# alenzhao/Mitty

Hardware: AMD Instinct MI355X
Metric: paired 2x150bp reads/sec at 30x WGS, 1/2/4/8 MI355X; qname POS/CIGAR bit-exact (higher is better)
Workload: dtype int64+u8

## Files before the change

include/mitty_hip.h:

```cpp
#ifndef MITTY_HIP_H
#define MITTY_HIP_H

#include <stdint.h>

#ifdef __cplusplus
extern "C" {
#endif

typedef struct mh_ctx mh_ctx;

enum {
  MH_OK = 0,
  MH_E_ARG = -1,
  MH_E_HIP = -2,
  MH_E_OOM = -3,
  MH_E_CAPACITY = -4,
  MH_E_COMPLEX_VARIANT = -5,
  MH_E_SEED = -6,
  MH_E_STATE = -7,
  MH_E_NO_DEVICE = -8
};

enum { MH_RNG_MITTY = 0, MH_RNG_PHILOX = 1 };

int32_t mh_version(void);
int32_t mh_device_count(int32_t *out);
int32_t mh_create(int32_t device, mh_ctx **out);
int32_t mh_destroy(mh_ctx *ctx);
const char *mh_last_error(const mh_ctx *ctx);
int32_t mh_sync(mh_ctx *ctx);

int32_t mh_selftest_scan_fault(mh_ctx *ctx);
int32_t mh_selftest_scan(mh_ctx *ctx, int32_t kind, int32_t fields, const int64_t *in, int64_t n, int32_t repeat,
                         int64_t *incl, int64_t *excl, int64_t *total, int64_t *info);
int32_t mh_selftest_sort(mh_ctx *ctx, const uint32_t *keys, int64_t n, int32_t end_bit, uint32_t *keys_out,
                         uint32_t *vals_out);

int32_t mh_read_model_params(int64_t mean_rlen, double coverage, double *p, int64_t *passes);
int32_t mh_work_units(uint64_t seed, const int32_t *ploidy, int64_t n_regions, int64_t passes,
                      int32_t *out_region, int32_t *out_cpy, uint32_t *out_seed, int64_t *out_n);

int32_t mh_upload_contig(mh_ctx *ctx, int32_t contig_id, const char *seq, int64_t len);
int32_t mh_release_contig(mh_ctx *ctx, int32_t contig_id);
int32_t mh_build_haplotype(mh_ctx *ctx, int32_t slot, int32_t contig_id, int64_t ref_start_pos,
                           const int64_t *v_pos, const uint8_t *v_op, const int64_t *v_oplen,
                           const int64_t *v_alt_off, const int64_t *v_alt_len, const char *alt_pool,
                           int64_t alt_pool_len, int64_t n_var,
                           int64_t *out_n_nodes, int64_t *out_p_min, int64_t *out_p_max);
int32_t mh_upload_variants(mh_ctx *ctx, int32_t vset, const int64_t *v_pos, const uint8_t *v_op,
                           const int64_t *v_oplen, const int64_t *v_alt_off, const int64_t *v_alt_len,
                           const char *alt_pool, int64_t alt_pool_len, int64_t n_var);
int32_t mh_build_haplotype_vset(mh_ctx *ctx, int32_t slot, int32_t contig_id, int64_t ref_start_pos, int32_t vset,
                                int64_t *out_n_nodes, int64_t *out_p_min, int64_t *out_p_max);
int32_t mh_build_haplotypes_vset(mh_ctx *ctx, int32_t n, const int32_t *slots, const int32_t *contig_ids,
                                 const int64_t *ref_starts, const int32_t *vsets, int64_t *out_n_nodes,
                                 int64_t *out_p_min, int64_t *out_p_max);
int32_t mh_prefetch_haplotypes_vset(mh_ctx *ctx, int32_t n, const int32_t *slots, const int32_t *contig_ids,
                                    const int64_t *ref_starts, const int32_t *vsets, int32_t n_units,
                                    const int32_t *unit_slots, const uint64_t *unit_seeds, double p);
int32_t mh_release_variants(mh_ctx *ctx, int32_t vset);
int32_t mh_get_nodes(mh_ctx *ctx, int32_t slot, int64_t *ps, int64_t *pr, uint8_t *op, int64_t *oplen,
                     char *hap, int64_t hap_cap, int64_t *hap_len);
int32_t mh_get_haplotype_aux(mh_ctx *ctx, int32_t slot, char *rc, int64_t rc_cap, int64_t *hap_len,
                             int64_t *run_start, int64_t *run_end, int64_t run_cap, int64_t *n_runs,
                             int32_t *bkt, int64_t bkt_cap, int64_t *n_bkt);
int32_t mh_release_haplotype(mh_ctx *ctx, int32_t slot);
int32_t mh_expand_variant(int64_t samp_pos, int64_t ref_pos, int64_t ref_start_pos, int64_t v_pos, int32_t op,
                          int64_t oplen, int64_t *out, int32_t *n_nodes, int64_t *samp_next, int64_t *ref_next);

int32_t mh_sample_templates(mh_ctx *ctx, int32_t slot, double p, int32_t rlen, const double *cum_tlen,
                            int32_t n_tlen, uint64_t seed, int32_t rng_mode, int64_t *out_n_templates);
int32_t mh_sample_templates_span(mh_ctx *ctx, int64_t p_min, int64_t p_max, double p, int32_t rlen,
                                 const double *cum_tlen, int32_t n_tlen, uint64_t seed, int32_t rng_mode,
                                 int64_t *out_n_templates);
int32_t mh_sample_units(mh_ctx *ctx, int32_t n_units, const int32_t *tpl_ids, const int32_t *slots,
                        const uint64_t *seeds, double p, int32_t rlen, const double *cum_tlen, int32_t n_tlen,
                        int32_t rng_mode, int64_t *out_n);
int32_t mh_sample_units_async(mh_ctx *ctx, int32_t n_units, const int32_t *tpl_ids, const int32_t *slots,
                              const uint64_t *seeds, double p, int32_t rlen, const double *cum_tlen, int32_t n_tlen,
                              int32_t rng_mode);
int32_t mh_templates_count(mh_ctx *ctx, int32_t tpl_id, int64_t *n);
int32_t mh_use_templates(mh_ctx *ctx, int32_t tpl_id);
int32_t mh_release_templates(mh_ctx *ctx, int32_t tpl_id);
int32_t mh_set_templates(mh_ctx *ctx, const int8_t *fo0, const int64_t *pos0, const int64_t *pos1, int64_t n,
                         int32_t rlen);
int32_t mh_get_templates(mh_ctx *ctx, int8_t *fo0, int64_t *pos0, int64_t *pos1, int64_t cap, int64_t *n);
int32_t mh_templates_export(mh_ctx *ctx, int32_t tpl_id, int32_t on_device, int8_t *fo0, int64_t *pos0,
                            int64_t *pos1, int64_t cap, int64_t *n);
int32_t mh_templates_import(mh_ctx *ctx, int32_t tpl_id, int32_t on_device, const int8_t *fo0, const int64_t *pos0,
                            const int64_t *pos1, int64_t n, int32_t rlen);

int32_t mh_emit_reads(mh_ctx *ctx, int32_t slot, const char *serial_stub, const char *chrom, int64_t cpy,
                      int32_t write_fastq2, uint64_t unit_key, int64_t *out_kept, int64_t *out_bytes1,
                      int64_t *out_bytes2);
int32_t mh_emit_prepare(mh_ctx *ctx, int32_t slot, const char *serial_stub, const char *chrom, int64_t cpy,
                        int32_t write_fastq2, uint64_t unit_key, int64_t *out_kept, int64_t *out_b1, int64_t *out_b2);
int32_t mh_emit_reads_range(mh_ctx *ctx, int32_t slot, const char *serial_stub, const char *chrom, int64_t cpy,
                            int32_t write_fastq2, uint64_t unit_key, int64_t t_begin, int64_t t_end,
                            int64_t cnt_base, int64_t *out_kept, int64_t *out_bytes1, int64_t *out_bytes2);
int32_t mh_emit_reads_async(mh_ctx *ctx, int32_t slot, const char *serial_stub, const char *chrom, int64_t cpy,
                            int32_t write_fastq2, uint64_t unit_key);
int32_t mh_emit_collect(mh_ctx *ctx, int64_t *out, int64_t cap, int64_t *n_units);
int32_t mh_emit_measure(mh_ctx *ctx, int32_t slot, const char *serial_stub, const char *chrom, int64_t cpy,
                        int32_t write_fastq2, uint64_t unit_key, int64_t t_begin, int64_t t_end, int64_t cnt_base,
                        int64_t *out_kept, int64_t *out_b1, int64_t *out_b2);
int32_t mh_count_kept(mh_ctx *ctx, int32_t slot, int64_t t_begin, int64_t t_end, int64_t *out_kept);
int32_t mh_output_size(mh_ctx *ctx, int64_t *bytes1, int64_t *bytes2);
int32_t mh_output_fetch(mh_ctx *ctx, int64_t offset1, char *fq1, int64_t len1, int64_t offset2, char *fq2,
                        int64_t len2);
int32_t mh_output_fetch_async(mh_ctx *ctx, int64_t offset1, char *fq1, int64_t len1, int64_t offset2, char *fq2,
                              int64_t len2, int32_t *ticket);
int32_t mh_output_fetch_wait(mh_ctx *ctx, int32_t ticket);
int32_t mh_output_reset(mh_ctx *ctx);
int32_t mh_host_alloc(int64_t bytes, void **out);
int32_t mh_host_free(void *p);
int32_t mh_device_cache_trim(int64_t *freed_bytes);
int32_t mh_device_live_bytes(int64_t *live, int64_t *peak, int32_t reset_peak);

int32_t mh_read_batch(mh_ctx *ctx, int32_t slot, const int64_t *p, const int64_t *l, int64_t n,
                      int64_t *out_pos, int64_t *out_n0, int64_t *out_n1,
                      char *cigar, int64_t cigar_cap, int64_t *cigar_off, int64_t *cigar_used,
                      char *vlist, int64_t vlist_cap, int64_t *vlist_off, int64_t *vlist_used,
                      char *seq, int64_t seq_cap, int64_t *seq_off, int64_t *seq_used);

int32_t mh_bam_set_refs(mh_ctx *ctx, int32_t n_refs, const char *names, const int64_t *lengths);
int32_t mh_bam_add_fastq(mh_ctx *ctx, const char *fq1, int64_t len1, const char *fq2, int64_t len2,
                         int64_t max_templates, int64_t *used1, int64_t *used2, int64_t *templates);
int32_t mh_bam_add_output(mh_ctx *ctx, int64_t max_templates, int64_t *templates);
int32_t mh_bam_records(mh_ctx *ctx, int64_t *n_records, int64_t *bytes);
int32_t mh_bam_sort(mh_ctx *ctx);
int32_t mh_bam_write(mh_ctx *ctx, const char *bam_path, const char *header_text, int64_t header_len, int32_t level,
                     int32_t threads, const char *bai_path, int64_t *out_records, int64_t *out_bytes);
int32_t mh_bam_reset(mh_ctx *ctx);
int32_t mh_bam_set_capacity(mh_ctx *ctx, int64_t bytes);
int32_t mh_bam_set_spill_dir(mh_ctx *ctx, const char *dir);
int32_t mh_bam_spilled(mh_ctx *ctx, int64_t *bytes, int64_t *blocks);
int32_t mh_bam_export(mh_ctx *ctx, int64_t r0, int64_t r1, uint8_t *recs, int64_t *roff, uint64_t *keys,
                      int32_t *info);
int32_t mh_bam_import(mh_ctx *ctx, const uint8_t *recs, const int64_t *roff, const uint64_t *keys, const int32_t *info,
                      int64_t n);
int32_t mh_bam_write_gpu(mh_ctx *ctx, const char *bam_path, const char *header_text, int64_t header_len,
                         const char *bai_path, int64_t *out_records, int64_t *out_bytes, int64_t *out_file_bytes);
int32_t mh_bam_partition(mh_ctx *ctx, const uint64_t *splitters, int32_t n_dest, uint64_t tie_base, int64_t *seg_off,
                         int64_t *seg_n, int64_t *seg_bytes);
int32_t mh_bam_partition_fetch(mh_ctx *ctx, void *out, int64_t cap);
int32_t mh_bam_import_tie(mh_ctx *ctx, const uint8_t *recs, const int64_t *roff, const uint64_t *keys,
                          const int32_t *info, const uint64_t *ties, int64_t n);
int32_t mh_bam_sorted_head(mh_ctx *ctx, int64_t len, uint8_t *out);
int32_t mh_bam_write_part(mh_ctx *ctx, const char *path, const char *header_text, int64_t header_len, int64_t skip,
                          const uint8_t *tail, int64_t tail_len, int32_t eof, int64_t *out_blocks, int64_t *out_data_pos,
                          int64_t *out_bytes, int64_t *boff, int64_t boff_cap);
int32_t mh_bam_bai_runs(mh_ctx *ctx, int64_t *n_runs, int64_t *runs, int64_t runs_cap, int64_t *n_win, int64_t *win,
                        int64_t win_cap, int64_t *ref_nwin);

typedef struct mh_bamfile mh_bamfile;
int32_t mh_bamfile_open(const char *path, int32_t threads, mh_bamfile **out);
int32_t mh_bamfile_open_gpu(const char *path, int32_t device, int32_t threads, mh_bamfile **out);
const char *mh_bamfile_error(const mh_bamfile *f);
int32_t mh_bamfile_header(const mh_bamfile *f, const char **text, int64_t *text_len, int32_t *n_ref,
                          const char **names, const int64_t **lengths);
int32_t mh_bamfile_next(mh_bamfile *f, int64_t max_bytes, const uint8_t **recs, int64_t *len, const int64_t **roff,
                        int64_t *n);
int32_t mh_bamfile_close(mh_bamfile *f);

int32_t mh_score_begin(mh_ctx *ctx, int32_t n_refs, const char *names, int32_t max_d, int32_t max_v_len,
                       int32_t strict, const char *sample_prefix);
int32_t mh_score_add_records(mh_ctx *ctx, const uint8_t *recs, int64_t len, const int64_t *roff, int64_t n);
int32_t mh_score_add_store(mh_ctx *ctx);
int32_t mh_score_result(mh_ctx *ctx, uint64_t *mq_mat, uint64_t *derr_mat, int64_t *counts);
int32_t mh_score_reset(mh_ctx *ctx);

#define MH_MODEL_NO_RLEN INT64_MAX
int32_t mh_model_begin(mh_ctx *ctx, int32_t n_refs, int32_t every, int32_t min_mq, int32_t max_bq, int32_t max_bp,
                       int32_t max_tlen);
int32_t mh_model_add_records(mh_ctx *ctx, const uint8_t *recs, int64_t len, const int64_t *roff, int64_t n);
int32_t mh_model_add_store(mh_ctx *ctx);
int32_t mh_model_result(mh_ctx *ctx, uint64_t *bq_mat, uint64_t *tlen_mat, int64_t *counts);
int32_t mh_model_reset(mh_ctx *ctx);

#define MH_COV_NO_POS INT64_MAX
int32_t mh_cov_begin(mh_ctx *ctx, int32_t n_refs, const int64_t *lengths, int64_t block_len);
int32_t mh_cov_add_records(mh_ctx *ctx, const uint8_t *recs, int64_t len, const int64_t *roff, int64_t n);
int32_t mh_cov_add_store(mh_ctx *ctx);
int32_t mh_cov_gc(mh_ctx *ctx, int32_t ref_index, int32_t contig_id);
int32_t mh_cov_result(mh_ctx *ctx, int32_t ref_index, uint32_t *n_n, uint32_t *n_gc, int64_t *covered,
                      uint64_t *span_sum, int64_t *min_pos, int64_t *max_end, int64_t n_blocks, int64_t *counts);
int32_t mh_cov_reset(mh_ctx *ctx);

#define MH_BQ_MAX_BP 500
// ... 68 lines not shown
```

mitty_amd/_native.py:

```python
import ctypes
import os
import sys

import numpy as np

LIB_PATH = (os.environ.get('MH_LIB') or
            os.path.join(os.path.dirname(os.path.abspath(__file__)), '_lib', 'libmitty_hip.so'))

MH_OK, MH_E_ARG, MH_E_HIP, MH_E_OOM, MH_E_CAPACITY, MH_E_COMPLEX_VARIANT, MH_E_SEED, MH_E_STATE, MH_E_NO_DEVICE = \
  0, -1, -2, -3, -4, -5, -6, -7, -8
MH_RNG_MITTY, MH_RNG_PHILOX = 0, 1

EXPORTS = ['mh_version', 'mh_device_count', 'mh_create', 'mh_destroy', 'mh_last_error', 'mh_sync',
           'mh_selftest_scan_fault', 'mh_selftest_scan', 'mh_selftest_sort', 'mh_selftest_bgzf',
           'mh_read_model_params', 'mh_work_units', 'mh_upload_contig', 'mh_release_contig', 'mh_build_haplotype', 'mh_upload_variants', 'mh_build_haplotype_vset', 'mh_build_haplotypes_vset', 'mh_prefetch_haplotypes_vset', 'mh_release_variants', 'mh_get_nodes', 'mh_get_haplotype_aux',
           'mh_release_haplotype', 'mh_expand_variant', 'mh_sample_templates', 'mh_sample_templates_span', 'mh_set_templates',
           'mh_get_templates', 'mh_templates_export', 'mh_templates_import', 'mh_emit_reads', 'mh_emit_prepare', 'mh_emit_reads_async', 'mh_emit_collect', 'mh_output_size', 'mh_output_fetch', 'mh_output_reset', 'mh_host_alloc', 'mh_host_free', 'mh_device_cache_trim', 'mh_device_live_bytes',
           'mh_read_batch', 'mh_set_corruption', 'mh_set_corruption_stream', 'mh_get_corruption_stream', 'mh_stage_times', 'mh_enable_timing', 'mh_sample_units', 'mh_sample_units_async', 'mh_templates_count',
           'mh_use_templates', 'mh_release_templates', 'mh_mt_window_at', 'mh_fixup_count', 'mh_set_emit_mode', 'mh_set_decode_mode',
           'mh_emit_reads_range', 'mh_emit_measure', 'mh_count_kept', 'mh_bam_set_refs', 'mh_bam_add_fastq', 'mh_bam_add_output',
           'mh_bam_records', 'mh_bam_set_capacity', 'mh_bam_set_spill_dir', 'mh_bam_spilled', 'mh_bam_export', 'mh_bam_import', 'mh_bam_sort', 'mh_bam_write', 'mh_bam_write_gpu', 'mh_bam_reset', 'mh_bam_partition', 'mh_bam_partition_fetch', 'mh_bam_import_tie', 'mh_bam_sorted_head', 'mh_bam_write_part', 'mh_bam_bai_runs', 'mh_corrupt_fastq', 'mh_bgzf_compress', 'mh_bgzf_eof', 'mh_bgzf_compress_device', 'mh_bgzf_compress_gpu', 'mh_output_bgzf',
           'mh_output_bgzf_range', 'mh_output_bgzf_pair', 'mh_output_bgzf_wait', 'mh_output_fetch_async',
           'mh_output_fetch_wait',
           'mh_vcf_open', 'mh_vcf_error', 'mh_vcf_close', 'mh_vcf_region', 'mh_vcf_copy', 'mh_vcf_filter',
           'mh_bamfile_open', 'mh_bamfile_open_gpu', 'mh_bgzf_inflate_gpu', 'mh_bamfile_error', 'mh_bamfile_header', 'mh_bamfile_next', 'mh_bamfile_close',
           'mh_score_begin', 'mh_score_add_records', 'mh_score_add_store', 'mh_score_result', 'mh_score_reset',
           'mh_model_begin', 'mh_model_add_records', 'mh_model_add_store', 'mh_model_result', 'mh_model_reset',
           'mh_cov_begin', 'mh_cov_add_records', 'mh_cov_add_store', 'mh_cov_gc', 'mh_cov_result', 'mh_cov_reset',
           'mh_bq_begin', 'mh_bq_add_records', 'mh_bq_add_store', 'mh_bq_result', 'mh_bq_reset',
           'mh_fasta_open', 'mh_fasta_error', 'mh_fasta_count', 'mh_fasta_contig', 'mh_fasta_copy', 'mh_fasta_close']


MODEL_NO_RLEN = (1 << 63) - 1
COV_NO_POS = (1 << 63) - 1
BQ_MAX_BP, BQ_MAX_BQ = 500, 100


class NativeError(RuntimeError):
  pass


class NativeUnavailable(NativeError):
  pass


_lib = None

c_i32, c_i64, c_u64, c_dbl, c_vp = ctypes.c_int32, ctypes.c_int64, ctypes.c_uint64, ctypes.c_double, ctypes.c_void_p
P_i64 = ctypes.POINTER(c_i64)


def _sig(L, name, args, res=c_i32):
  f = getattr(L, name)
  f.argtypes = args
  f.restype = res


def lib():
  global _lib
  if _lib is not None:
    return _lib
  if not os.path.exists(LIB_PATH):
    raise NativeUnavailable('libmitty_hip.so not built ({}); run __graft_entry__.build() or make -C '
                            'mitty_amd/csrc'.format(LIB_PATH))
  if 'torch' not in sys.modules and int(os.environ.get('WORLD_SIZE', '1')) > 1:
    import torch
  L = ctypes.CDLL(LIB_PATH)
  _sig(L, 'mh_version', [])
  _sig(L, 'mh_device_count', [ctypes.POINTER(c_i32)])
  _sig(L, 'mh_create', [c_i32, ctypes.POINTER(c_vp)])
  _sig(L, 'mh_destroy', [c_vp])
  _sig(L, 'mh_last_error', [c_vp], ctypes.c_char_p)
  _sig(L, 'mh_sync', [c_vp])
  _sig(L, 'mh_selftest_scan_fault', [c_vp])
  _sig(L, 'mh_selftest_scan', [c_vp, c_i32, c_i32, c_vp, c_i64, c_i32, c_vp, c_vp, c_vp, c_vp])
  _sig(L, 'mh_selftest_sort', [c_vp, c_vp, c_i64, c_i32, c_vp, c_vp])
  _sig(L, 'mh_selftest_bgzf', [c_vp, c_vp, c_i64, c_i32, c_vp, c_i64, P_i64])
  _sig(L, 'mh_read_model_params', [c_i64, c_dbl, ctypes.POINTER(c_dbl), P_i64])
  _sig(L, 'mh_work_units', [c_u64, c_vp, c_i64, c_i64, c_vp, c_vp, c_vp, P_i64])
  _sig(L, 'mh_upload_contig', [c_vp, c_i32, c_vp, c_i64])
  _sig(L, 'mh_release_contig', [c_vp, c_i32])
  _sig(L, 'mh_upload_variants', [c_vp, c_i32, c_vp, c_vp, c_vp, c_vp, c_vp, c_vp, c_i64, c_i64])
  _sig(L, 'mh_build_haplotype_vset', [c_vp, c_i32, c_i32, c_i64, c_i32, c_vp, c_vp, c_vp])
  _sig(L, 'mh_release_variants', [c_vp, c_i32])
  _sig(L, 'mh_build_haplotype', [c_vp, c_i32, c_i32, c_i64, c_vp, c_vp, c_vp, c_vp, c_vp, c_vp, c_i64, c_i64,
                                 P_i64, P_i64, P_i64])
  _sig(L, 'mh_get_nodes', [c_vp, c_i32, c_vp, c_vp, c_vp, c_vp, c_vp, c_i64, P_i64])
  _sig(L, 'mh_get_haplotype_aux', [c_vp, c_i32, c_vp, c_i64, P_i64, c_vp, c_vp, c_i64, P_i64, c_vp, c_i64, P_i64])
  _sig(L, 'mh_release_haplotype', [c_vp, c_i32])
  _sig(L, 'mh_bgzf_compress_device', [c_vp, c_vp, c_i64, c_vp, c_i64, P_i64])
  _sig(L, 'mh_bgzf_compress_gpu', [c_vp, c_vp, c_i64, c_vp, c_i64, P_i64])
  _sig(L, 'mh_output_bgzf', [c_vp, c_i32, c_vp, c_i64, P_i64])
  _sig(L, 'mh_output_bgzf_range', [c_vp, c_i32, c_i64, c_i64, c_vp, c_i64, P_i64])
  _sig(L, 'mh_output_bgzf_pair', [c_vp, c_i64, c_i64, c_i64, c_vp, c_i64, c_vp, c_i64, P_i64, P_i64,
                                  ctypes.POINTER(c_i32)])
  _sig(L, 'mh_output_bgzf_wait', [c_vp, c_i32])
  _sig(L, 'mh_output_fetch_async', [c_vp, c_i64, c_vp, c_i64, c_i64, c_vp, c_i64, ctypes.POINTER(c_i32)])
  _sig(L, 'mh_output_fetch_wait', [c_vp, c_i32])
  _sig(L, 'mh_expand_variant', [c_i64, c_i64, c_i64, c_i64, c_i32, c_i64, P_i64, ctypes.POINTER(c_i32), P_i64, P_i64])
  _sig(L, 'mh_sample_templates', [c_vp, c_i32, c_dbl, c_i32, c_vp, c_i32, c_u64, c_i32, P_i64])
  _sig(L, 'mh_sample_templates_span', [c_vp, c_i64, c_i64, c_dbl, c_i32, c_vp, c_i32, c_u64, c_i32, P_i64])
  _sig(L, 'mh_set_templates', [c_vp, c_vp, c_vp, c_vp, c_i64, c_i32])
  _sig(L, 'mh_get_templates', [c_vp, c_vp, c_vp, c_vp, c_i64, P_i64])
  _sig(L, 'mh_emit_reads', [c_vp, c_i32, ctypes.c_char_p, ctypes.c_char_p, c_i64, c_i32, c_u64, P_i64, P_i64, P_i64])
  _sig(L, 'mh_emit_prepare', [c_vp, c_i32, ctypes.c_char_p, ctypes.c_char_p, c_i64, c_i32, c_u64, P_i64, P_i64, P_i64])
  _sig(L, 'mh_emit_reads_async', [c_vp, c_i32, ctypes.c_char_p, ctypes.c_char_p, c_i64, c_i32, c_u64])
  _sig(L, 'mh_emit_collect', [c_vp, c_vp, c_i64, P_i64])
  _sig(L, 'mh_build_haplotypes_vset', [c_vp, c_i32, c_vp, c_vp, c_vp, c_vp, c_vp, c_vp, c_vp])
  _sig(L, 'mh_prefetch_haplotypes_vset', [c_vp, c_i32, c_vp, c_vp, c_vp, c_vp, c_i32, c_vp, c_vp, c_dbl])
  _sig(L, 'mh_emit_reads_range', [c_vp, c_i32, ctypes.c_char_p, ctypes.c_char_p, c_i64, c_i32, c_u64, c_i64, c_i64,
                                   c_i64, P_i64, P_i64, P_i64])
  _sig(L, 'mh_count_kept', [c_vp, c_i32, c_i64, c_i64, P_i64])
  _sig(L, 'mh_emit_measure', [c_vp, c_i32, ctypes.c_char_p, ctypes.c_char_p, c_i64, c_i32, c_u64, c_i64, c_i64, c_i64,
                              P_i64, P_i64, P_i64])
  _sig(L, 'mh_bam_set_refs', [c_vp, c_i32, ctypes.c_char_p, c_vp])
  _sig(L, 'mh_bam_add_fastq', [c_vp, c_vp, c_i64, c_vp, c_i64, c_i64, P_i64, P_i64, P_i64])
  _sig(L, 'mh_bam_add_output', [c_vp, c_i64, P_i64])
  _sig(L, 'mh_bam_records', [c_vp, P_i64, P_i64])
  _sig(L, 'mh_bam_set_capacity', [c_vp, c_i64])
  _sig(L, 'mh_bam_spilled', [c_vp, P_i64, P_i64])
  _sig(L, 'mh_bam_export', [c_vp, c_i64, c_i64, c_vp, c_vp, c_vp, c_vp])
  _sig(L, 'mh_bam_import', [c_vp, c_vp, c_vp, c_vp, c_vp, c_i64])
  _sig(L, 'mh_bam_partition', [c_vp, c_vp, c_i32, ctypes.c_uint64, c_vp, c_vp, c_vp])
  _sig(L, 'mh_bam_set_spill_dir', [c_vp, ctypes.c_char_p])
  _sig(L, 'mh_bam_partition_fetch', [c_vp, c_vp, c_i64])
  _sig(L, 'mh_bam_import_tie', [c_vp, c_vp, c_vp, c_vp, c_vp, c_vp, c_i64])
  _sig(L, 'mh_bam_sorted_head', [c_vp, c_i64, c_vp])
  _sig(L, 'mh_bam_write_part', [c_vp, ctypes.c_char_p, ctypes.c_char_p, c_i64, c_i64, c_vp, c_i64, c_i32, P_i64,
                                P_i64, P_i64, c_vp, c_i64])
  _sig(L, 'mh_bam_bai_runs', [c_vp, P_i64, c_vp, c_i64, P_i64, c_vp, c_i64, c_vp])
  _sig(L, 'mh_bam_write', [c_vp, ctypes.c_char_p, ctypes.c_char_p, c_i64, c_i32, c_i32, ctypes.c_char_p, P_i64,
                           P_i64])
  _sig(L, 'mh_bam_write_gpu', [c_vp, ctypes.c_char_p, ctypes.c_char_p, c_i64, ctypes.c_char_p, P_i64, P_i64, P_i64])
  _sig(L, 'mh_bam_reset', [c_vp])
  _sig(L, 'mh_bam_sort', [c_vp])
  _sig(L, 'mh_corrupt_fastq', [c_vp, c_vp, c_i64, c_vp, c_i64, c_i64, P_i64, P_i64, P_i64])
  _sig(L, 'mh_bgzf_compress', [c_vp, c_i64, c_i32, c_i32, c_vp, c_i64, P_i64])
  _sig(L, 'mh_bgzf_eof', [c_vp])
  _sig(L, 'mh_vcf_open', [ctypes.c_char_p, ctypes.c_char_p, ctypes.POINTER(c_vp)])
  _sig(L, 'mh_vcf_error', [c_vp], ctypes.c_char_p)
  _sig(L, 'mh_vcf_close', [c_vp])
  _sig(L, 'mh_vcf_region', [c_vp, ctypes.c_char_p, c_i64, c_i64, ctypes.POINTER(c_i32), c_vp, c_vp, c_i32])
  _sig(L, 'mh_vcf_copy', [c_vp, c_i32, c_vp, c_vp, c_vp, c_vp, c_vp, c_vp])
  _sig(L, 'mh_vcf_filter', [ctypes.c_char_p, ctypes.c_char_p, c_i32, c_vp, c_vp, c_vp, ctypes.c_char_p, c_i32, c_i32,
                            P_i64, P_i64, ctypes.c_char_p, c_i32])
  _sig(L, 'mh_bamfile_open', [ctypes.c_char_p, c_i32, ctypes.POINTER(c_vp)])
  _sig(L, 'mh_bamfile_open_gpu', [ctypes.c_char_p, c_i32, c_i32, ctypes.POINTER(c_vp)])
  _sig(L, 'mh_bgzf_inflate_gpu', [c_i32, c_vp, c_i64, c_vp, c_i64, P_i64, P_i64])
  _sig(L, 'mh_bamfile_error', [c_vp], ctypes.c_char_p)
  _sig(L, 'mh_bamfile_header', [c_vp, ctypes.POINTER(c_vp), P_i64, ctypes.POINTER(c_i32), ctypes.POINTER(c_vp),
                                ctypes.POINTER(c_vp)])
  _sig(L, 'mh_bamfile_next', [c_vp, c_i64, ctypes.POINTER(c_vp), P_i64, ctypes.POINTER(c_vp), P_i64])
  _sig(L, 'mh_bamfile_close', [c_vp])
  _sig(L, 'mh_score_begin', [c_vp, c_i32, ctypes.c_char_p, c_i32, c_i32, c_i32, ctypes.c_char_p])
  _sig(L, 'mh_score_add_records', [c_vp, c_vp, c_i64, c_vp, c_i64])
  _sig(L, 'mh_score_add_store', [c_vp])
  _sig(L, 'mh_score_result', [c_vp, c_vp, c_vp, c_vp])
  _sig(L, 'mh_score_reset', [c_vp])
  _sig(L, 'mh_model_begin', [c_vp, c_i32, c_i32, c_i32, c_i32, c_i32, c_i32])
  _sig(L, 'mh_model_add_records', [c_vp, c_vp, c_i64, c_vp, c_i64])
  _sig(L, 'mh_model_add_store', [c_vp])
  _sig(L, 'mh_model_result', [c_vp, c_vp, c_vp, c_vp])
  _sig(L, 'mh_model_reset', [c_vp])
  _sig(L, 'mh_cov_begin', [c_vp, c_i32, c_vp, c_i64])
  _sig(L, 'mh_cov_add_records', [c_vp, c_vp, c_i64, c_vp, c_i64])
  _sig(L, 'mh_cov_add_store', [c_vp])
  _sig(L, 'mh_cov_gc', [c_vp, c_i32, c_i32])
  _sig(L, 'mh_cov_result', [c_vp, c_i32, c_vp, c_vp, c_vp, c_vp, c_vp, c_vp, c_i64, c_vp])
  _sig(L, 'mh_cov_reset', [c_vp])
  _sig(L, 'mh_bq_begin', [c_vp, c_i32])
  _sig(L, 'mh_bq_add_records', [c_vp, c_vp, c_i64, c_vp, c_i64])
  _sig(L, 'mh_bq_add_store', [c_vp])
  _sig(L, 'mh_bq_result', [c_vp, c_i32, c_vp, c_vp])
  _sig(L, 'mh_bq_reset', [c_vp])
  _sig(L, 'mh_fasta_open', [ctypes.c_char_p, c_vp, ctypes.POINTER(c_vp)])
  _sig(L, 'mh_fasta_error', [c_vp], ctypes.c_char_p)
  _sig(L, 'mh_fasta_count', [c_vp, ctypes.POINTER(c_i32)])
  _sig(L, 'mh_fasta_contig', [c_vp, c_i32, ctypes.POINTER(ctypes.c_char_p), ctypes.POINTER(c_vp), P_i64])
  _sig(L, 'mh_fasta_copy', [c_vp, c_i32, c_vp])
  _sig(L, 'mh_fasta_close', [c_vp])
  _sig(L, 'mh_output_size', [c_vp, P_i64, P_i64])
  _sig(L, 'mh_output_fetch', [c_vp, c_i64, c_vp, c_i64, c_i64, c_vp, c_i64])
  _sig(L, 'mh_output_reset', [c_vp])
  _sig(L, 'mh_host_alloc', [c_i64, ctypes.POINTER(c_vp)])
  _sig(L, 'mh_host_free', [c_vp])
  _sig(L, 'mh_device_cache_trim', [ctypes.POINTER(c_i64)])
  _sig(L, 'mh_device_live_bytes', [ctypes.POINTER(c_i64), ctypes.POINTER(c_i64), c_i32])
  _sig(L, 'mh_read_batch', [c_vp, c_i32, c_vp, c_vp, c_i64, c_vp, c_vp, c_vp,
                            c_vp, c_i64, c_vp, P_i64, c_vp, c_i64, c_vp, P_i64, c_vp, c_i64, c_vp, P_i64])
  _sig(L, 'mh_set_corruption', [c_vp, c_i32, c_vp, c_i32, c_i32, c_vp, c_u64])
  _sig(L, 'mh_templates_export', [c_vp, c_i32, c_i32, c_vp, c_vp, c_vp, c_i64, P_i64])
  _sig(L, 'mh_templates_import', [c_vp, c_i32, c_i32, c_vp, c_vp, c_vp, c_i64, c_i32])
  _sig(L, 'mh_set_corruption_stream', [c_vp, c_i32, c_u64, c_vp, c_i32])
  _sig(L, 'mh_get_corruption_stream', [c_vp, c_vp, ctypes.POINTER(c_i32), P_i64])
  _sig(L, 'mh_stage_times', [c_vp, ctypes.POINTER(ctypes.c_char_p), ctypes.POINTER(c_dbl), c_i32,
                             ctypes.POINTER(c_i32)])
  _sig(L, 'mh_enable_timing', [c_vp, c_i32])
  _sig(L, 'mh_sample_units', [c_vp, c_i32, c_vp, c_vp, c_vp, c_dbl, c_i32, c_vp, c_i32, c_i32, c_vp])
  _sig(L, 'mh_sample_units_async', [c_vp, c_i32, c_vp, c_vp, c_vp, c_dbl, c_i32, c_vp, c_i32, c_i32])
  _sig(L, 'mh_templates_count', [c_vp, c_i32, c_vp])
  _sig(L, 'mh_use_templates', [c_vp, c_i32])
  _sig(L, 'mh_release_templates', [c_vp, c_i32])
  _sig(L, 'mh_mt_window_at', [ctypes.c_uint32, c_u64, c_vp])
  _sig(L, 'mh_fixup_count', [c_vp, P_i64])
  _sig(L, 'mh_set_emit_mode', [c_vp, c_i32])
  _sig(L, 'mh_set_decode_mode', [c_vp, c_i32])
  _lib = L
  return L


def mt_window_at(seed, offset):
  out = np.empty(624, np.uint32)
  rc = lib().mh_mt_window_at(int(seed), int(offset), _ptr(out))
  if rc:
    _raise(rc, 'mh_mt_window_at failed')
  return out


def bgzf_compress(data, level=6, threads=8):
  n = len(data)
  src = np.frombuffer(data, np.uint8) if n else np.zeros(1, np.uint8)
  cap = n + (n // 0xff00 + 1) * 64 + 64
  out = np.empty(cap, np.uint8)
  used = c_i64()
  rc = lib().mh_bgzf_compress(_ptr(src), n, int(level), int(threads), _ptr(out), cap, ctypes.byref(used))
  if rc == MH_E_CAPACITY:
    out = np.empty(used.value, np.uint8)
    rc = lib().mh_bgzf_compress(_ptr(src), n, int(level), int(threads), _ptr(out), used.value, ctypes.byref(used))
  if rc:
# ... 802 lines not shown
    self._chk(self._L.mh_bq_add_store(self._h))

  def bq_result(self, ref_index):
    mat = np.zeros((BQ_MAX_BP, BQ_MAX_BQ), np.uint64)
    cnt = np.zeros(8, np.int64)
    self._chk(self._L.mh_bq_result(self._h, int(ref_index), _ptr(mat), _ptr(cnt)))
    return mat, _model_counts(cnt)

  def bq_reset(self):
    self._chk(self._L.mh_bq_reset(self._h))

  def bam_partition(self, splitters, tie_base):
    sp = np.ascontiguousarray(splitters, dtype=np.uint64)
    nd = len(sp) + 1
    off, n, nb = np.zeros(nd + 1, np.int64), np.zeros(nd, np.int64), np.zeros(nd, np.int64)
    self._chk(self._L.mh_bam_partition(self._h, _ptr(sp) if len(sp) else None, nd, int(tie_base), _ptr(off), _ptr(n),
                                       _ptr(nb)))
    return off, n, nb

  def bam_partition_fetch(self, ptr, cap):
    self._chk(self._L.mh_bam_partition_fetch(self._h, c_vp(ptr), int(cap)))

  def bam_import_tie(self, n, nbytes, ptr):
    o_roff, o_key, o_info, o_tie, _ = bam_part_layout(n, nbytes)
    self._chk(self._L.mh_bam_import_tie(self._h, c_vp(ptr), c_vp(ptr + o_roff), c_vp(ptr + o_key),
                                        c_vp(ptr + o_info), c_vp(ptr + o_tie), int(n)))

  def bam_sorted_head(self, n):
    out = np.empty(max(int(n), 1), np.uint8)
    self._chk(self._L.mh_bam_sorted_head(self._h, int(n), _ptr(out)))
    return out[:int(n)].tobytes()

  def bam_write_part(self, path, header_text=None, skip=0, tail=b'', eof=False):
    nb, dp, fb = c_i64(), c_i64(), c_i64()
    h = header_text.encode() if header_text is not None else b''
    t = np.frombuffer(tail, np.uint8) if len(tail) else None
    args = (self._h, path.encode(), h, len(h) if header_text is not None else -1, int(skip), _ptr(t), len(tail),
            1 if eof else 0, ctypes.byref(nb), ctypes.byref(dp), ctypes.byref(fb))
    n_bytes = self.bam_records()[1]
    cap = (n_bytes - int(skip) + len(tail)) // 0xff00 + 2
    boff = np.zeros(cap, np.int64)
    self._chk(self._L.mh_bam_write_part(*args, _ptr(boff), cap))
    return nb.value, dp.value, fb.value, boff[:nb.value + 1]

  def bam_bai_runs(self, n_refs):
    nr, nw = c_i64(), c_i64()
    self._chk(self._L.mh_bam_bai_runs(self._h, ctypes.byref(nr), None, 0, ctypes.byref(nw), None, 0, None))
    runs = np.zeros(max(4 * nr.value, 4), np.int64)
    win = np.zeros(max(nw.value, 1), np.int64)
    rn = np.zeros(max(n_refs, 1), np.int64)
    self._chk(self._L.mh_bam_bai_runs(self._h, ctypes.byref(nr), _ptr(runs), len(runs), ctypes.byref(nw), _ptr(win),
                                      len(win), _ptr(rn)))
    return runs[:4 * nr.value].reshape(-1, 4), win[:nw.value], rn[:n_refs]

  def bam_sort(self):
    self._chk(self._L.mh_bam_sort(self._h))

  def corrupt_fastq(self, fq1, fq2=None, t_base=0):
    u1, u2, t = c_i64(), c_i64(), c_i64()
    a1 = np.frombuffer(fq1, np.uint8) if len(fq1) else np.zeros(1, np.uint8)
    a2 = None if fq2 is None else (np.frombuffer(fq2, np.uint8) if len(fq2) else np.zeros(1, np.uint8))
    self._chk(self._L.mh_corrupt_fastq(self._h, _ptr(a1), len(fq1), None if a2 is None else _ptr(a2),
                                       0 if fq2 is None else len(fq2), int(t_base), ctypes.byref(u1),
                                       ctypes.byref(u2), ctypes.byref(t)))
    return u1.value, u2.value, t.value

  def read_batch(self, slot, p, l):
    p = np.ascontiguousarray(p, dtype=np.int64)
    l = np.ascontiguousarray(l, dtype=np.int64)
    n = len(p)
    pos, n0, n1 = (np.empty(max(n, 1), np.int64) for _ in range(3))
    offs = [np.empty(n + 1, np.int64) for _ in range(3)]
    used = [c_i64() for _ in range(3)]
    caps = [max(64, 64 * n), max(64, 16 * n), max(64, int(l.sum()) + 16 if n else 64)]
    for _ in range(2):
      bufs = [np.empty(c, np.uint8) for c in caps]
      rc = self._L.mh_read_batch(self._h, slot, _ptr(p), _ptr(l), n, _ptr(pos), _ptr(n0), _ptr(n1),
                                 _ptr(bufs[0]), caps[0], _ptr(offs[0]), ctypes.byref(used[0]),
                                 _ptr(bufs[1]), caps[1], _ptr(offs[1]), ctypes.byref(used[1]),
                                 _ptr(bufs[2]), caps[2], _ptr(offs[2]), ctypes.byref(used[2]))
      if rc == MH_E_CAPACITY:
        caps = [max(c, u.value + 16) for c, u in zip(caps, used)]
        continue
      self._chk(rc)
      break
    texts = [b[:u.value].tobytes().decode('latin-1') for b, u in zip(bufs, used)]
    return pos[:n], n0[:n], n1[:n], texts, offs

  def set_corruption(self, enable, cum_bq=None, phred_p=None, seed=0):
    if not enable:
      self._chk(self._L.mh_set_corruption(self._h, 0, None, 0, 0, None, 0))
      return
    cb = np.ascontiguousarray(cum_bq, dtype=np.float64)
    ph = np.ascontiguousarray(phred_p, dtype=np.float64)
    self._chk(self._L.mh_set_corruption(self._h, 1, _ptr(cb), cb.shape[1], cb.shape[2], _ptr(ph), int(seed)))

  def templates_export(self, tpl_id, fo0=None, pos0=None, pos1=None, cap=None):
    n = c_i64()
    if fo0 is not None:
      self._chk(self._L.mh_templates_export(self._h, int(tpl_id), 1, c_vp(fo0), c_vp(pos0), c_vp(pos1), int(cap),
                                            ctypes.byref(n)))
      return n.value
    self._L.mh_templates_export(self._h, int(tpl_id), 0, None, None, None, 0, ctypes.byref(n))
    m = n.value
    a, b, c = np.empty(max(m, 1), np.int8), np.empty(max(m, 1), np.int64), np.empty(max(m, 1), np.int64)
    self._chk(self._L.mh_templates_export(self._h, int(tpl_id), 0, _ptr(a), _ptr(b), _ptr(c), max(m, 1),
                                          ctypes.byref(n)))
    return a[:m], b[:m], c[:m]

  def templates_import(self, tpl_id, n, rlen, fo0, pos0, pos1, on_device=False):
    if on_device:
      self._chk(self._L.mh_templates_import(self._h, int(tpl_id), 1, c_vp(fo0), c_vp(pos0), c_vp(pos1), int(n),
                                            int(rlen)))
      return
    a = np.ascontiguousarray(fo0, dtype=np.int8)
    b = np.ascontiguousarray(pos0, dtype=np.int64)
    c = np.ascontiguousarray(pos1, dtype=np.int64)
    self._chk(self._L.mh_templates_import(self._h, int(tpl_id), 0, _ptr(a), _ptr(b), _ptr(c), int(n), int(rlen)))

  def set_corruption_stream(self, rng_mode, seed=0, key=None, pos=624):
    k = None if key is None else np.ascontiguousarray(key, dtype=np.uint32)
    if k is not None and k.shape != (624,):
      raise ValueError('MT19937 key must hold 624 words')
    self._chk(self._L.mh_set_corruption_stream(self._h, int(rng_mode), int(seed), None if k is None else _ptr(k),
                                               int(pos)))

  def get_corruption_stream(self):
    key = np.empty(624, np.uint32)
    pos, words = c_i32(), c_i64()
    self._chk(self._L.mh_get_corruption_stream(self._h, _ptr(key), ctypes.byref(pos), ctypes.byref(words)))
    return key, pos.value, words.value

  def enable_timing(self, on=True):
    self._chk(self._L.mh_enable_timing(self._h, 1 if on else 0))

  def stage_times(self):
    n = c_i32()
    self._L.mh_stage_times(self._h, None, None, 0, ctypes.byref(n))
    names = (ctypes.c_char_p * max(n.value, 1))()
    ms = (c_dbl * max(n.value, 1))()
    self._L.mh_stage_times(self._h, names, ms, n.value, ctypes.byref(n))
    return [(names[i].decode(), ms[i]) for i in range(n.value)]

  def sync(self):
    self._chk(self._L.mh_sync(self._h))

  def selftest_sort(self, keys, end_bit):
    import numpy as np
    k = np.ascontiguousarray(keys, dtype=np.uint32)
    ko, vo = np.empty_like(k), np.empty_like(k)
    self._chk(self._L.mh_selftest_sort(self._h, k.ctypes.data, k.size, int(end_bit), ko.ctypes.data, vo.ctypes.data))
    return ko, vo

  def selftest_scan(self, kind, x, repeat=1):
    x = np.ascontiguousarray(x, dtype=np.int64)
    if x.ndim not in (1, 2):
      raise ValueError('selftest_scan: a 1-d or 2-d array')
    fields = 1 if x.ndim == 1 else x.shape[1]
    n = x.shape[0]
    scans = int(kind) != 3
    incl = np.empty_like(x) if scans else None
    excl = np.empty_like(x) if scans else None
    total, info = np.zeros(max(fields, 1), np.int64), np.zeros(2, np.int64)
    self._chk(self._L.mh_selftest_scan(self._h, int(kind), int(fields), _ptr(x), n, int(repeat), _ptr(incl),
                                       _ptr(excl), _ptr(total), _ptr(info)))
    return incl, excl, (total[0] if x.ndim == 1 else total), (int(info[0]), int(info[1]))

  def selftest_bgzf(self, data, misalign=0):
    n = len(data)
    if n == 0:
      return b''
    src = np.frombuffer(data, np.uint8)
    out = np.empty(n + (n // 0xff00 + 2) * 40 + 64, np.uint8)
    used = c_i64()
    self._chk(self._L.mh_selftest_bgzf(self._h, _ptr(src), n, int(misalign), _ptr(out), len(out), ctypes.byref(used)))
    return out[:used.value].tobytes()

  def selftest_scan_fault(self):
    rc = self._L.mh_selftest_scan_fault(self._h)
    return rc, self._L.mh_last_error(self._h).decode(errors='replace')


def expand_variant(samp_pos, ref_pos, ref_start_pos, v_pos, op, oplen):
  out = (c_i64 * 10)()
  n, sn, rn = c_i32(), c_i64(), c_i64()
  rc = lib().mh_expand_variant(int(samp_pos), int(ref_pos), int(ref_start_pos), int(v_pos), ord(op), int(oplen), out,
                               ctypes.byref(n), ctypes.byref(sn), ctypes.byref(rn))
  if rc:
    _raise(rc, 'mh_expand_variant: bad variant (op {!r}, oplen {})'.format(op, oplen))
  return [(out[5 * j], out[5 * j + 1], chr(out[5 * j + 2]), out[5 * j + 3], out[5 * j + 4])
          for j in range(n.value)], sn.value, rn.value
```

mitty_amd/csrc/mh_api.hip:

```cpp
#include <sys/mman.h>
#include <sys/syscall.h>
#include <unistd.h>

#include <algorithm>
#include <atomic>
#include <cctype>
#include <cstdio>
#include <unordered_map>
#include <chrono>
#include <cmath>
#include <condition_variable>
#include <cstring>
#include <map>
#include <mutex>
#include <thread>
#include <type_traits>

#include "mh_bgzf.h"
#include <vector>

#include "mh_corrupt.h"
#include "mh_internal.h"
#include "mh_scan.h"
#include "mh_sort.h"
// ... 407 lines not shown
  ctx->device = device;
  {
    static std::atomic<int> next{0};
    ctx->fault_slot = 1 + next++ % (SCAN_FAULT_SLOTS - 1);
    (void)scan_fault_take(ctx->fault_slot);
  }
  int prio_lo = 0, prio_hi = 0;
  (void)hipSetDevice(device);
  (void)hipDeviceGetStreamPriorityRange(&prio_lo, &prio_hi);
  if (hipSetDevice(device) != hipSuccess ||
      hipStreamCreateWithPriority(&ctx->stream, hipStreamNonBlocking, prio_hi) != hipSuccess ||
      hipStreamCreateWithPriority(&ctx->stream2, hipStreamNonBlocking, prio_hi) != hipSuccess ||
      hipEventCreateWithFlags(&ctx->ev_fork, hipEventDisableTiming) != hipSuccess ||
      hipEventCreateWithFlags(&ctx->ev_join, hipEventDisableTiming) != hipSuccess ||
      hipStreamCreateWithPriority(&ctx->wstream, hipStreamNonBlocking, prio_lo) != hipSuccess ||
      hipEventCreateWithFlags(&ctx->ev_ready, hipEventDisableTiming) != hipSuccess ||
      hipEventCreateWithFlags(&ctx->ev_writer, hipEventDisableTiming) != hipSuccess ||
      [&] {
        for (auto &e : ctx->eset)
          if (hipEventCreateWithFlags(&e.done, hipEventDisableTiming) != hipSuccess ||
              hipEventCreateWithFlags(&e.rb, hipEventDisableTiming) != hipSuccess ||
              hipHostMalloc((void **)&e.h_stat, 64 + 8192, hipHostMallocDefault) != hipSuccess)
            return true;
        return false;
      }()) {
    delete ctx;
    return MH_E_HIP;
  }
  hipDeviceProp_t prop;
  if (hipGetDeviceProperties(&prop, device) == hipSuccess) ctx->max_cu = prop.multiProcessorCount;
  *out = ctx;
  return MH_OK;
}

int32_t mh_destroy(mh_ctx *ctx) {
  if (!ctx) return MH_OK;
  if (ctx->pf_thread.joinable()) ctx->pf_thread.join();
  (void)hipSetDevice(ctx->device);
  (void)hipStreamSynchronize(ctx->wstream);
  (void)hipStreamSynchronize(ctx->stream);
  if (ctx->stream2) (void)hipStreamSynchronize(ctx->stream2);
  if (ctx->pstream) (void)hipStreamSynchronize(ctx->pstream);
  for (auto x : ctx->xstream)
    if (x) (void)hipStreamSynchronize(x);
  for (auto &kv : ctx->contigs) release(kv.second.seq);
  for (auto &kv : ctx->haps) release_hap(kv.second);
  for (auto &h : ctx->hap_spare) release_hap(h);
  for (auto &kv : ctx->vsets) release_vars(kv.second);
  for (auto &kv : ctx->tsets) {
    release(kv.second.fo0); release(kv.second.pos0); release(kv.second.pos1); release(kv.second.n0);
    if (kv.second.used) (void)hipEventDestroy(kv.second.used);
  }
  release(ctx->jump_polys); release(ctx->perm_tmp); release(ctx->nrun_tmp); release(ctx->dec_buf);
  for (auto &b : ctx->pb) release(b);
  release(ctx->pb_tmp);
  release(ctx->gz_slots); release(ctx->gz_tok); release(ctx->gz_info); release(ctx->gz_off); release(ctx->gz_scan); release(ctx->gz_out);
  release(ctx->gz_in);
  for (auto &b : ctx->s) release(b);
  for (auto &b : ctx->lane2) release(b);
  for (auto &l : ctx->xlane)
    for (auto &b : l) release(b);
  for (auto &b : ctx->xscan) release(b);
  release(ctx->scan_partials); release(ctx->scan_partials2); release(ctx->d_small);
  release(ctx->corrupt_cum); release(ctx->corrupt_phred);
  release(ctx->out1); release(ctx->out2);
  release(ctx->cr_rows);
  release(ctx->cr_codes);
  release(ctx->scan_partials_w);
  for (auto &b : ctx->sl2) release(b);
  for (auto &b : ctx->sl3) release(b);
  ctx->tail_state.reset();
  for (hipEvent_t e : ctx->ev_gz)
    if (e) (void)hipEventDestroy(e);
  for (hipEvent_t e : ctx->ev_fetch)
    if (e) (void)hipEventDestroy(e);
  if (ctx->h_small) (void)hipHostFree(ctx->h_small);
  if (ctx->h_small3) (void)hipHostFree(ctx->h_small3);
  if (ctx->h_units) (void)hipHostFree(ctx->h_units);
  for (uint8_t *p : ctx->h_bam_pin)
    if (p) (void)hipHostFree(p);
  for (auto &e : ctx->eset) {
    release(e.recs); release(e.off); release(e.tsum); release(e.tpre); release(e.stat); release(e.crrec);
    (void)hipEventDestroy(e.done);
    if (e.rb) (void)hipEventDestroy(e.rb);
    if (e.h_stat) (void)hipHostFree(e.h_stat);
  }
  (void)hipEventDestroy(ctx->ev_ready);
  (void)hipEventDestroy(ctx->ev_writer);
  (void)hipStreamDestroy(ctx->wstream);
  bam_release(ctx->bam);
  score_release(ctx->score);
  model_release(ctx->model);
  model_release(ctx->bq);
  cov_release(ctx->cov);
  if (ctx->ev_fork) (void)hipEventDestroy(ctx->ev_fork);
  if (ctx->ev_join) (void)hipEventDestroy(ctx->ev_join);
  if (ctx->stream2) (void)hipStreamDestroy(ctx->stream2);
  if (ctx->ev_prefetch) (void)hipEventDestroy(ctx->ev_prefetch);
  if (ctx->pstream) (void)hipStreamDestroy(ctx->pstream);
  for (int l = 0; l < 2; l++) {
    if (ctx->xstream[l]) (void)hipStreamDestroy(ctx->xstream[l]);
    if (ctx->ev_xjoin[l]) (void)hipEventDestroy(ctx->ev_xjoin[l]);
  }
  (void)hipStreamDestroy(ctx->stream);
  delete ctx;
  return MH_OK;
}

const char *mh_last_error(const mh_ctx *ctx) { return ctx ? ctx->err.c_str() : "null context"; }

int32_t mh_sync(mh_ctx *ctx) {
  CTX_GUARD(ctx);
  MH_TRY(lazy_resolve(ctx));
  SYNCCHK(ctx, hipStreamSynchronize(ctx->stream));
  return MH_OK;
}

namespace {
struct LoadOne {
  __device__ int64_t operator()(int64_t) const { return 1; }
};
struct StoreCheck {
  int32_t *bad;
  __device__ void operator()(int64_t i, int64_t, int64_t ex) const {
    if (ex != i) atomicOr(bad, 1);
  }
};
}

int32_t mh_selftest_sort(mh_ctx *ctx, const uint32_t *keys, int64_t n, int32_t end_bit, uint32_t *keys_out,
                         uint32_t *vals_out) {
  CTX_GUARD(ctx);
  if (n < 0 || (n > 0 && (!keys || !keys_out || !vals_out)) || end_bit < 0 || end_bit > 32)
    return arg_fail(ctx, MH_E_ARG, "bad sort arguments");
  hipStream_t st = ctx->stream;
  size_t tmp = 0;
  HIPCHK(ctx, lsd_sort_pairs_iota(nullptr, tmp, nullptr, nullptr, nullptr, n, (unsigned)end_bit, st));
  DevBuf b;
  const size_t kb = (4 * (size_t)n + 255) & ~(size_t)255;
  MH_TRY(ensure(ctx, b, 3 * kb + tmp + 256));
  uint32_t *dk = (uint32_t *)b.p, *ko = (uint32_t *)((char *)b.p + kb), *vo = (uint32_t *)((char *)b.p + 2 * kb);
  const int32_t rc = [&]() -> int32_t {
    if (n) HIPCHK(ctx, hipMemcpyAsync(dk, keys, 4 * (size_t)n, hipMemcpyHostToDevice, st));
    HIPCHK(ctx, lsd_sort_pairs_iota((char *)b.p + 3 * kb, tmp, dk, ko, vo, n, (unsigned)end_bit, st));
    if (n) {
      HIPCHK(ctx, hipMemcpyAsync(keys_out, ko, 4 * (size_t)n, hipMemcpyDeviceToHost, st));
      HIPCHK(ctx, hipMemcpyAsync(vals_out, vo, 4 * (size_t)n, hipMemcpyDeviceToHost, st));
    }
    SYNCCHK(ctx, hipStreamSynchronize(st));
    return MH_OK;
  }();
  release(b);
  return rc;
}

int32_t mh_selftest_scan(mh_ctx *ctx, int32_t kind, int32_t fields, const int64_t *in, int64_t n, int32_t repeat,
                         int64_t *incl, int64_t *excl, int64_t *total, int64_t *info) {
  CTX_GUARD(ctx);
  if (kind < 0 || kind > 3 || fields < 1 || fields > 3 || (kind == 1 && fields != 1) || n < 0 ||
      n > ((int64_t)1 << 27) || repeat < 1 || repeat > (1 << 20) || ((kind == 1 || kind == 3) && repeat != 1) ||
      !total || !info || (n > 0 && (!in || (kind != 3 && (!incl || !excl)))))
    return arg_fail(ctx, MH_E_ARG, "bad scan self-test arguments");
  if (kind == 2) {
    uint64_t sum[3] = {0, 0, 0};
    for (int64_t i = 0; i < n * fields; i++) {
      if (in[i] < 0) return arg_fail(ctx, MH_E_ARG, "look-back scan: a negative input");
      uint64_t &s = sum[i % fields];
      s += (uint64_t)in[i];
      if (s >= ((uint64_t)1 << 46)) return arg_fail(ctx, MH_E_ARG, "look-back scan: a field's total is 2^46 or more");
    }
  }
  info[0] = info[1] = 0;
  if (fields == 1) return selftest_scan_run<int64_t>(ctx, kind, in, n, repeat, incl, excl, total, info);
  if (fields == 2) return selftest_scan_run<Sc2>(ctx, kind, in, n, repeat, incl, excl, total, info);
  return selftest_scan_run<Sc3>(ctx, kind, in, n, repeat, incl, excl, total, info);
}

int32_t mh_selftest_scan_fault(mh_ctx *ctx) {
  CTX_GUARD(ctx);
  hipStream_t st = ctx->stream;
  const int64_t n = 2 * (int64_t)LB_TILE + 5;
  MH_TRY(ensure(ctx, ctx->scan_partials, scan_lb_scratch_bytes<int64_t>(n)));
  MH_TRY(ensure(ctx, ctx->scan_partials2, scan_lb_scratch_bytes<int64_t>(n)));
  MH_TRY(ensure(ctx, ctx->d_small, 8192 + 256));
  int64_t *tot = (int64_t *)((char *)ctx->d_small.p + 160);
  int32_t *bad = (int32_t *)((char *)ctx->d_small.p + 168);
  auto fault_once = [&](hipStream_t s, void *scratch) -> int32_t {
    HIPCHK(ctx, hipMemsetAsync(bad, 0, 4, s));
    HIPCHK(ctx, device_scan_sum<int64_t>(s, n, LoadOne{}, StoreCheck{bad}, scratch, tot, true));
    SYNCCHK(ctx, hipStreamSynchronize(s));
    return MH_OK;
  };
  int32_t rc_lane = MH_OK;
  std::thread t1([&]() {
    lane_thread_enter(ctx);
    if (hipSetDevice(ctx->device) != hipSuccess) {
      rc_lane = MH_E_HIP;
      return;
    }
    rc_lane = fault_once(ctx->stream2, ctx->scan_partials2.p);
  });
  t1.join();
  if (rc_lane != MH_E_STATE) return arg_fail(ctx, MH_E_HIP, "the timed-out scan of a lane thread was not reported");
  const int32_t rc = fault_once(st, ctx->scan_partials.p);
  if (rc != MH_E_STATE) return arg_fail(ctx, MH_E_HIP, "the timed-out scan was not reported");
  const std::string msg = ctx->err;
  HIPCHK(ctx, hipMemsetAsync(bad, 0, 4, st));
  HIPCHK(ctx, device_scan_sum<int64_t>(st, n, LoadOne{}, StoreCheck{bad}, ctx->scan_partials.p, tot));
  int32_t hb = 0;
  HIPCHK(ctx, hipMemcpyAsync(&hb, bad, 4, hipMemcpyDeviceToHost, st));
  SYNCCHK(ctx, hipStreamSynchronize(st));
  if (hb) return arg_fail(ctx, MH_E_HIP, "the scan after the fault is wrong");
  arg_fail(ctx, MH_E_STATE, msg);
  return MH_E_STATE;
}

int32_t mh_read_model_params(int64_t mean_rlen, double coverage, double *p_out, int64_t *passes_out) {
  if (!p_out || !passes_out || mean_rlen <= 0) return MH_E_ARG;
  double p = 1.0;
  int64_t passes = 1;
  while (p > 0.1) {
    passes *= 2;
    p = 0.5 * coverage / (double)(2 * mean_rlen * passes);
  }
  *p_out = p;
  *passes_out = passes;
  return MH_OK;
}

int32_t mh_work_units(uint64_t seed, const int32_t *ploidy, int64_t n_regions, int64_t passes, int32_t *out_region,
                      int32_t *out_cpy, uint32_t *out_seed, int64_t *out_n) {
  if (seed > 0xffffffffull) return MH_E_SEED;
  if (n_regions < 0 || passes < 0 || (n_regions && !ploidy)) return MH_E_ARG;
  HostMT s;
  s.seed((uint32_t)seed);
  uint32_t shuffle_seed = (uint32_t)s.interval(0xfffffffeull);
  int64_t n = 0;
  for (int64_t r = 0; r < n_regions; r++)
    for (int32_t c = 0; c < ploidy[r]; c++)
      for (int64_t k = 0; k < passes; k++) {
        out_region[n] = (int32_t)r;
        out_cpy[n] = c;
        out_seed[n] = (uint32_t)s.interval(0xfffffffeull);
        n++;
      }
  HostMT sh;
  sh.seed(shuffle_seed);
  for (int64_t i = n - 1; i >= 1; i--) {
    int64_t j = (int64_t)sh.interval((uint64_t)i);
    std::swap(out_region[i], out_region[j]);
    std::swap(out_cpy[i], out_cpy[j]);
    std::swap(out_seed[i], out_seed[j]);
  }
  *out_n = n;
  return MH_OK;
}

int32_t mh_upload_contig(mh_ctx *ctx, int32_t contig_id, const char *seq, int64_t len) {
  CTX_GUARD(ctx);
  if (len < 0 || (len > 0 && !seq)) return arg_fail(ctx, MH_E_ARG, "bad contig");
  Contig &c = ctx->contigs[contig_id];
  MH_TRY(ensure(ctx, c.seq, len + 16));
  if (len) HIPCHK(ctx, hipMemcpyAsync(c.seq.p, seq, len, hipMemcpyHostToDevice, ctx->stream));
  SYNCCHK(ctx, hipStreamSynchronize(ctx->stream));
  c.len = len;
  return MH_OK;
}

int32_t mh_release_contig(mh_ctx *ctx, int32_t contig_id) {
  CTX_GUARD(ctx);
  auto it = ctx->contigs.find(contig_id);
  if (it == ctx->contigs.end()) return MH_OK;
  SYNCCHK(ctx, hipStreamSynchronize(ctx->stream));
  release(it->second.seq);
  ctx->contigs.erase(it);
  return MH_OK;
}

static int32_t hap_for_build(mh_ctx *ctx, int32_t slot, int64_t need, Hap **out, hipStream_t st = nullptr) {
  if (!ctx->haps.count(slot)) {
    int best = -1, big = -1;
    for (int i = 0; i < (int)ctx->hap_spare.size(); i++) {
      const Hap &s = ctx->hap_spare[i];
      if (s.used_set && hipEventQuery(s.used) != hipSuccess) continue;
      if (s.hap.cap >= (size_t)need && (best < 0 || s.hap.cap < ctx->hap_spare[best].hap.cap)) best = i;
      if (big < 0 || s.hap.cap > ctx->hap_spare[big].hap.cap) big = i;
    }
    if (best < 0) best = big;
    if (best >= 0) {
      Hap r{};
      const Hap &s = ctx->hap_spare[best];
      r.hap = s.hap; r.rc = s.rc; r.keys = s.keys; r.ps = s.ps; r.pr = s.pr; r.op = s.op; r.oplen = s.oplen;
      r.nrun_s = s.nrun_s; r.nrun_e = s.nrun_e; r.nd = s.nd; r.bkt = s.bkt;
      r.used = s.used; r.used_set = s.used_set;
      ctx->hap_spare.erase(ctx->hap_spare.begin() + best);
      ctx->haps[slot] = r;
    }
  }
  Hap &h = ctx->haps[slot];
  MH_TRY(wait_unused(ctx, h.used, h.used_set, st));
  h.valid = false;
  *out = &h;
  return MH_OK;
}

static int32_t build_from(mh_ctx *ctx, int32_t slot, int32_t contig_id, int64_t ref_start_pos, const VarSet &v,
// ... 1728 lines not shown
```

mitty_amd/csrc/mh_internal.h:

```cpp
#pragma once

#include <hip/hip_runtime.h>

#include <cstdint>
#include <functional>
#include <map>
#include <mutex>
#include <unordered_map>
#include <memory>
#include <string>
#include <thread>
#include <vector>

#include "../../include/mitty_hip.h"

namespace mh {

struct Status {
  int32_t code = MH_OK;
  std::string msg;
};

#define MH_TRY(expr)                        \
  do {                                      \
// ... 120 lines not shown

struct Contig {
  DevBuf seq;
  int64_t len = 0;
};

struct VarSet {
  DevBuf pos, op, oplen, aoff, alen, pool;
  int64_t n = 0, pool_len = 0;
};

struct BamStore {
  bool refs_set = false;
  std::vector<std::string> ref_names;
  std::vector<int64_t> ref_len;
  DevBuf names, name_off;
  DevBuf in1, in2;
  DevBuf nl1, nl2;
  DevBuf tpl;
  DevBuf roff, recs;
  DevBuf key, val, info;
  DevBuf key2, val2, sort_tmp, soff, srecs, sinfo;
  DevBuf bai_lin, bai_runs, bai_out;
  DevBuf tie, tie2, tval, tkey;
  DevBuf part_dest, part_dk, part_ord, part_soff, part_start, part_seg, part_split, part_tmp, send;
  bool use_tie = false;
  int64_t send_bytes = 0;
  int64_t n_rec = 0, bytes = 0;
  int32_t n_files = 0;
  bool sorted = false;
  bool direct = false;
  int64_t cap = 0;
  struct HostBlock {
    uint8_t *p;
    int64_t b0, b1;
    bool mapped = false;
  };
  std::vector<HostBlock> spill;
  int64_t spilled = 0;
  std::string spill_dir;
};

}

#include "mh_recs.h"

namespace mh {

extern const RecTexts SCORE_TEXTS, MODEL_TEXTS, BQ_TEXTS, COV_TEXTS;

struct ScoreState {
  RecSession ses{SCORE_TEXTS};
  int32_t max_d = 0, max_v = 0, strict = 0, n_refs = 0, plen = 0;
  int64_t n_mq = 0, n_dv = 0, n_all = 0;
  DevBuf acc, delta;
  DevBuf names, name_off, prefix;
};

struct ModelState {
  static constexpr int N_REF = 24;
  RecSession ses;
  explicit ModelState(const RecTexts &t) : ses(t) {}
  int32_t n_refs = 0, every = 1, min_mq = 0, max_bq = 0, max_bp = 0, max_tlen = 0;
  int32_t n_tab = 2;
  bool by_ref = false;
  int32_t slab_bp = 0, n_slab = 0;
  int64_t n_bq = 0, n_all = 0;
  DevBuf acc, delta;
  DevBuf desc;
  DevBuf tile_ord;
};

struct CovState {
  static constexpr int N_REF = ModelState::N_REF;
  RecSession ses{COV_TEXTS};
  int32_t n_refs = 0, n_vis = 0;
  int64_t block_len = 0;
  int64_t ln[N_REF] = {0}, cbase[N_REF + 1] = {0}, bbase[N_REF + 1] = {0};
  int64_t n_cells = 0, n_blk = 0;
  DevBuf track, depth;
  DevBuf blk;
  DevBuf cnt;
  DevBuf desc;
  DevBuf partials;
  DevBuf tab;
  bool scanned = false;
};

struct StageTime {
  const char *name;
  hipEvent_t a, b;
};

}

namespace mh {
struct EmitSet {
  DevBuf recs, off;
  DevBuf tsum, tpre;
  DevBuf crrec;
  DevBuf stat;
  int64_t *h_stat = nullptr;
  hipEvent_t rb = nullptr;
  hipEvent_t done = nullptr;
  bool busy = false;
  bool prepared = false;
};
}

struct mh_ctx {
  int fault_slot = 0;
  int device = 0;
  hipStream_t stream = nullptr;
  hipStream_t stream2 = nullptr;
  hipEvent_t ev_fork = nullptr, ev_join = nullptr;
  hipStream_t wstream = nullptr;
  std::shared_ptr<void> tail_state;
  int64_t *h_units = nullptr, *d_units = nullptr;
  hipEvent_t ev_ready = nullptr, ev_writer = nullptr;
  bool writer_pending = false;
  static constexpr int N_ESET = 16;
  mh::EmitSet eset[N_ESET];
  int64_t eset_max_m = 0;
  int eset_i = 0;
  hipStream_t stage_stream = nullptr;
  std::string err;
  int32_t max_cu = 256;

  std::map<int32_t, mh::Contig> contigs;
  std::map<int32_t, mh::Hap> haps;

  std::map<int32_t, mh::TplSet> tsets;
  int32_t cur_tpl = -1;

  mh::DevBuf jump_polys;
  int64_t jump_k = 0, jump_seg = 0;
  int64_t fixups = 0;
  std::map<int32_t, mh::VarSet> vsets;
  std::vector<mh::Hap> hap_spare;
  mh::DevBuf perm_tmp;
  mh::DevBuf pb[6];
  mh::DevBuf pb_tmp;
  mh::DevBuf gz_slots, gz_info, gz_off, gz_scan, gz_out, gz_in;
  mh::DevBuf gz_tok;
  hipEvent_t ev_gz[2] = {nullptr, nullptr};
  hipEvent_t ev_fetch[2] = {nullptr, nullptr};
  bool fetch_pending[2] = {false, false};
  int fetch_next = 0;
  bool gz_pending[2] = {false, false};
  int gz_half = 0;
  mh::DevBuf nrun_tmp;
  mh::DevBuf dec_buf;
  int64_t dec_passes = 0;

  mh::DevBuf s[16];
  mh::DevBuf scan_partials;
  mh::DevBuf lane2[8];
  mh::DevBuf scan_partials2;
  hipStream_t xstream[2] = {nullptr, nullptr};
  mh::DevBuf xlane[2][8];
  mh::DevBuf xscan[2];
  hipEvent_t ev_xjoin[2] = {nullptr, nullptr};
  mh::DevBuf sl2[8];
  hipStream_t pstream = nullptr;
  hipEvent_t ev_prefetch = nullptr;
  bool prefetch_pending = false;
  std::thread pf_thread;
  int32_t pf_rc = 0;
  mh::DevBuf sl3[8];
  int64_t *h_small3 = nullptr;
  mh::PrefetchedWords pf_words;
  mh::DevBuf pinned_small;
  mh::DevBuf d_small;

  bool corrupt_on = false;
  mh::DevBuf corrupt_cum, corrupt_phred;
  int32_t corrupt_max_bp = 0, corrupt_n_bq = 0;
  size_t corrupt_guide_off = 0;
  size_t corrupt_bk_off = 0, corrupt_T16_off = 0, corrupt_Fp16_off = 0;
  size_t corrupt_bkf_off = 0;
  uint64_t corrupt_seed = 0;
  int32_t cx_mode = 0;
  uint32_t cx_seed = 0;
  int64_t cx_pos = 0;
  uint32_t cx_key[624] = {0};
  int32_t cx_kpos = 624;
  mh::DevBuf cx_words, cx_bits, cx_start, cx_aux;

  bool emit_lds_only = false;
  bool decode_sequential = false;
  bool force_fixup = false;
  bool force_geo = false;

  mh::DevBuf out1, out2;
  int64_t used1 = 0, used2 = 0;
  static constexpr int LZ_SLOTS = 4096;
  int64_t *h_lazy = nullptr, *d_lazy = nullptr;
  mh::DevBuf d_cur;
  mh::DevBuf fused_lb;
  struct LazyUnit {
    int32_t slot;
    int64_t gen;
    int64_t known[3];
  };
  std::vector<LazyUnit> lazy;
  std::vector<int64_t> lazy_done;
  int64_t lazy_seq = 0;
  int64_t lazy_gen = 0;
  bool chain_open = false;
  int64_t used_ub1 = 0, used_ub2 = 0;
  int64_t batch_left = 0;
  bool emit_two_pass = false;
  bool emit_single = false;
  mh::DevBuf cr_rows, cr_codes;
  mh::DevBuf scan_partials_w;
  int64_t *h_small = nullptr;
  uint8_t *h_bam_pin[2] = {nullptr, nullptr};

  bool timing = false;
  std::vector<mh::StageTime> stages;
  std::vector<mh::StageTime> pending;
  std::vector<std::pair<const char *, double>> last_times;

  mh::BamStore bam;
  mh::ScoreState score;
  mh::ModelState model{mh::MODEL_TEXTS}, bq{mh::BQ_TEXTS};
  mh::CovState cov;
};

namespace mh {

int32_t hip_fail(mh_ctx *ctx, hipError_t e, const char *what, const char *file, int line);
int32_t arg_fail(mh_ctx *ctx, int32_t code, const std::string &msg);

#define HIPCHK(ctx, call)                                                     \
  do {                                                                        \
    hipError_t _e = (call);                                                   \
    if (_e != hipSuccess) return ::mh::hip_fail((ctx), _e, #call, __FILE__, __LINE__); \
  } while (0)

int32_t scan_fault_fail(mh_ctx *ctx);
#define SYNCCHK(ctx, call)                                                    \
  do {                                                                        \
    HIPCHK(ctx, call);                                                        \
    if (::mh::scan_fault_pending(ctx)) return ::mh::scan_fault_fail(ctx);     \
  } while (0)
bool scan_fault_pending(const mh_ctx *ctx);

int32_t ensure(mh_ctx *ctx, DevBuf &b, size_t bytes);
int32_t ensure_keep(mh_ctx *ctx, DevBuf &b, size_t bytes, size_t keep, int32_t grow_shift = 1);
void release(DevBuf &b);
void release_hap(Hap &h);
int32_t join_writer(mh_ctx *ctx);
int32_t mark_used(mh_ctx *ctx, hipEvent_t &ev, bool &set);
int32_t wait_unused(mh_ctx *ctx, hipEvent_t ev, bool set, hipStream_t st = nullptr);
int32_t join_prefetch(mh_ctx *ctx);
int32_t prefetch_words(mh_ctx *ctx, hipStream_t st, int32_t n_units, const int64_t *p_min, const int64_t *p_max,
                       const uint64_t *seeds, double p);

void stage_begin(mh_ctx *ctx, const char *name);
void stage_end(mh_ctx *ctx);
void stages_collect(mh_ctx *ctx);
struct StageScope {
  mh_ctx *ctx;
  bool open = true;
  StageScope(mh_ctx *c, const char *name) : ctx(c) { stage_begin(c, name); }
  StageScope(const StageScope &) = delete;
  StageScope &operator=(const StageScope &) = delete;
  void end() {
    if (open) stage_end(ctx);
    open = false;
  }
  ~StageScope() { end(); }
};
struct StageStreamScope {
  mh_ctx *ctx;
  hipStream_t prev;
  StageStreamScope(mh_ctx *c, hipStream_t st) : ctx(c), prev(c->stage_stream) { c->stage_stream = st; }
  StageStreamScope(const StageStreamScope &) = delete;
  StageStreamScope &operator=(const StageStreamScope &) = delete;
  ~StageStreamScope() { ctx->stage_stream = prev; }
};

inline void prep_drop(mh_ctx *ctx, const TplSet &tp) {
  if (tp.prep.valid) ctx->eset[tp.prep.set].prepared = false;
  tp.prep.valid = false;
}

inline unsigned grid_for(int64_t n, int threads, int64_t cap = 1 << 20) {
  int64_t g = (n + threads - 1) / threads;
  if (g < 1) g = 1;
  if (g > cap) g = cap;
  return (unsigned)g;
}

int32_t var_upload(mh_ctx *ctx, VarSet &v, const int64_t *v_pos, const uint8_t *v_op, const int64_t *v_oplen,
                   const int64_t *v_alt_off, const int64_t *v_alt_len, const char *alt_pool, int64_t alt_pool_len,
                   int64_t n_var);
void release_vars(VarSet &v);
int32_t splice_build(mh_ctx *ctx, Hap &h, const Contig &c, int64_t ref_start_pos, const VarSet &v, int lane = 0);

int32_t sample_units(mh_ctx *ctx, int32_t n_units, const int32_t *tpl_ids, const int64_t *p_min, const int64_t *p_max,
                     const uint64_t *seeds, double p, int32_t rlen, const double *cum_tlen, int32_t n_tlen,
                     int32_t rng_mode, int64_t *out_n, const NodeIdx *nidx = nullptr);
int32_t sample_units_async(mh_ctx *ctx, int32_t n_units, const int32_t *tpl_ids, const int64_t *p_min,
                           const int64_t *p_max, const uint64_t *seeds, double p, int32_t rlen, const double *cum_tlen,
                           int32_t n_tlen, int32_t rng_mode, const NodeIdx *nidx = nullptr);
int32_t tpl_resolve(mh_ctx *ctx, TplSet &ts);
int32_t tpl_resolve_all(mh_ctx *ctx);

int32_t sync_writers(mh_ctx *ctx);
int32_t bgzf_device(mh_ctx *ctx, hipStream_t st, const uint8_t *d_in, int64_t n, uint8_t *d_out, int64_t cap,
                    int64_t *used, std::vector<int64_t> *boff = nullptr,
                    const std::function<void(int64_t, int64_t)> *on_piece = nullptr);
int64_t bgzf_device_bound(int64_t n);
int gpu_numa_node(int dev);
std::mutex &host_allocs_mu();
std::unordered_map<void *, size_t> &host_allocs();
int64_t *pinned_small(mh_ctx *ctx);
int32_t emit_reads(mh_ctx *ctx, const Hap &h, int32_t slot, const char *serial_stub, const char *chrom, int64_t cpy,
                   int32_t write_fastq2, uint64_t unit_key, int64_t t_begin, int64_t t_end, int64_t cnt_base,
                   bool prepare_only, int64_t *out_kept, int64_t *out_b1, int64_t *out_b2);
int32_t count_kept(mh_ctx *ctx, const Hap &h, int64_t t_begin, int64_t t_end, int64_t *out_kept);
int32_t emit_unit_async(mh_ctx *ctx, const Hap &h, const char *serial_stub, const char *chrom, int64_t cpy,
                        int32_t write_fastq2, uint64_t unit_key, bool *queued);
int32_t lazy_resolve(mh_ctx *ctx);

int32_t bam_set_refs(mh_ctx *ctx, int32_t n_refs, const char *names, const int64_t *lengths);
int32_t bam_add(mh_ctx *ctx, const uint8_t *d1, int64_t len1, const uint8_t *d2, int64_t len2, int64_t max_templates,
                int64_t *used1, int64_t *used2, int64_t *templates, bool sorted_direct = false);
int32_t bam_sort(mh_ctx *ctx, const void *pa = nullptr);
int32_t bam_undirect(mh_ctx *ctx);
int32_t bam_fetch_sorted(mh_ctx *ctx, uint8_t *recs, int64_t *soff, int32_t *info);
int32_t bam_spill(mh_ctx *ctx);
int32_t bam_export(mh_ctx *ctx, int64_t r0, int64_t r1, uint8_t *recs, int64_t *roff, uint64_t *key, int32_t *info);
int32_t bam_import(mh_ctx *ctx, const uint8_t *recs, const int64_t *roff, const uint64_t *key, const int32_t *info,
                   int64_t n, const uint64_t *tie = nullptr);
int32_t bam_partition(mh_ctx *ctx, const uint64_t *split, int32_t n_dest, uint64_t tie_base, int64_t *seg_off,
                      int64_t *seg_n, int64_t *seg_bytes);
int32_t bam_bai_raw(mh_ctx *ctx, std::vector<int64_t> &runs, std::vector<int64_t> &win, std::vector<uint32_t> &nwin,
                    std::vector<int64_t> &woff, bool *ok);
struct BamHostOrder {
  std::vector<uint32_t> val;
  std::vector<int64_t> roff, soff;
};
int32_t bam_host_order(mh_ctx *ctx, BamHostOrder &o);
void bam_assemble(const BamStore &B, const BamHostOrder &o, int64_t w0, int64_t w1, uint8_t *dst, int threads);
struct BaiPlan;
int32_t bam_bai_plan(mh_ctx *ctx, BaiPlan &plan, std::vector<int64_t> &offs, bool *ok);
void bam_release(BamStore &B);
void bam_free_spill(BamStore &B);
int32_t newline_index(mh_ctx *ctx, const uint8_t *b, int64_t len, DevBuf &nl, int64_t *count);
int32_t score_begin(mh_ctx *ctx, int32_t n_refs, const char *names, int32_t max_d, int32_t max_v_len, int32_t strict,
                    const char *sample_prefix);
int32_t score_add_records(mh_ctx *ctx, const uint8_t *recs, int64_t len, const int64_t *roff, int64_t n);
int32_t score_add_store(mh_ctx *ctx);
int32_t score_result(mh_ctx *ctx, uint64_t *mq_mat, uint64_t *derr_mat, int64_t *counts);
int32_t score_reset(mh_ctx *ctx);
void score_release(ScoreState &S);
int32_t model_begin(mh_ctx *ctx, ModelState &S, int32_t n_refs, int32_t every, int32_t min_mq, int32_t max_bq,
                    int32_t max_bp, int32_t max_tlen, bool by_ref);
int32_t model_add_records(mh_ctx *ctx, ModelState &S, const uint8_t *recs, int64_t len, const int64_t *roff,
                          int64_t n);
int32_t model_add_store(mh_ctx *ctx, ModelState &S);
int32_t model_result(mh_ctx *ctx, ModelState &S, uint64_t *bq_mat, uint64_t *tlen_mat, int64_t *counts);
int32_t model_result_table(mh_ctx *ctx, ModelState &S, int32_t tab, uint64_t *mat, int64_t *counts);
int32_t model_reset(mh_ctx *ctx, ModelState &S);
void model_release(ModelState &S);
int32_t cov_begin(mh_ctx *ctx, int32_t n_refs, const int64_t *lengths, int64_t block_len);
int32_t cov_add_records(mh_ctx *ctx, const uint8_t *recs, int64_t len, const int64_t *roff, int64_t n);
int32_t cov_add_store(mh_ctx *ctx);
int32_t cov_gc(mh_ctx *ctx, int32_t ref_index, int32_t contig_id);
int32_t cov_result(mh_ctx *ctx, int32_t ref_index, uint32_t *n_n, uint32_t *n_gc, int64_t *covered, uint64_t *span_sum,
                   int64_t *min_pos, int64_t *max_end, int64_t n_blocks, int64_t *counts);
int32_t cov_reset(mh_ctx *ctx);
void cov_release(CovState &S);
int32_t corrupt_fastq(mh_ctx *ctx, const uint8_t *d0, int64_t len0, const uint8_t *d1, int64_t len1, int64_t t_base,
                      int64_t *used0, int64_t *used1, int64_t *templates);

int32_t read_batch(mh_ctx *ctx, const Hap &h, const int64_t *p, const int64_t *l, int64_t n, int64_t *out_pos,
                   int64_t *out_n0, int64_t *out_n1, char *cigar, int64_t cigar_cap, int64_t *cigar_off,
                   int64_t *cigar_used, char *vlist, int64_t vlist_cap, int64_t *vlist_off, int64_t *vlist_used,
                   char *seq, int64_t seq_cap, int64_t *seq_off, int64_t *seq_used);


int32_t mt_stream_words(mh_ctx *ctx, hipStream_t st, uint32_t seed, int64_t first, int64_t count, DevBuf &out,
                        DevBuf &jobs_buf, int64_t *lead);
int32_t mt_state_words(mh_ctx *ctx, hipStream_t st, const uint32_t *key624, int32_t pos, int64_t count, DevBuf &out,
                       DevBuf &key_buf);

struct CorruptCfg;
CorruptCfg corrupt_cfg(const mh_ctx *ctx, uint64_t unit_key, int64_t t_base);

struct HostMT {
  uint32_t key[624];
  int pos;
  void seed(uint32_t s);
  uint32_t next();
  double next_double();
  uint64_t interval(uint64_t max);
};

}
```

mitty_amd/csrc/mh_sample.hip:

```cpp
#include <algorithm>
#include <cmath>
#include <cstdio>
#include <cstdlib>
#include <cstring>


#include "mh_device.h"
#include "mh_internal.h"
#include "mh_scan.h"
#include "mh_sort.h"


namespace mh {

namespace jump {
void jump_poly_words(uint64_t L, int64_t k, uint32_t *out624);
}

namespace {

constexpr uint32_t MT_UP = 0x80000000u, MT_LO = 0x7fffffffu, MT_A = 0x9908b0dfu;
constexpr int64_t SEG_WORDS_DEFAULT = 624 * 640;
static int64_t seg_words() { return SEG_WORDS_DEFAULT; }

// ... 14 lines not shown
    uint32_t v = seed;
    st[0] = v;
    for (int i = 1; i < 624; i++) {
      v = 1812433253u * (v ^ (v >> 30)) + (uint32_t)i;
      st[i] = v;
    }
  }
  lds_barrier();
}

template <typename Emit>
__device__ __forceinline__ void mt_twist_block(const uint32_t *o, uint32_t *nw, Emit emit) {
  const int t = threadIdx.x;
  if (t < 227) {
    uint32_t v = o[t + 397] ^ mt_mix(o[t], o[t + 1]);
    nw[t] = v;
    emit(t, mt_temper(v));
  }
  lds_barrier();
  if (t < 227) {
    int i = 227 + t;
    uint32_t v = nw[i - 227] ^ mt_mix(o[i], o[i + 1]);
    nw[i] = v;
    emit(i, mt_temper(v));
  }
  lds_barrier();
  if (t < 170) {
    int i = 454 + t;
    uint32_t nxt = (i < 623) ? o[i + 1] : nw[0];
    uint32_t v = nw[i - 227] ^ mt_mix(o[i], nxt);
    nw[i] = v;
    emit(i, mt_temper(v));
  }
  lds_barrier();
}

struct SegJob {
  uint32_t *out;
  int64_t start;
  int64_t count;
  uint32_t seed;
  int32_t k;
};

constexpr int CB_WORDS = 2048;
constexpr int CB_MASK = CB_WORDS - 1;
constexpr int JW = 208;
constexpr int CB_ZERO = 2 * CB_WORDS;
constexpr int JB = 16;

__global__ void __launch_bounds__(256) k_mt_segments(const SegJob *jobs, const uint32_t *polys) {
  __shared__ uint32_t cb[2 * CB_WORDS + 624];
  __shared__ uint32_t gp[624];
  const SegJob job = jobs[blockIdx.x];
  const int t = threadIdx.x;
  mt_seed_lds(cb, job.seed);
  if (job.k > 0) {
    const uint32_t *g = polys + (int64_t)job.k * 624;
    for (int i = t; i < 624; i += 256) {
      gp[i] = g[i];
      cb[CB_WORDS + i] = cb[i];
      cb[CB_ZERO + i] = 0u;
    }
    lds_barrier();
    const int w = t < JW ? t : 0;
    uint32_t a0 = 0, a1 = 0, a2 = 0;
    int32_t G = 624;
    for (int pw = 0; pw < 624; pw++) {
      const int kb = pw * 32;
      while (G <= kb + 31 + 623) {
#pragma unroll
        for (int ph = 0; ph < 3; ph++) {
          if (t < (ph < 2 ? 227 : 170)) {
            const int i = G + 227 * ph + t;
            const uint32_t v = cb[(i - 227) & CB_MASK] ^ mt_mix(cb[(i - 624) & CB_MASK], cb[(i - 623) & CB_MASK]);
            cb[i & CB_MASK] = v;
            cb[(i & CB_MASK) + CB_WORDS] = v;
          }
          lds_barrier();
        }
        G += 624;
      }
      uint32_t m = __builtin_amdgcn_readfirstlane(gp[pw]);
      const int base = kb & CB_MASK;
      for (int nleft = __builtin_popcount(m); nleft > 0; nleft -= JB) {
        int off[JB];
#pragma unroll
        for (int u = 0; u < JB; u++) {
          off[u] = u < nleft ? base + __builtin_ctz(m) : CB_ZERO;
          m &= m - 1u;
        }
        uint32_t v0[JB], v1[JB], v2[JB];
#pragma unroll
        for (int u = 0; u < JB; u++) {
          const uint32_t *q = cb + off[u] + w;
          v0[u] = q[0];
          v1[u] = q[JW];
          v2[u] = q[2 * JW];
        }
#pragma unroll
        for (int u = 0; u < JB; u++) {
          a0 ^= v0[u];
          a1 ^= v1[u];
          a2 ^= v2[u];
        }
      }
    }
    lds_barrier();
    if (t < JW) {
      cb[t] = a0;
      cb[t + JW] = a1;
      cb[t + 2 * JW] = a2;
    }
    lds_barrier();
  }
  uint32_t *st0 = cb, *st1 = cb + 624;
  uint32_t *out = job.out + job.start;
  const int64_t cnt = job.count;
  for (int64_t base = 0; base < cnt; base += 624) {
    mt_twist_block(st0, st1, [&](int k, uint32_t w) {
      if (base + k < cnt) out[base + k] = w;
    });
    uint32_t *tmp = st0; st0 = st1; st1 = tmp;
  }
}

__device__ __forceinline__ uint32_t interval_mask(uint32_t m) {
  m |= m >> 1; m |= m >> 2; m |= m >> 4; m |= m >> 8; m |= m >> 16;
  return m;
}

struct DecJob {
  const uint32_t *words;
  int64_t n_words;
  int64_t n;
  uint32_t *j;
  int64_t *status;
};

constexpr int DC_THREADS = 256;
constexpr int DC_WAVES = DC_THREADS / 64;
constexpr int DC_PER = 4;
constexpr int DC_CHUNK = DC_THREADS * DC_PER;

__global__ void __launch_bounds__(DC_THREADS) k_shuffle_decode2(const DecJob *jobs) {
  __shared__ int32_t wsum[DC_WAVES];
  __shared__ int32_t s_tot;
  const DecJob job = jobs[blockIdx.x];
  const int t = threadIdx.x, lane = t & 63, wave = t >> 6;
  if (t == 0 && job.n > 0) job.j[0] = 0;
  int64_t i0 = job.n - 1;
  int64_t base = 0;
  float ratio = 0.75f;
  uint4 nxt = make_uint4(0, 0, 0, 0);
  if (DC_PER * t + 3 < job.n_words) nxt = *(const uint4 *)(job.words + DC_PER * t);
  while (i0 >= 1 && base < job.n_words) {
    uint32_t w[DC_PER] = {nxt.x, nxt.y, nxt.z, nxt.w};
    bool valid[DC_PER];
#pragma unroll
    for (int e = 0; e < DC_PER; e++) valid[e] = base + DC_PER * t + e < job.n_words;
    {
      const int64_t nb = base + DC_CHUNK + DC_PER * t;
      if (nb + 3 < job.n_words) nxt = *(const uint4 *)(job.words + nb);
    }
    int32_t A = (int32_t)(ratio * (float)(DC_PER * t));
    int32_t cnt = 0;
    uint32_t v[DC_PER];
    bool acc[DC_PER];
    bool converged = false;
    for (int it = 0; it < 24; it++) {
      cnt = 0;
#pragma unroll
      for (int e = 0; e < DC_PER; e++) {
        const int64_t i = i0 - A - cnt;
        v[e] = (i >= 1) ? (w[e] & interval_mask((uint32_t)i)) : 0u;
        acc[e] = valid[e] && i >= 1 && v[e] <= (uint32_t)i;
        cnt += acc[e];
      }
      int32_t incl = cnt;
#pragma unroll
      for (int d = 1; d < 64; d <<= 1) {
        int32_t o = __shfl_up(incl, d, 64);
        if (lane >= d) incl += o;
      }
      if (lane == 63) wsum[wave] = incl;
      __syncthreads();
      int32_t pre = 0, tot = 0;
#pragma unroll
      for (int q = 0; q < DC_WAVES; q++) {
        const int32_t s = wsum[q];
        pre += q < wave ? s : 0;
        tot += s;
      }
      const int32_t A2 = pre + incl - cnt;
      const int same = __syncthreads_and(A2 == A);
      A = A2;
      if (t == 0) s_tot = tot;
      if (same) {
        converged = true;
        break;
      }
    }
    if (!converged) {
      __syncthreads();
      if (t == 0) {
        int64_t ii = i0;
        for (int64_t k = 0; k < DC_CHUNK && base + k < job.n_words && ii >= 1; k++) {
          const uint32_t vv = job.words[base + k] & interval_mask((uint32_t)ii);
          if (vv <= (uint32_t)ii) { job.j[ii] = vv; ii--; }
        }
        s_tot = (int32_t)(i0 - ii);
      }
      __syncthreads();
    } else {
      int32_t a = 0;
#pragma unroll
      for (int e = 0; e < DC_PER; e++) {
        if (acc[e]) job.j[i0 - A - a] = v[e];
        a += acc[e];
      }
    }
    __syncthreads();
    const int32_t tot = s_tot;
    i0 -= tot;
    base += DC_CHUNK;
    ratio = (float)tot / (float)DC_CHUNK;
    __syncthreads();
  }
  if (t == 0) *job.status = i0 < 1 ? 0 : i0;
}

struct ChunkJob {
  const uint32_t *words;
  int64_t n_words;
  int64_t base;
  uint32_t *j;
  int32_t tail;
  int32_t size;
};

constexpr int32_t DC_BIG = 1 << 30;

template <bool WRITE>
__device__ void decode_chunk(const ChunkJob *jobs, int32_t c, const int64_t *start, int32_t *count, int32_t *margin,
                             int32_t *wsum, int32_t *wlo, int32_t *whi, int32_t &s_tot) {
  const ChunkJob job = jobs[c];
  const int64_t i0 = start[c];
  const int t = threadIdx.x, lane = t & 63, wave = t >> 6;
  if (job.tail) {
    if (!WRITE && t == 0) {
      count[c] = 0;
      margin[2 * c] = -DC_BIG;
      margin[2 * c + 1] = DC_BIG;
    }
    return;
  }
  if (i0 < 1) {
    if (t == 0) {
      count[c] = 0;
      margin[2 * c] = -DC_BIG;
      margin[2 * c + 1] = 0;
    }
    return;
  }
  const int64_t base = job.base;
  uint32_t w[DC_PER];
  bool valid[DC_PER];
  if (base + DC_PER * t + 3 < job.n_words) {
    const uint4 q = *(const uint4 *)(job.words + base + DC_PER * t);
    w[0] = q.x; w[1] = q.y; w[2] = q.z; w[3] = q.w;
  } else {
#pragma unroll
    for (int e = 0; e < DC_PER; e++) w[e] = base + DC_PER * t + e < job.n_words ? job.words[base + DC_PER * t + e] : 0u;
  }
#pragma unroll
  for (int e = 0; e < DC_PER; e++) valid[e] = DC_PER * t + e < job.size && base + DC_PER * t + e < job.n_words;
  const uint32_t m0 = interval_mask((uint32_t)i0);
  int32_t A = (int32_t)((float)(i0 + 1) / ((float)m0 + 1.0f) * (float)(DC_PER * t));
  int32_t cnt = 0;
  uint32_t v[DC_PER];
  bool acc[DC_PER];
  bool converged = false;
  for (int it = 0; it < 24; it++) {
    cnt = 0;
#pragma unroll
    for (int e = 0; e < DC_PER; e++) {
      const int64_t i = i0 - A - cnt;
      v[e] = (i >= 1) ? (w[e] & interval_mask((uint32_t)i)) : 0u;
      acc[e] = valid[e] && i >= 1 && v[e] <= (uint32_t)i;
      cnt += acc[e];
    }
    int32_t incl = cnt;
#pragma unroll
    for (int d = 1; d < 64; d <<= 1) {
      int32_t o = __shfl_up(incl, d, 64);
      if (lane >= d) incl += o;
    }
    if (lane == 63) wsum[wave] = incl;
    __syncthreads();
    int32_t pre = 0, tot = 0;
#pragma unroll
    for (int q = 0; q < DC_WAVES; q++) {
      const int32_t s = wsum[q];
      pre += q < wave ? s : 0;
      tot += s;
    }
    const int32_t A2 = pre + incl - cnt;
    const int same = __syncthreads_and(A2 == A);
    A = A2;
    if (t == 0) s_tot = tot;
    if (same) {
      converged = true;
      break;
    }
  }
  if (!converged) {
    __syncthreads();
    if (t == 0) {
      int64_t ii = i0;
      int64_t lo = -DC_BIG, hi = DC_BIG;
      for (int64_t k = 0; k < job.size && base + k < job.n_words; k++) {
        if (ii < 1) { hi = 0; break; }
        const uint32_t m = interval_mask((uint32_t)ii);
        const uint32_t vv = job.words[base + k] & m;
        lo = max(lo, (int64_t)(m >> 1) + 1 - ii);
        hi = min(hi, (int64_t)m - ii);
        if (vv <= (uint32_t)ii) {
          lo = max(lo, (int64_t)vv - ii);
          if (WRITE) job.j[ii] = vv;
          ii--;
        } else {
          hi = min(hi, (int64_t)vv - ii - 1);
        }
      }
      count[c] = (int32_t)(i0 - ii);
      margin[2 * c] = (int32_t)lo;
      margin[2 * c + 1] = (int32_t)hi;
    }
    return;
  }
  int64_t lo = -DC_BIG, hi = DC_BIG;
  {
    int32_t a = 0;
#pragma unroll
    for (int e = 0; e < DC_PER; e++) {
      if (!valid[e]) continue;
      const int64_t i = i0 - A - a;
      if (i < 1) { hi = 0; continue; }
      const uint32_t m = interval_mask((uint32_t)i);
      lo = max(lo, (int64_t)(m >> 1) + 1 - i);
      hi = min(hi, (int64_t)m - i);
      if (acc[e]) lo = max(lo, (int64_t)v[e] - i); else hi = min(hi, (int64_t)v[e] - i - 1);
      if (WRITE && acc[e]) job.j[i] = v[e];
      a += acc[e];
    }
  }
  int32_t l32 = (int32_t)max(lo, (int64_t)-DC_BIG), h32 = (int32_t)min(hi, (int64_t)DC_BIG);
#pragma unroll
  for (int d = 32; d >= 1; d >>= 1) {
    l32 = max(l32, __shfl_xor(l32, d, 64));
    h32 = min(h32, __shfl_xor(h32, d, 64));
  }
  if (lane == 0) { wlo[wave] = l32; whi[wave] = h32; }
  __syncthreads();
  if (t == 0) {
    int32_t L = -DC_BIG, H = DC_BIG;
    for (int q = 0; q < DC_WAVES; q++) { L = max(L, wlo[q]); H = min(H, whi[q]); }
    count[c] = s_tot;
    margin[2 * c] = L;
    margin[2 * c + 1] = H;
  }
}

template <bool WRITE>
__global__ void __launch_bounds__(DC_THREADS) k_decode_chunks(const ChunkJob *jobs, const int32_t *todo,
                                                              const int32_t *n_todo, int32_t n_all,
                                                              const int64_t *start, int32_t *count,
                                                              int32_t *margin) {
  __shared__ int32_t wsum[DC_WAVES];
  __shared__ int32_t wlo[DC_WAVES], whi[DC_WAVES];
  __shared__ int32_t s_tot;
  const int32_t n = todo ? *n_todo : n_all;
  for (int32_t i = blockIdx.x; i < n; i += gridDim.x) {
    decode_chunk<WRITE>(jobs, todo ? todo[i] : i, start, count, margin, wsum, wlo, whi, s_tot);
    __syncthreads();
  }
}

constexpr int DR_THREADS = 256, DR_PER = 8, DR_TILE = DR_THREADS * DR_PER;
struct DecTile {
  int32_t unit, begin, end, first_tile;
};

__device__ __forceinline__ int64_t block_sum_dr(int64_t v, int64_t *wsum) {
  const int lane = threadIdx.x & 63, wave = threadIdx.x >> 6;
#pragma unroll
  for (int d = 32; d >= 1; d >>= 1) v += __shfl_xor(v, d, 64);
  if (lane == 0) wsum[wave] = v;
  __syncthreads();
  int64_t tot = 0;
#pragma unroll
  for (int q = 0; q < DR_THREADS / 64; q++) tot += wsum[q];
  return tot;
}

__global__ void __launch_bounds__(DR_THREADS) k_decode_resolve(const DecTile *tiles, const int64_t *n_draws,
                                                               const int32_t *count, const int32_t *margin,
                                                               int64_t *s0, int64_t *s1, int32_t *todo,
                                                               int32_t *n_todo, int32_t *n_next, int64_t *rem) {
  __shared__ int64_t wsum[DR_THREADS / 64];
  const int t = threadIdx.x, lane = t & 63, wave = t >> 6;
  const DecTile tl = tiles[blockIdx.x];
  if (blockIdx.x == 0 && t == 0) *n_next = 0;
  int64_t before = 0;
  for (int32_t k = tl.first_tile; k < (int32_t)blockIdx.x; k++) {
    const int32_t b = tiles[k].begin + t * DR_PER, e = tiles[k].end;
    int32_t cb[DR_PER];
#pragma unroll
    for (int q = 0; q < DR_PER; q++) cb[q] = b + q < e ? count[b + q] : 0;
#pragma unroll
    for (int q = 0; q < DR_PER; q++) before += cb[q];
  }
  const int64_t carry = n_draws[tl.unit] - 1 - block_sum_dr(before, wsum);
  __syncthreads();
  const int32_t c0 = tl.begin + t * DR_PER;
  int32_t cv[DR_PER];
  int64_t loc = 0;
#pragma unroll
  for (int k = 0; k < DR_PER; k++) {
    cv[k] = c0 + k < tl.end ? count[c0 + k] : 0;
    loc += cv[k];
  }
  int64_t incl = loc;
#pragma unroll
  for (int d = 1; d < 64; d <<= 1) {
    const int64_t o = __shfl_up(incl, d, 64);
    if (lane >= d) incl += o;
  }
  if (lane == 63) wsum[wave] = incl;
  __syncthreads();
  int64_t pre = 0;
#pragma unroll
  for (int q = 0; q < DR_THREADS / 64; q++) pre += q < wave ? wsum[q] : 0;
  int64_t s = carry - (pre + incl - loc);
  int64_t o0[DR_PER];
  int32_t mlo[DR_PER], mhi[DR_PER];
#pragma unroll
  for (int k = 0; k < DR_PER; k++) {
    const int32_t c = c0 + k < tl.end ? c0 + k : tl.begin;
    o0[k] = s0[c];
    mlo[k] = margin[2 * c];
    mhi[k] = margin[2 * c + 1];
  }
  uint32_t rq = 0;
#pragma unroll
  for (int k = 0; k < DR_PER; k++) {
    const int32_t c = c0 + k;
    if (c < tl.end) {
      const int64_t sv = s > 0 ? s : 0;
      s1[c] = sv;
      const int64_t d = sv - o0[k];
      if (d < mlo[k] || d > mhi[k]) {
        s0[c] = sv;
        rq |= 1u << k;
      }
    }
    s -= cv[k];
  }
  const int32_t nrq = __popc(rq);
  int32_t rincl = nrq;
#pragma unroll
  for (int d = 1; d < 64; d <<= 1) {
    const int32_t o = __shfl_up(rincl, d, 64);
    if (lane >= d) rincl += o;
  }
  const int32_t wtot = __shfl(rincl, 63, 64);
  if (wtot > 0) {
    int32_t q0 = 0;
    if (lane == 63) q0 = atomicAdd(n_todo, wtot);
    q0 = __shfl(q0, 63, 64) + rincl - nrq;
#pragma unroll
    for (int k = 0; k < DR_PER; k++)
      if (rq & (1u << k)) todo[q0++] = c0 + k;
  }
  if (t == DR_THREADS - 1 && (blockIdx.x + 1 == gridDim.x || tiles[blockIdx.x + 1].unit != tl.unit)) {
    const int64_t left = carry - (pre + incl);
    rem[tl.unit] = left < 1 ? 0 : left;
  }
}

struct TailJob {
  const uint32_t *words;
  int64_t n_words;
  int64_t base;
  const int64_t *start;
  uint32_t *j;
  int64_t *status;
};

constexpr int DT_PER = 4;
constexpr int DT_STEP = 64 * DT_PER;

__device__ __forceinline__ void tail_load(const TailJob &job, int64_t at, uint32_t (&w)[DT_PER]) {
  if (at + DT_PER <= job.n_words) {
    const uint4 q = *(const uint4 *)(job.words + at);
    w[0] = q.x; w[1] = q.y; w[2] = q.z; w[3] = q.w;
  } else {
#pragma unroll
    for (int e = 0; e < DT_PER; e++) w[e] = at + e < job.n_words ? job.words[at + e] : 0u;
  }
}

__device__ __forceinline__ bool tail_step(const TailJob &job, int64_t &i, int64_t pos, const uint32_t (&w)[DT_PER],
                                          int lane, uint64_t below) {
  const int64_t at = pos + DT_PER * lane;
  const uint32_t m0 = interval_mask((uint32_t)min(i, (int64_t)0xFFFFFFFF));
  int32_t A = (int32_t)((float)(i + 1) / ((float)m0 + 1.0f) * (float)(DT_PER * lane));
  uint32_t v[DT_PER];
  bool acc[DT_PER];
  for (int it = 0; it < 66; it++) {
    int32_t cnt = 0;
#pragma unroll
    for (int e = 0; e < DT_PER; e++) {
      const int64_t ii = i - A - cnt;
      v[e] = ii >= 1 ? (w[e] & interval_mask((uint32_t)ii)) : 0u;
      acc[e] = at + e < job.n_words && ii >= 1 && v[e] <= (uint32_t)ii;
      cnt += acc[e];
    }
    const uint64_t b0 = __ballot(cnt & 1), b1 = __ballot(cnt & 2), b2 = __ballot(cnt & 4);
    const int32_t A2 = (int32_t)(__popcll(b0 & below) + 2 * __popcll(b1 & below) + 4 * __popcll(b2 & below));
    if (__ballot(A2 != A) == 0) {
      int32_t a = 0;
#pragma unroll
      for (int e = 0; e < DT_PER; e++) {
        if (acc[e]) job.j[i - A - a] = v[e];
        a += acc[e];
      }
      i -= (int64_t)(__popcll(b0) + 2 * __popcll(b1) + 4 * __popcll(b2));
      return true;
    }
    A = A2;
  }
  return false;
}

constexpr int DT_RING = 4;

__global__ void __launch_bounds__(64) k_decode_tail(const TailJob *jobs) {
  const TailJob job = jobs[blockIdx.x];
  const int lane = threadIdx.x;
  const uint64_t below = lane ? (~0ull >> (64 - lane)) : 0ull;
  int64_t i = *job.start;
  int64_t pos = job.base;
  uint32_t w[DT_RING][DT_PER];
#pragma unroll
  for (int r = 0; r < DT_RING; r++) tail_load(job, pos + (int64_t)r * DT_STEP + DT_PER * lane, w[r]);
  bool ok = true;
  while (ok && i >= 1 && pos < job.n_words) {
#pragma unroll
    for (int r = 0; r < DT_RING; r++) {
      if (!(ok && i >= 1 && pos < job.n_words)) break;
      ok = tail_step(job, i, pos, w[r], lane, below);
      tail_load(job, pos + (int64_t)DT_RING * DT_STEP + DT_PER * lane, w[r]);
      pos += DT_STEP;
    }
  }
  if (lane == 0) *job.status = i < 1 ? 0 : i;
}

constexpr int SD_THREADS = 640;
constexpr int SD_WAVES = SD_THREADS / 64;

__global__ void __launch_bounds__(SD_THREADS) k_shuffle_decode(uint32_t seed, int64_t n, uint32_t *j) {
  __shared__ uint32_t st[2][624];
  __shared__ uint32_t words[624];
  __shared__ int32_t wave_cnt[SD_WAVES];
  __shared__ int64_t s_i0;
  const int t = threadIdx.x, lane = t & 63, wave = t >> 6;
  if (t == 0) {
    s_i0 = n - 1;
    if (n > 0) j[0] = 0;
  }
  mt_seed_lds(st[0], seed);
  int cur = 0;
  int64_t i0 = n - 1;
  while (i0 >= 1) {
    mt_twist_block(st[cur], st[cur ^ 1], [&](int k, uint32_t w) { words[k] = w; });
    cur ^= 1;
    const bool have = t < 624;
    const uint32_t w = have ? words[t] : 0u;
    int32_t A = t;
    bool acc = false;
    uint32_t v = 0;
    bool converged = false;
    for (int it = 0; it < 16; it++) {
      int64_t i = i0 - A;
      acc = have && i >= 1 && ((v = (w & interval_mask((uint32_t)i))) <= (uint32_t)i);
      uint64_t bal = __ballot(acc);
      if (lane == 0) wave_cnt[wave] = __popcll(bal);
      __syncthreads();
      int32_t pre = 0;
      for (int q = 0; q < wave; q++) pre += wave_cnt[q];
      int32_t A2 = pre + (int32_t)__popcll(bal & ((lane ? (~0ull >> (64 - lane)) : 0ull)));
      int same = __syncthreads_and(A2 == A);
      A = A2;
      if (same) { converged = true; break; }
    }
    if (!converged) {
      if (t == 0) {
        int64_t ii = i0;
        for (int k = 0; k < 624 && ii >= 1; k++) {
          uint32_t vv = words[k] & interval_mask((uint32_t)ii);
          if (vv <= (uint32_t)ii) { j[ii] = vv; ii--; }
        }
        s_i0 = ii;
      }
      __syncthreads();
      i0 = s_i0;
      __syncthreads();
      continue;
    }
    if (acc) j[i0 - A] = v;
    int32_t tot = 0;
    for (int q = 0; q < SD_WAVES; q++) tot += wave_cnt[q];
    i0 -= tot;
    __syncthreads();
  }
}

__global__ void __launch_bounds__(256) k_perm_heads(int64_t n, const uint32_t *K, const uint32_t *V, int32_t *nxt) {
  const int64_t k = (int64_t)blockIdx.x * blockDim.x + threadIdx.x;
  if (k >= n) return;
  const uint32_t b = K[k];
  if (k > 0 && K[k - 1] == b) return;
  int32_t s = (int32_t)V[k];
  if ((uint32_t)s == b) s = (k + 1 < n && K[k + 1] == b) ? (int32_t)V[k + 1] : -1;
  nxt[b] = s;
}

__global__ void __launch_bounds__(256) k_perm_chase(int64_t k0, int64_t n, const uint32_t *K, const uint32_t *V,
                                                    const int32_t *nxt, const int64_t *ts, int64_t *out) {
  const int64_t k = k0 + (int64_t)blockIdx.x * blockDim.x + threadIdx.x;
  if (k >= n) return;
  const uint32_t b = K[k], p = V[k];
  int64_t q = b;
  if (k + 1 < n && K[k + 1] == b) {
    int32_t c = (int32_t)V[k + 1], d;
    while ((d = nxt[c]) >= 0) c = d;
    q = c;
  }
  out[p] = ts[q];
}

constexpr int PK_UNITS = 512;
__global__ void __launch_bounds__(256) k_perm_keys(int64_t total, const uint32_t *jall, const int64_t *u_off,
                                                   const int64_t *u_n, int32_t n_units, uint32_t *keys,
                                                   int32_t *nxt) {
  __shared__ int64_t s_off[PK_UNITS], s_n[PK_UNITS];
  for (int i = threadIdx.x; i < n_units; i += 256) {
    s_off[i] = u_off[i];
    s_n[i] = u_n[i];
  }
  __syncthreads();
  const int64_t g = (int64_t)blockIdx.x * blockDim.x + threadIdx.x;
  if (g >= total) return;
  int lo = 0, hi = n_units - 1;
  while (lo < hi) {
    const int mid = (lo + hi + 1) >> 1;
    if (s_off[mid] <= g) lo = mid; else hi = mid - 1;
  }
  const int64_t k = g - s_off[lo];
  keys[g] = k < s_n[lo] ? (uint32_t)(s_off[lo] + jall[g]) : (uint32_t)g;
  nxt[g] = -1;
}

__device__ __forceinline__ double mt_double(const uint32_t *w, int64_t k) {
  int32_t a = (int32_t)(w[2 * k] >> 5), b = (int32_t)(w[2 * k + 1] >> 6);
  return (a * 67108864.0 + b) / 9007199254740992.0;
}

struct GeoFlags {
  int64_t *idx;
  uint32_t *count;
  uint32_t cap;
};

__device__ __forceinline__ int64_t geometric_draw(double U, double p, double log_q, GeoFlags fl, int64_t k) {
  if (p >= 0.333333333333333333333333) {
    double sum = p, prod = p, q = 1.0 - p;
    int64_t X = 1;
    while (U > sum) { prod *= q; sum += prod; X++; }
    return X;
  }
  double qv = log1p(-U) / log_q;
  double r = rint(qv);
  if (fabs(qv - r) <= 1e-12 * fmax(1.0, fabs(qv))) {
    uint32_t s = atomicAdd(fl.count, 1u);
    if (s < fl.cap) fl.idx[s] = k;
  }
  return (int64_t)ceil(qv);
}

struct LoadGeo {
  const uint32_t *w; double p, log_q; GeoFlags fl;
  __device__ int64_t operator()(int64_t k) const { return geometric_draw(mt_double(w, k), p, log_q, fl, k); }
};
struct LoadArr {
  const int64_t *a;
  __device__ int64_t operator()(int64_t k) const { return a[k]; }
};
__global__ void k_geo_array(int64_t n, const uint32_t *w, double p, double log_q, GeoFlags fl, int64_t *g) {
  int64_t k = (int64_t)blockIdx.x * blockDim.x + threadIdx.x;
  if (k < n) g[k] = geometric_draw(mt_double(w, k), p, log_q, fl, k);
}
struct StoreTs {
  int64_t *ts; int64_t add; NodeIdx ni;
  __device__ void operator()(int64_t k, int64_t incl, int64_t) const { ts[k] = ts_pack(ni, incl + add); }
};

constexpr int TLEN_PER = 8;
// ... 45 lines not shown
    k.x += 0x9E3779B9u;
    k.y += 0xBB67AE85u;
  }
  return c;
}
__global__ void k_philox_words(uint32_t *out, int64_t count, uint64_t key, uint32_t stream) {
  int64_t q = (int64_t)blockIdx.x * blockDim.x + threadIdx.x;
  if (q * 4 >= count) return;
  uint4 r = philox4x32(make_uint4((uint32_t)q, (uint32_t)(q >> 32), stream, 0x6d697479u),
                       make_uint2((uint32_t)key, (uint32_t)(key >> 32)));
  uint32_t v[4] = {r.x, r.y, r.z, r.w};
  for (int e = 0; e < 4; e++)
    if (q * 4 + e < count) out[q * 4 + e] = v[e];
}

int64_t shuffle_words_alloc(int64_t n) {
  if (n <= 1) return DC_CHUNK;
  double E = 0.0;
  auto H = [](double x) { return x < 20 ? 0.0 : std::log(x) + 0.5772156649015329 + 1.0 / (2 * x) - 1.0 / (12 * x * x); };
  for (int64_t a = 1; a <= n - 1; a *= 2) {
    int64_t b = std::min(2 * a - 1, n - 1);
    double M = (double)(2 * a);
    if (b < 64) {
      for (int64_t i = a; i <= b; i++) E += M / (double)(i + 1);
    } else {
      E += M * (H((double)(b + 1)) - H((double)a));
    }
  }
  double sd = 2.0 * std::sqrt((double)n);
  int64_t w = (int64_t)(E + 12.0 * sd) + 2 * DC_CHUNK;
  return ((w + DC_CHUNK - 1) / DC_CHUNK) * DC_CHUNK;
}

}

void HostMT::seed(uint32_t s) {
  key[0] = s;
  for (int i = 1; i < 624; i++) key[i] = 1812433253u * (key[i - 1] ^ (key[i - 1] >> 30)) + (uint32_t)i;
  pos = 624;
}
uint32_t HostMT::next() {
  if (pos == 624) {
    int i;
    uint32_t y;
    for (i = 0; i < 624 - 397; i++) {
      y = (key[i] & MT_UP) | (key[i + 1] & MT_LO);
      key[i] = key[i + 397] ^ (y >> 1) ^ ((y & 1u) ? MT_A : 0u);
    }
    for (; i < 623; i++) {
      y = (key[i] & MT_UP) | (key[i + 1] & MT_LO);
      key[i] = key[i + 397 - 624] ^ (y >> 1) ^ ((y & 1u) ? MT_A : 0u);
    }
    y = (key[623] & MT_UP) | (key[0] & MT_LO);
    key[623] = key[396] ^ (y >> 1) ^ ((y & 1u) ? MT_A : 0u);
    pos = 0;
  }
  uint32_t y = key[pos++];
  y ^= (y >> 11);
  y ^= (y << 7) & 0x9d2c5680u;
  y ^= (y << 15) & 0xefc60000u;
  y ^= (y >> 18);
  return y;
}
double HostMT::next_double() {
  int32_t a = (int32_t)(next() >> 5), b = (int32_t)(next() >> 6);
  return (a * 67108864.0 + b) / 9007199254740992.0;
}
uint64_t HostMT::interval(uint64_t max) {
  if (max == 0) return 0;
  uint64_t mask = max, v;
  mask |= mask >> 1; mask |= mask >> 2; mask |= mask >> 4; mask |= mask >> 8; mask |= mask >> 16; mask |= mask >> 32;
  if (max <= 0xffffffffull) {
    while ((v = (next() & mask)) > max) {}
  } else {
    while ((v = ((((uint64_t)next()) << 32 | next()) & mask)) > max) {}
  }
  return v;
}

namespace {

int32_t ensure_polys(mh_ctx *ctx, hipStream_t st, int64_t kmax, int64_t seg) {
  if (ctx->jump_k >= kmax + 1 && ctx->jump_seg == seg) return MH_OK;
  std::vector<uint32_t> polys((size_t)(kmax + 1) * 624);
  for (int64_t k = 0; k <= kmax; k++) jump::jump_poly_words((uint64_t)seg, k, polys.data() + k * 624);
  MH_TRY(ensure(ctx, ctx->jump_polys, 4 * polys.size()));
  HIPCHK(ctx, hipMemcpyAsync(ctx->jump_polys.p, polys.data(), 4 * polys.size(), hipMemcpyHostToDevice, st));
  SYNCCHK(ctx, hipStreamSynchronize(st));
  ctx->jump_k = kmax + 1;
  ctx->jump_seg = seg;
  return MH_OK;
}

__global__ void __launch_bounds__(256) k_mt_state(const uint32_t *key, int32_t pos, int64_t count, uint32_t *out) {
  __shared__ uint32_t st[2][624];
  for (int i = threadIdx.x; i < 624; i += 256) st[0][i] = key[i];
  lds_barrier();
  const int64_t lead = 624 - pos;
  for (int64_t i = threadIdx.x; i < lead && i < count; i += 256) out[i] = mt_temper(st[0][pos + i]);
  uint32_t *o = st[0], *nw = st[1];
  for (int64_t base = lead; base < count; base += 624) {
    mt_twist_block(o, nw, [&](int k, uint32_t w) {
      if (base + k < count) out[base + k] = w;
    });
    uint32_t *tmp = o; o = nw; nw = tmp;
  }
}

}

int32_t mt_stream_words(mh_ctx *ctx, hipStream_t st, uint32_t seed, int64_t first, int64_t count, DevBuf &out,
                        DevBuf &jobs_buf, int64_t *lead) {
  const int64_t SEG = seg_words();
  const int64_t k0 = first / SEG, k1 = (first + std::max<int64_t>(count, 1) - 1) / SEG;
  *lead = first - k0 * SEG;
  MH_TRY(ensure(ctx, out, 4 * (size_t)((k1 - k0 + 1) * SEG) + 64));
  std::vector<SegJob> jobs;
  for (int64_t k = k0; k <= k1; k++)
    jobs.push_back(SegJob{(uint32_t *)out.p, (k - k0) * SEG, std::min(SEG, first + count - k * SEG), seed, (int32_t)k});
  MH_TRY(ensure_polys(ctx, st, k1, SEG));
  MH_TRY(ensure(ctx, jobs_buf, sizeof(SegJob) * jobs.size() + 64));
  HIPCHK(ctx, hipMemcpyAsync(jobs_buf.p, jobs.data(), sizeof(SegJob) * jobs.size(), hipMemcpyHostToDevice, st));
  hipLaunchKernelGGL(k_mt_segments, dim3((unsigned)jobs.size()), dim3(256), 0, st, (const SegJob *)jobs_buf.p,
                     (const uint32_t *)ctx->jump_polys.p);
  HIPCHK(ctx, hipGetLastError());
  SYNCCHK(ctx, hipStreamSynchronize(st));
  return MH_OK;
}

int32_t mt_state_words(mh_ctx *ctx, hipStream_t st, const uint32_t *key624, int32_t pos, int64_t count, DevBuf &out,
                       DevBuf &key_buf) {
  if (pos < 0 || pos > 624) return arg_fail(ctx, MH_E_ARG, "MT19937 state position outside 0..624");
  MH_TRY(ensure(ctx, out, 4 * (size_t)count + 64));
  MH_TRY(ensure(ctx, key_buf, 4 * 624));
  HIPCHK(ctx, hipMemcpyAsync(key_buf.p, key624, 4 * 624, hipMemcpyHostToDevice, st));
  hipLaunchKernelGGL(k_mt_state, dim3(1), dim3(256), 0, st, (const uint32_t *)key_buf.p, pos, count,
                     (uint32_t *)out.p);
  HIPCHK(ctx, hipGetLastError());
  SYNCCHK(ctx, hipStreamSynchronize(st));
  return MH_OK;
}

namespace {

struct UnitPlan {
  NodeIdx ni;
  int64_t p_min, p_max, n, n_fo_words, n_shuf_words;
  uint32_t s_tloc, s_tlen, s_shuf, s_fo;
  int64_t w_tloc, w_tlen, w_fo, w_shuf;
  int64_t j_off;
  TplSet *out;
};

int32_t decode_parallel(mh_ctx *ctx, const std::vector<DecJob> &dec, int64_t *d_status, bool *done) {
  hipStream_t st = ctx->stream;
  *done = false;
  const int64_t div = 128;
  const int64_t minw = 64;
  std::vector<ChunkJob> cj;
  std::vector<int64_t> s0;
  std::vector<int32_t> first(dec.size() + 1, 0);
  for (size_t u = 0; u < dec.size(); u++) {
    first[u] = (int32_t)cj.size();
    double i = (double)(dec[u].n - 1);
    for (int64_t b = 0; b < dec[u].n_words;) {
      int64_t size = DC_CHUNK;
      while (size > minw && (double)size * (double)div > i) size >>= 1;
      cj.push_back(ChunkJob{dec[u].words, dec[u].n_words, b, dec[u].j, 0, (int32_t)size});
      s0.push_back(b == 0 ? dec[u].n - 1 : (i >= 1.0 ? (int64_t)llround(i) : 0));
      double rem = (double)size;
      while (rem > 0 && i >= 1.0) {
        uint32_t ii = (uint32_t)i, m = ii;
        m |= m >> 1; m |= m >> 2; m |= m >> 4; m |= m >> 8; m |= m >> 16;
        const double rate = (i + 1.0) / ((double)m + 1.0);
        const double lo = (double)((m >> 1) + 1);
        const double need = (i - lo + 1.0) / rate;
        if (need >= rem) { i -= rem * rate; rem = 0; }
        else { i = lo - 1.0; rem -= need; }
      }
      b += size;
    }
  }
  first[dec.size()] = (int32_t)cj.size();
  const int64_t C = (int64_t)cj.size();
  if (C == 0) {
    *done = true;
    return MH_OK;
  }
  const int32_t U = (int32_t)dec.size();
  const int64_t tail_at = (int64_t)1 << 15;
  std::vector<int32_t> tail_c(U, -1);
  for (int32_t u = 0; u < U; u++)
    for (int32_t c = first[u]; c < first[u + 1] && tail_at > 0; c++)
      if (s0[c] < tail_at) {
        tail_c[u] = c;
        for (int32_t k = c; k < first[u + 1]; k++) cj[k].tail = 1;
        break;
      }
  const int32_t tile_sz = DR_TILE;
  std::vector<DecTile> tiles;
  for (int32_t u = 0; u < U; u++) {
    const int32_t ft = (int32_t)tiles.size();
    for (int32_t b = first[u]; b < first[u + 1]; b += tile_sz)
      tiles.push_back(DecTile{u, b, std::min(b + tile_sz, first[u + 1]), ft});
  }
  const int32_t T = (int32_t)tiles.size();
  const size_t bytes = ((sizeof(ChunkJob) * C + 15) / 16) * 16 + 8 * C * 2 + 8 * U * 2 + sizeof(TailJob) * U +
                       sizeof(DecTile) * (T + 1) + 4 * C * 2 + 8 * C + 512;
  MH_TRY(ensure(ctx, ctx->dec_buf, bytes));
  char *p = (char *)ctx->dec_buf.p;
  ChunkJob *d_jobs = (ChunkJob *)p;
  int64_t *d_s0 = (int64_t *)(p + ((sizeof(ChunkJob) * C + 15) / 16) * 16);
  int64_t *d_s1 = d_s0 + C;
  int64_t *d_ndraw = d_s1 + C;
  int64_t *d_rem = d_ndraw + U;
  TailJob *d_tail = (TailJob *)(d_rem + U);
  DecTile *d_tiles = (DecTile *)(d_tail + U);
  int32_t *d_count = (int32_t *)(d_tiles + T + 1);
  int32_t *d_todo = d_count + C;
  int32_t *d_margin = d_todo + C;
  int32_t *d_ntodo = d_margin + 2 * C;
  std::vector<int64_t> ndraw(U);
  for (int32_t u = 0; u < U; u++) ndraw[u] = dec[u].n;
  std::vector<TailJob> tj;
  for (int32_t u = 0; u < U; u++)
    if (tail_c[u] >= 0 && dec[u].n > 0)
      tj.push_back(TailJob{dec[u].words, dec[u].n_words, cj[tail_c[u]].base, d_s1 + tail_c[u], dec[u].j, dec[u].status});
  HIPCHK(ctx, hipMemcpyAsync(d_jobs, cj.data(), sizeof(ChunkJob) * C, hipMemcpyHostToDevice, st));
  HIPCHK(ctx, hipMemcpyAsync(d_s0, s0.data(), 8 * C, hipMemcpyHostToDevice, st));
  HIPCHK(ctx, hipMemcpyAsync(d_tiles, tiles.data(), sizeof(DecTile) * T, hipMemcpyHostToDevice, st));
  HIPCHK(ctx, hipMemcpyAsync(d_ndraw, ndraw.data(), 8 * U, hipMemcpyHostToDevice, st));
  if (!tj.empty()) HIPCHK(ctx, hipMemcpyAsync(d_tail, tj.data(), sizeof(TailJob) * tj.size(), hipMemcpyHostToDevice, st));
  HIPCHK(ctx, hipMemsetAsync(d_ntodo, 0, 8, st));
  const unsigned grid = (unsigned)std::min<int64_t>(C, 4096);
  constexpr int MAX_PASSES = 64;
  const int PASS_BATCH = 24;
  hipLaunchKernelGGL(k_decode_chunks<false>, dim3(grid), dim3(DC_THREADS), 0, st, (const ChunkJob *)d_jobs,
                     (const int32_t *)nullptr, (const int32_t *)nullptr, (int32_t)C, (const int64_t *)d_s0, d_count,
                     d_margin);
  HIPCHK(ctx, hipGetLastError());
  bool conv = false;
  int passes = 1;
  while (passes < MAX_PASSES) {
    int32_t *cur = d_ntodo;
    for (int k = 0; k < PASS_BATCH; k++, passes++) {
      cur = d_ntodo + (passes & 1);
      int32_t *nxt = d_ntodo + ((passes + 1) & 1);
      const unsigned g = passes < 4 ? grid : std::min(grid, 1024u);
      hipLaunchKernelGGL(k_decode_resolve, dim3(T), dim3(DR_THREADS), 0, st, (const DecTile *)d_tiles,
                         (const int64_t *)d_ndraw, (const int32_t *)d_count, (const int32_t *)d_margin, d_s0, d_s1,
                         d_todo, cur, nxt, d_rem);
      hipLaunchKernelGGL(k_decode_chunks<false>, dim3(g), dim3(DC_THREADS), 0, st, (const ChunkJob *)d_jobs,
                         (const int32_t *)d_todo, (const int32_t *)cur, (int32_t)C, (const int64_t *)d_s0, d_count,
                         d_margin);
    }
    HIPCHK(ctx, hipGetLastError());
    int64_t *hs = pinned_small(ctx);
    if (!hs) return arg_fail(ctx, MH_E_OOM, "pinned host memory");
    HIPCHK(ctx, hipMemcpyAsync(hs + 32, cur, 4, hipMemcpyDeviceToHost, st));
    SYNCCHK(ctx, hipStreamSynchronize(st));
    const int32_t h_ntodo = (int32_t)(hs[32] & 0xffffffff);
    if (h_ntodo == 0) {
      conv = true;
      break;
    }
  }
  ctx->dec_passes = passes;
  if (!conv) return MH_OK;
  hipLaunchKernelGGL(k_decode_chunks<true>, dim3(grid), dim3(DC_THREADS), 0, st, (const ChunkJob *)d_jobs,
                     (const int32_t *)nullptr, (const int32_t *)nullptr, (int32_t)C, (const int64_t *)d_s1, d_count,
                     d_margin);
  HIPCHK(ctx, hipGetLastError());
  for (int32_t u = 0; u < U; u++)
    if (dec[u].n > 0 && tail_c[u] < 0) HIPCHK(ctx, hipMemcpyAsync(dec[u].status, d_rem + u, 8, hipMemcpyDeviceToDevice, st));
  if (!tj.empty()) {
    hipLaunchKernelGGL(k_decode_tail, dim3((unsigned)tj.size()), dim3(64), 0, st, (const TailJob *)d_tail);
    HIPCHK(ctx, hipGetLastError());
  }
  for (size_t u = 0; u < dec.size(); u++)
    if (dec[u].n > 0) HIPCHK(ctx, hipMemsetAsync(dec[u].j, 0, 4, st));
  SYNCCHK(ctx, hipStreamSynchronize(st));
  *done = true;
  return MH_OK;
}

template <class KIn>
static hipError_t perm_sort(void *tmp, size_t &tmp_bytes, KIn keys_in, uint32_t *keys_out, uint32_t *vals_out,
                            size_t n, unsigned end_bit, hipStream_t st) {
  return lsd_sort_pairs_iota(tmp, tmp_bytes, keys_in, keys_out, vals_out, (int64_t)n, end_bit, st);
}

struct BatchPerm {
  int64_t *ts, *tsh;
};

int32_t finish_unit(mh_ctx *ctx, UnitPlan &u, const uint32_t *words, const uint32_t *jarr, double p, int32_t rlen,
                    const double *d_cum, int32_t n_tlen, int32_t rng_mode, bool exact, int64_t *d_m,
                    uint32_t *d_flag, int lane = 0, int phase = 0, const BatchPerm *bp = nullptr) {
  hipStream_t st = lane == 0 ? ctx->stream : lane == 1 ? ctx->stream2 : ctx->xstream[lane - 2];
  ctx->stage_stream = lane ? st : nullptr;
  struct Restore {
    mh_ctx *c;
    ~Restore() { c->stage_stream = nullptr; }
  } restore{ctx};
  mh::DevBuf *S4 = lane == 0 ? ctx->s + 4 : lane == 1 ? ctx->lane2 : ctx->xlane[lane - 2];
  mh::DevBuf &perm_tmp = lane == 0 ? ctx->perm_tmp : S4[7];
  void *scan_partials = lane == 0 ? ctx->scan_partials.p : lane == 1 ? ctx->scan_partials2.p : ctx->xscan[lane - 2].p;
  const int64_t n = u.n;
  const uint32_t *w_tloc = words + u.w_tloc, *w_tlen = words + u.w_tlen, *w_fo = words + u.w_fo;
  int64_t *ts = bp ? bp->ts + u.j_off : (int64_t *)S4[0].p;
  int64_t *ts_shuf = (int64_t *)S4[1].p, *te = (int64_t *)S4[2].p;
  uint32_t *sk = (uint32_t *)S4[4].p, *sv = (uint32_t *)S4[5].p;
  int32_t *nxt = (int32_t *)S4[6].p;
  const bool permute = rng_mode == MH_RNG_MITTY && n > 1 && !bp;
  uint8_t *keep = (uint8_t *)S4[3].p;
  int64_t *flag_idx = (int64_t *)ctx->s[11].p;
  int64_t *tot = (int64_t *)((char *)ctx->d_small.p + 128 + 64 * lane);
  const double log_q = std::log(1.0 - p);
  GeoFlags fl{flag_idx, d_flag, 1024};

  if (phase != 2) {
    stage_begin(ctx, "sample_geometric_scan");
    if (!exact) {
      HIPCHK(ctx, device_scan_sum<int64_t>(st, n, LoadGeo{w_tloc, p, log_q, fl}, StoreTs{ts, u.p_min + 1, u.ni},
                                           scan_partials, tot));
    } else {
      int64_t *g = (int64_t *)ctx->s[12].p;
      uint32_t nflag = 0;
      HIPCHK(ctx, hipMemsetAsync(d_flag, 0, 4, st));
      hipLaunchKernelGGL(k_geo_array, dim3(grid_for(n, 256, INT32_MAX)), dim3(256), 0, st, n, w_tloc, p, log_q, fl, g);
      HIPCHK(ctx, hipMemcpyAsync(&nflag, d_flag, 4, hipMemcpyDeviceToHost, st));
      SYNCCHK(ctx, hipStreamSynchronize(st));
      auto host_geo = [&](const uint32_t *ww) {
        double U = (((int32_t)(ww[0] >> 5)) * 67108864.0 + ((int32_t)(ww[1] >> 6))) / 9007199254740992.0;
        return (int64_t)std::ceil(std::log1p(-U) / std::log(1.0 - p));
      };
      if (ctx->force_geo && p < 0.333333333333333333333333) {
        std::vector<uint32_t> hw(2 * (size_t)n);
        std::vector<int64_t> hg((size_t)n);
        HIPCHK(ctx, hipMemcpy(hw.data(), w_tloc, 8 * (size_t)n, hipMemcpyDeviceToHost));
        for (int64_t k = 0; k < n; k++) hg[k] = host_geo(hw.data() + 2 * k);
        HIPCHK(ctx, hipMemcpy(g, hg.data(), 8 * (size_t)n, hipMemcpyHostToDevice));
      } else {
        if (nflag > 1024) return arg_fail(ctx, MH_E_ARG, "too many near-integer geometric quotients");
        std::vector<int64_t> idx(nflag);
        if (nflag) HIPCHK(ctx, hipMemcpy(idx.data(), flag_idx, 8 * nflag, hipMemcpyDeviceToHost));
        for (int64_t k : idx) {
          uint32_t ww[2];
          HIPCHK(ctx, hipMemcpy(ww, w_tloc + 2 * k, 8, hipMemcpyDeviceToHost));
          int64_t gv = host_geo(ww);
          HIPCHK(ctx, hipMemcpy(g + k, &gv, 8, hipMemcpyHostToDevice));
        }
      }
      HIPCHK(ctx, hipMemsetAsync(d_flag, 0, 4, st));
      HIPCHK(ctx, device_scan<int64_t>(st, n, LoadArr{g}, StoreTs{ts, u.p_min + 1, u.ni}, OpSum{}, (int64_t)0,
                                       (int64_t *)scan_partials, tot));
    }
    stage_end(ctx);

    if (permute) {
      stage_begin(ctx, "sample_permutation");
      unsigned end_bit = 1;
      while (end_bit < 32 && ((int64_t)1 << end_bit) < n) end_bit++;
      size_t tmp = 0;
      HIPCHK(ctx, perm_sort(nullptr, tmp, jarr, sk, sv, (size_t)n, end_bit, st));
      MH_TRY(ensure(ctx, perm_tmp, tmp + 256));
      HIPCHK(ctx, perm_sort(perm_tmp.p, tmp, jarr, sk, sv, (size_t)n, end_bit, st));
      HIPCHK(ctx, hipMemsetAsync(nxt, 0xff, 4 * (size_t)n, st));
      hipLaunchKernelGGL(k_perm_heads, dim3(grid_for(n, 256, INT32_MAX)), dim3(256), 0, st, n, (const uint32_t *)sk,
                         (const uint32_t *)sv, nxt);
      HIPCHK(ctx, hipGetLastError());
      stage_end(ctx);
    }
  }
  if (phase == 1) return MH_OK;

  const int64_t *ts_use = bp && rng_mode == MH_RNG_MITTY && n > 1 ? bp->tsh + u.j_off : ts;
  if (permute) {
    stage_begin(ctx, "sample_permutation");
    hipLaunchKernelGGL(k_perm_chase, dim3(grid_for(n, 256, INT32_MAX)), dim3(256), 0, st, (int64_t)0, n,
                       (const uint32_t *)sk, (const uint32_t *)sv, (const int32_t *)nxt, (const int64_t *)ts, ts_shuf);
    HIPCHK(ctx, hipGetLastError());
    stage_end(ctx);
    ts_use = ts_shuf;
  }

  stage_begin(ctx, "sample_tlen_compact");
  hipLaunchKernelGGL(k_tlen, dim3(grid_for((n + TLEN_PER - 1) / TLEN_PER, 256, INT32_MAX)), dim3(256), 8 * n_tlen, st,
                     n, w_tlen, d_cum, n_tlen,
                     (int64_t)rlen, u.p_max, ts_use, te, keep);
  HIPCHK(ctx, hipGetLastError());
  HIPCHK(ctx, device_scan_sum<int64_t>(st, n, LoadKeep{keep},
                                       StoreCompact{keep, ts_use, te, (int64_t *)u.out->pos0.p,
                                                    (int64_t *)u.out->pos1.p, (int64_t)rlen, w_fo,
                                                    (int8_t *)u.out->fo0.p,
                                                    u.out->has_n0 ? (int32_t *)u.out->n0.p : nullptr},
                                       scan_partials, d_m));
  stage_end(ctx);
  return MH_OK;
}

}

struct SampleState {
  std::vector<UnitPlan> plan;
  int32_t n_units = 0, rng_mode = 0, rlen = 0, n_tlen = 0, n_lanes = 1;
  bool two_lanes = false, batch = false;
  double p = 0;
  int64_t j_total = 0, nn = 0;
  uint32_t *words = nullptr, *jall = nullptr;
  double *d_cum = nullptr;
  int64_t *d_m = nullptr, *d_status = nullptr;
  uint32_t *d_flags = nullptr;
  BatchPerm bp{nullptr, nullptr};
  std::vector<hipEvent_t> ev;
  int32_t n_pending = 0;
  ~SampleState() {
    for (hipEvent_t e : ev)
      if (e) (void)hipEventDestroy(e);
  }
};

static void plan_unit_words(UnitPlan &q, int64_t p_min, int64_t p_max, uint64_t seed, double p, int32_t rng_mode,
                            int64_t &words_total) {
  q.p_min = p_min;
  q.p_max = p_max;
  q.n = (int64_t)((double)(q.p_max - q.p_min) * p * 1.2);
  if (q.n < 0) q.n = 0;
  HostMT sr;
  sr.seed((uint32_t)seed);
  q.s_tloc = (uint32_t)sr.interval(0xfffffffeull);
  q.s_tlen = (uint32_t)sr.interval(0xfffffffeull);
  q.s_shuf = (uint32_t)sr.interval(0xfffffffeull);
  q.s_fo = (uint32_t)sr.interval(0xfffffffeull);
  q.n_fo_words = (q.n + 3) / 4 + 1;
  q.n_shuf_words = rng_mode == MH_RNG_MITTY ? shuffle_words_alloc(q.n) : 0;
  auto take = [&](int64_t cnt) {
    int64_t at = words_total;
    words_total = (words_total + cnt + 4 + 3) & ~(int64_t)3;
    return at;
  };
  q.w_tloc = take(2 * q.n);
  q.w_tlen = take(2 * q.n);
  q.w_fo = take(q.n_fo_words);
  q.w_shuf = take(q.n_shuf_words);
}

static void unit_seg_jobs(uint32_t *words, const UnitPlan &q, std::vector<SegJob> &jobs, int64_t &kmax) {
  const int64_t SEG_WORDS = seg_words();
  auto add_stream = [&](uint32_t *out, int64_t count, uint32_t seed) {
    for (int64_t k = 0; k * SEG_WORDS < count; k++) {
      int64_t s0 = k * SEG_WORDS;
      jobs.push_back(SegJob{out, s0, std::min(SEG_WORDS, count - s0), seed, (int32_t)k});
      kmax = std::max(kmax, k);
    }
  };
  add_stream(words + q.w_tloc, 2 * q.n, q.s_tloc);
  add_stream(words + q.w_tlen, 2 * q.n, q.s_tlen);
  add_stream(words + q.w_fo, q.n_fo_words, q.s_fo);
  add_stream(words + q.w_shuf, q.n_shuf_words, q.s_shuf);
}

static int32_t sample_head(mh_ctx *ctx, SampleState &S, int32_t n_units, const int32_t *tpl_ids, const int64_t *p_min,
                           const int64_t *p_max, const uint64_t *seeds, double p, int32_t rlen, const double *cum_tlen,
                           int32_t n_tlen, int32_t rng_mode, const NodeIdx *nidx) {
  for (int32_t u = 0; u < n_units; u++)
    if (seeds[u] > 0xffffffffull)
      return arg_fail(ctx, MH_E_SEED, "Seed value " + std::to_string(seeds[u]) + " is out of range 0 - 4294967295");
  if (n_tlen <= 0 || n_tlen > 8192) return arg_fail(ctx, MH_E_ARG, "cum_tlen must have 1..8192 entries");
  if (rng_mode != MH_RNG_MITTY && rng_mode != MH_RNG_PHILOX) return arg_fail(ctx, MH_E_ARG, "unknown rng_mode");
  MH_TRY(tpl_resolve_all(ctx));
  hipStream_t st = ctx->stream;

  std::vector<UnitPlan> plan(n_units);
  int64_t words_total = 0, j_total = 0, n_max = 1;
  for (int32_t u = 0; u < n_units; u++) {
    UnitPlan &q = plan[u];
    plan_unit_words(q, p_min[u], p_max[u], seeds[u], p, rng_mode, words_total);
    if (q.n > ((int64_t)1 << 30) - 8) return arg_fail(ctx, MH_E_ARG, "region too large for one work unit");
    q.j_off = j_total; j_total += q.n + 4;
    n_max = std::max(n_max, q.n);
    TplSet &ts = ctx->tsets[tpl_ids[u]];
    MH_TRY(wait_unused(ctx, ts.used, ts.used_set));
    MH_TRY(ensure(ctx, ts.fo0, q.n + 16));
    MH_TRY(ensure(ctx, ts.pos0, 8 * (q.n + 16)));
    MH_TRY(ensure(ctx, ts.pos1, 8 * (q.n + 16)));
    q.ni = nidx ? nidx[u] : NodeIdx{};
    ts.n_draws = q.n;
    ts.has_n0 = q.ni.nd != nullptr;
    if (ts.has_n0) MH_TRY(ensure(ctx, ts.n0, 4 * (q.n + 16)));
    ts.valid = false;
    q.out = &ts;
  }
  const int64_t nn = n_max + 1;
  ctx->batch_left = 0;
  for (const UnitPlan &q : plan) ctx->batch_left += q.n;
  PrefetchedWords &pw = ctx->pf_words;
  const bool have_words = rng_mode == MH_RNG_MITTY && pw.valid && pw.p == p && pw.seeds.size() == (size_t)n_units &&
                          std::equal(pw.seeds.begin(), pw.seeds.end(), seeds) &&
                          std::equal(pw.p_min.begin(), pw.p_min.end(), p_min) &&
                          std::equal(pw.p_max.begin(), pw.p_max.end(), p_max) && pw.words_total == words_total;
  pw.valid = false;
  if (have_words) std::swap(ctx->s[0], pw.buf);
  MH_TRY(ensure(ctx, ctx->s[0], 4 * (size_t)words_total + 64));
  MH_TRY(ensure(ctx, ctx->s[3], 4 * (size_t)j_total + 64));
  MH_TRY(ensure(ctx, ctx->s[4], 8 * nn));
  MH_TRY(ensure(ctx, ctx->s[5], 8 * nn));
  MH_TRY(ensure(ctx, ctx->s[6], 8 * nn));
  MH_TRY(ensure(ctx, ctx->s[7], nn));
  MH_TRY(ensure(ctx, ctx->s[8], 4 * (nn + 1)));
  MH_TRY(ensure(ctx, ctx->s[9], 4 * (nn + 1)));
  MH_TRY(ensure(ctx, ctx->s[10], 4 * nn));
  MH_TRY(ensure(ctx, ctx->s[11], 8 * 1024));
  int n_lanes = std::max(1, std::min(2, (int)n_units));
  const bool two_lanes = n_lanes > 1;
  for (int l = 2; l < n_lanes; l++)
    if (!ctx->xstream[l - 2]) {
      int lo = 0, hi = 0;
      (void)hipDeviceGetStreamPriorityRange(&lo, &hi);
      HIPCHK(ctx, hipStreamCreateWithPriority(&ctx->xstream[l - 2], hipStreamNonBlocking, hi));
      HIPCHK(ctx, hipEventCreateWithFlags(&ctx->ev_xjoin[l - 2], hipEventDisableTiming));
    }
  for (int l = 1; l < n_lanes; l++) {
    mh::DevBuf *L = l == 1 ? ctx->lane2 : ctx->xlane[l - 2];
    MH_TRY(ensure(ctx, L[0], 8 * nn));
    MH_TRY(ensure(ctx, L[1], 8 * nn));
    MH_TRY(ensure(ctx, L[2], 8 * nn));
    MH_TRY(ensure(ctx, L[3], nn));
    MH_TRY(ensure(ctx, L[4], 4 * (nn + 1)));
    MH_TRY(ensure(ctx, L[5], 4 * (nn + 1)));
    MH_TRY(ensure(ctx, L[6], 4 * nn));
    MH_TRY(ensure(ctx, l == 1 ? ctx->scan_partials2 : ctx->xscan[l - 2],
                  std::max<size_t>(16 * scan_partials_count(nn + 1) + 64, scan_lb_scratch_bytes<int64_t>(nn + 1))));
  }
  MH_TRY(ensure(ctx, ctx->s[13], 8 * (size_t)n_tlen + 64));
  MH_TRY(ensure(ctx, ctx->s[1], 64 * (size_t)n_units + 64));
  MH_TRY(ensure(ctx, ctx->d_small, 8192 + 256));
  MH_TRY(ensure(ctx, ctx->scan_partials, std::max<size_t>(16 * scan_partials_count(nn + 1) + 64,
                                                           scan_lb_scratch_bytes<int64_t>(nn + 1))));
  uint32_t *words = (uint32_t *)ctx->s[0].p, *jall = (uint32_t *)ctx->s[3].p;
  double *d_cum = (double *)ctx->s[13].p;
  int64_t *d_m = (int64_t *)ctx->s[1].p;
  int64_t *d_status = d_m + n_units;
  uint32_t *d_flags = (uint32_t *)(d_status + n_units);
  HIPCHK(ctx, hipMemsetAsync(ctx->s[1].p, 0, 64 * (size_t)n_units + 64, st));
  HIPCHK(ctx, hipMemcpyAsync(d_cum, cum_tlen, 8 * n_tlen, hipMemcpyHostToDevice, st));

  stage_begin(ctx, "sample");
  if (rng_mode == MH_RNG_MITTY) {
    std::vector<SegJob> jobs;
    std::vector<DecJob> dec;
    int64_t kmax = 0;
    const int64_t SEG_WORDS = seg_words();
    for (int32_t u = 0; u < n_units; u++) {
      UnitPlan &q = plan[u];
      if (q.n == 0) continue;
      unit_seg_jobs(words, q, jobs, kmax);
      dec.push_back(DecJob{words + q.w_shuf, q.n_shuf_words, q.n, jall + q.j_off, d_status + u});
    }
    if (!jobs.empty()) {
      MH_TRY(ensure_polys(ctx, st, kmax, SEG_WORDS));
      MH_TRY(ensure(ctx, ctx->s[2], sizeof(SegJob) * jobs.size() + sizeof(DecJob) * dec.size() + 64));
      SegJob *d_jobs = (SegJob *)ctx->s[2].p;
      DecJob *d_dec = (DecJob *)((char *)ctx->s[2].p + ((sizeof(SegJob) * jobs.size() + 15) / 16) * 16);
      HIPCHK(ctx, hipMemcpyAsync(d_jobs, jobs.data(), sizeof(SegJob) * jobs.size(), hipMemcpyHostToDevice, st));
      HIPCHK(ctx, hipMemcpyAsync(d_dec, dec.data(), sizeof(DecJob) * dec.size(), hipMemcpyHostToDevice, st));
      if (!have_words) {
        stage_begin(ctx, "sample_mt_segments");
        hipLaunchKernelGGL(k_mt_segments, dim3((unsigned)jobs.size()), dim3(256), 0, st, (const SegJob *)d_jobs,
                           (const uint32_t *)ctx->jump_polys.p);
        HIPCHK(ctx, hipGetLastError());
        stage_end(ctx);
      }
      stage_begin(ctx, "sample_shuffle_decode");
      bool done = false;
      if (!ctx->decode_sequential) MH_TRY(decode_parallel(ctx, dec, d_status, &done));
      if (!done) {
        hipLaunchKernelGGL(k_shuffle_decode2, dim3((unsigned)dec.size()), dim3(DC_THREADS), 0, st,
                           (const DecJob *)d_dec);
        HIPCHK(ctx, hipGetLastError());
      }
      stage_end(ctx);
      SYNCCHK(ctx, hipStreamSynchronize(st));
    }
  } else {
    for (int32_t u = 0; u < n_units; u++) {
      UnitPlan &q = plan[u];
      if (q.n == 0) continue;
      uint64_t key = ((uint64_t)q.s_tloc << 32) | q.s_tlen;
      hipLaunchKernelGGL(k_philox_words, dim3(grid_for((2 * q.n + 3) / 4, 256, INT32_MAX)), dim3(256), 0, st,
                         words + q.w_tloc, 2 * q.n, key, 1u);
      hipLaunchKernelGGL(k_philox_words, dim3(grid_for((2 * q.n + 3) / 4, 256, INT32_MAX)), dim3(256), 0, st,
                         words + q.w_tlen, 2 * q.n, key, 2u);
      hipLaunchKernelGGL(k_philox_words, dim3(grid_for((q.n_fo_words + 3) / 4, 256, INT32_MAX)), dim3(256), 0, st,
                         words + q.w_fo, q.n_fo_words, key, 3u);
      HIPCHK(ctx, hipGetLastError());
    }
  }

  if (two_lanes) {
    HIPCHK(ctx, hipEventRecord(ctx->ev_fork, st));
    HIPCHK(ctx, hipStreamWaitEvent(ctx->stream2, ctx->ev_fork, 0));
    for (int l = 2; l < n_lanes; l++) HIPCHK(ctx, hipStreamWaitEvent(ctx->xstream[l - 2], ctx->ev_fork, 0));
  }
  const bool batch = rng_mode == MH_RNG_MITTY && j_total < ((int64_t)1 << 30) && n_units <= PK_UNITS;
  if (batch) {
    MH_TRY(ensure(ctx, ctx->pb[0], 8 * (size_t)j_total + 64));
    MH_TRY(ensure(ctx, ctx->pb[1], 8 * (size_t)j_total + 64));
    for (int b = 2; b < 6; b++) MH_TRY(ensure(ctx, ctx->pb[b], 4 * (size_t)j_total + 64));
    BatchPerm bp{(int64_t *)ctx->pb[0].p, (int64_t *)ctx->pb[1].p};
    for (int32_t u = 0, k = 0; u < n_units; u++) {
      if (plan[u].n == 0) continue;
      MH_TRY(finish_unit(ctx, plan[u], words, jall + plan[u].j_off, p, rlen, d_cum, n_tlen, rng_mode, false, d_m + u,
                         d_flags + u, k++ % n_lanes, 1, &bp));
    }
    if (two_lanes) {
      HIPCHK(ctx, hipEventRecord(ctx->ev_join, ctx->stream2));
      HIPCHK(ctx, hipStreamWaitEvent(st, ctx->ev_join, 0));
      for (int l = 2; l < n_lanes; l++) {
        HIPCHK(ctx, hipEventRecord(ctx->ev_xjoin[l - 2], ctx->xstream[l - 2]));
        HIPCHK(ctx, hipStreamWaitEvent(st, ctx->ev_xjoin[l - 2], 0));
      }
    }
    stage_begin(ctx, "sample_permutation");
    std::vector<int64_t> uo(n_units), un(n_units);
    for (int32_t u = 0; u < n_units; u++) {
      uo[u] = plan[u].j_off;
      un[u] = plan[u].n;
    }
    int64_t *d_uo = (int64_t *)ctx->s[12].p;
    MH_TRY(ensure(ctx, ctx->s[12], 16 * (size_t)n_units + 64));
    d_uo = (int64_t *)ctx->s[12].p;
    HIPCHK(ctx, hipMemcpyAsync(d_uo, uo.data(), 8 * n_units, hipMemcpyHostToDevice, st));
    HIPCHK(ctx, hipMemcpyAsync(d_uo + n_units, un.data(), 8 * n_units, hipMemcpyHostToDevice, st));
    uint32_t *gk = (uint32_t *)ctx->pb[2].p, *sk = (uint32_t *)ctx->pb[3].p, *sv = (uint32_t *)ctx->pb[4].p;
    int32_t *nxt = (int32_t *)ctx->pb[5].p;
    hipLaunchKernelGGL(k_perm_keys, dim3(grid_for(j_total, 256, INT32_MAX)), dim3(256), 0, st, j_total,
                       (const uint32_t *)jall, (const int64_t *)d_uo, (const int64_t *)(d_uo + n_units), n_units, gk,
                       nxt);
    HIPCHK(ctx, hipGetLastError());
    unsigned end_bit = 1;
    while (end_bit < 32 && ((int64_t)1 << end_bit) < j_total) end_bit++;
    size_t tmp = 0;
    HIPCHK(ctx, perm_sort(nullptr, tmp, gk, sk, sv, (size_t)j_total, end_bit, st));
    MH_TRY(ensure(ctx, ctx->pb_tmp, tmp + 256));
    HIPCHK(ctx, perm_sort(ctx->pb_tmp.p, tmp, gk, sk, sv, (size_t)j_total, end_bit, st));
    hipLaunchKernelGGL(k_perm_heads, dim3(grid_for(j_total, 256, INT32_MAX)), dim3(256), 0, st, j_total,
                       (const uint32_t *)sk, (const uint32_t *)sv, nxt);
    HIPCHK(ctx, hipGetLastError());
    stage_end(ctx);
    S.bp = bp;
  } else {
    for (int32_t u = 0, k = 0; u < n_units; u++) {
      if (plan[u].n == 0) continue;
      MH_TRY(finish_unit(ctx, plan[u], words, jall + plan[u].j_off, p, rlen, d_cum, n_tlen, rng_mode, false, d_m + u,
                         d_flags + u, k++ % n_lanes));
    }
  }
  S.plan = std::move(plan);
  S.n_units = n_units;
  S.rng_mode = rng_mode;
  S.rlen = rlen;
  S.n_tlen = n_tlen;
  S.n_lanes = n_lanes;
  S.two_lanes = two_lanes;
  S.batch = batch;
  S.p = p;
  S.j_total = j_total;
  S.nn = nn;
  S.words = words;
  S.jall = jall;
  S.d_cum = d_cum;
  S.d_m = d_m;
  S.d_status = d_status;
  S.d_flags = d_flags;
  return MH_OK;
}

static int32_t sample_tail(mh_ctx *ctx, SampleState &S, int64_t *out_n) {
  hipStream_t st = ctx->stream;
  std::vector<UnitPlan> &plan = S.plan;
  const int32_t n_units = S.n_units, rng_mode = S.rng_mode, rlen = S.rlen, n_tlen = S.n_tlen, n_lanes = S.n_lanes;
  const bool two_lanes = S.two_lanes;
  const double p = S.p;
  const int64_t j_total = S.j_total, nn = S.nn;
  uint32_t *words = S.words, *jall = S.jall;
  double *d_cum = S.d_cum;
  int64_t *d_m = S.d_m, *d_status = S.d_status;
  uint32_t *d_flags = S.d_flags;
  if (S.batch) {
    const BatchPerm &bp = S.bp;
    const uint32_t *sk = (const uint32_t *)ctx->pb[3].p, *sv = (const uint32_t *)ctx->pb[4].p;
    const int32_t *nxt = (const int32_t *)ctx->pb[5].p;
    stage_begin(ctx, "sample_permutation");
    hipLaunchKernelGGL(k_perm_chase, dim3(grid_for(j_total, 256, INT32_MAX)), dim3(256), 0, st, (int64_t)0, j_total,
                       sk, sv, nxt, (const int64_t *)bp.ts, bp.tsh);
    HIPCHK(ctx, hipGetLastError());
    stage_end(ctx);
    if (two_lanes) {
      HIPCHK(ctx, hipEventRecord(ctx->ev_fork, st));
      HIPCHK(ctx, hipStreamWaitEvent(ctx->stream2, ctx->ev_fork, 0));
      for (int l = 2; l < n_lanes; l++) HIPCHK(ctx, hipStreamWaitEvent(ctx->xstream[l - 2], ctx->ev_fork, 0));
    }
    for (int32_t u = 0, k = 0; u < n_units; u++) {
      if (plan[u].n == 0) continue;
      MH_TRY(finish_unit(ctx, plan[u], words, jall + plan[u].j_off, p, rlen, d_cum, n_tlen, rng_mode, false, d_m + u,
                         d_flags + u, k++ % n_lanes, 2, &bp));
    }
  }
  if (two_lanes) {
    HIPCHK(ctx, hipEventRecord(ctx->ev_join, ctx->stream2));
    HIPCHK(ctx, hipStreamWaitEvent(st, ctx->ev_join, 0));
    for (int l = 2; l < n_lanes; l++) {
      HIPCHK(ctx, hipEventRecord(ctx->ev_xjoin[l - 2], ctx->xstream[l - 2]));
      HIPCHK(ctx, hipStreamWaitEvent(st, ctx->ev_xjoin[l - 2], 0));
    }
  }
  std::vector<int64_t> hm(n_units), hstat(n_units);
  std::vector<uint32_t> hflag(n_units);
  int64_t *hs = pinned_small(ctx);
  const size_t rb_bytes = 20 * (size_t)n_units;
  if (hs && rb_bytes <= 3072) {
    HIPCHK(ctx, hipMemcpyAsync(hs + 64, d_m, rb_bytes, hipMemcpyDeviceToHost, st));
    SYNCCHK(ctx, hipStreamSynchronize(st));
    std::memcpy(hm.data(), hs + 64, 8 * n_units);
    std::memcpy(hstat.data(), hs + 64 + n_units, 8 * n_units);
    std::memcpy(hflag.data(), hs + 64 + 2 * n_units, 4 * n_units);
  } else {
    HIPCHK(ctx, hipMemcpyAsync(hm.data(), d_m, 8 * n_units, hipMemcpyDeviceToHost, st));
    HIPCHK(ctx, hipMemcpyAsync(hstat.data(), d_status, 8 * n_units, hipMemcpyDeviceToHost, st));
    HIPCHK(ctx, hipMemcpyAsync(hflag.data(), d_flags, 4 * n_units, hipMemcpyDeviceToHost, st));
    SYNCCHK(ctx, hipStreamSynchronize(st));
  }

// ... 2 lines not shown
    if (q.n == 0) continue;
    if (ctx->force_fixup) hstat[u] = 1;
    if (ctx->force_geo) hflag[u] = 1;
    if (hstat[u] == 0 && hflag[u] == 0) continue;
    if (rng_mode == MH_RNG_MITTY && hstat[u] != 0) {
      hipLaunchKernelGGL(k_shuffle_decode, dim3(1), dim3(SD_THREADS), 0, st, q.s_shuf, q.n, jall + q.j_off);
      HIPCHK(ctx, hipGetLastError());
    }
    MH_TRY(ensure(ctx, ctx->s[12], 8 * (size_t)nn));
    HIPCHK(ctx, hipMemsetAsync(d_flags + u, 0, 4, st));
    MH_TRY(finish_unit(ctx, q, words, jall + q.j_off, p, rlen, d_cum, n_tlen, rng_mode, hflag[u] != 0, d_m + u,
                       d_flags + u));
    HIPCHK(ctx, hipMemcpyAsync(&hm[u], d_m + u, 8, hipMemcpyDeviceToHost, st));
    SYNCCHK(ctx, hipStreamSynchronize(st));
    ctx->fixups++;
  }
  stage_end(ctx);
  for (int32_t u = 0; u < n_units; u++) {
    TplSet &ts = *plan[u].out;
    ts.n = plan[u].n == 0 ? 0 : hm[u];
    ts.rlen = rlen;
    ts.valid = true;
    if (out_n) out_n[u] = ts.n;
  }
  return MH_OK;
}

__global__ void k_unit_result(const int64_t *m, const int64_t *status, const uint32_t *flag, int64_t *out) {
  if (threadIdx.x == 0) {
    out[0] = *m;
    out[1] = *status;
    out[2] = (int64_t)*flag;
  }
}

static int32_t sample_tail_async(mh_ctx *ctx, const std::shared_ptr<SampleState> &Sp) {
  SampleState &S = *Sp;
  std::vector<UnitPlan> &plan = S.plan;
  const int32_t n_units = S.n_units;
  hipStream_t st = ctx->stream, l1 = ctx->stream2;
  const BatchPerm &bp = S.bp;
  const uint32_t *sk = (const uint32_t *)ctx->pb[3].p, *sv = (const uint32_t *)ctx->pb[4].p;
  const int32_t *nxt = (const int32_t *)ctx->pb[5].p;
  HIPCHK(ctx, hipEventRecord(ctx->ev_fork, st));
  HIPCHK(ctx, hipStreamWaitEvent(l1, ctx->ev_fork, 0));
  S.ev.assign(n_units, nullptr);
  for (int32_t u = 0; u < n_units; u++) {
    UnitPlan &q = plan[u];
    TplSet &ts = *q.out;
    if (q.n == 0) {
      ts.n = 0;
      ts.rlen = S.rlen;
      ts.valid = true;
      continue;
    }
    ctx->stage_stream = l1;
    stage_begin(ctx, "sample_permutation");
    const int64_t k0 = q.j_off, k1 = q.j_off + q.n + 4;
    hipLaunchKernelGGL(k_perm_chase, dim3(grid_for(k1 - k0, 256, INT32_MAX)), dim3(256), 0, l1, k0, k1, sk, sv, nxt,
                       (const int64_t *)bp.ts, bp.tsh);
    stage_end(ctx);
    ctx->stage_stream = nullptr;
    HIPCHK(ctx, hipGetLastError());
    MH_TRY(finish_unit(ctx, q, S.words, S.jall + q.j_off, S.p, S.rlen, S.d_cum, S.n_tlen, S.rng_mode, false,
                       S.d_m + u, S.d_flags + u, 1, 2, &bp));
    hipLaunchKernelGGL(k_unit_result, dim3(1), dim3(64), 0, l1, (const int64_t *)(S.d_m + u),
                       (const int64_t *)(S.d_status + u), (const uint32_t *)(S.d_flags + u), ctx->d_units + 4 * u);
    HIPCHK(ctx, hipGetLastError());
    HIPCHK(ctx, hipEventCreateWithFlags(&S.ev[u], hipEventDisableTiming));
    HIPCHK(ctx, hipEventRecord(S.ev[u], l1));
    ts.pend = u;
    S.n_pending++;
  }
  stage_end(ctx);
  if (S.n_pending) ctx->tail_state = Sp;
  return MH_OK;
}

int32_t tpl_resolve(mh_ctx *ctx, TplSet &ts) {
  if (ts.pend < 0) return MH_OK;
  const int32_t u = ts.pend;
  ts.pend = -1;
  auto Sp = std::static_pointer_cast<SampleState>(ctx->tail_state);
  if (!Sp || u >= Sp->n_units || Sp->plan[u].out != &ts)
    return arg_fail(ctx, MH_E_STATE, "template set of a lost sampling batch");
  SampleState &S = *Sp;
  UnitPlan &q = S.plan[u];
  hipStream_t st = ctx->stream;
  SYNCCHK(ctx, hipEventSynchronize(S.ev[u]));
  const volatile int64_t *r = ctx->h_units + 4 * u;
  int64_t m = r[0];
  const int64_t status = ctx->force_fixup ? 1 : r[1];
  const uint32_t flag = ctx->force_geo ? 1u : (uint32_t)r[2];
  HIPCHK(ctx, hipStreamWaitEvent(st, S.ev[u], 0));
  if (status != 0 || flag != 0) {
    if (S.rng_mode == MH_RNG_MITTY && status != 0) {
      hipLaunchKernelGGL(k_shuffle_decode, dim3(1), dim3(SD_THREADS), 0, st, q.s_shuf, q.n, S.jall + q.j_off);
      HIPCHK(ctx, hipGetLastError());
    }
    MH_TRY(ensure(ctx, ctx->s[12], 8 * (size_t)S.nn));
    HIPCHK(ctx, hipMemsetAsync(S.d_flags + u, 0, 4, st));
    MH_TRY(finish_unit(ctx, q, S.words, S.jall + q.j_off, S.p, S.rlen, S.d_cum, S.n_tlen, S.rng_mode, flag != 0,
                       S.d_m + u, S.d_flags + u));
    HIPCHK(ctx, hipMemcpyAsync(&m, S.d_m + u, 8, hipMemcpyDeviceToHost, st));
    SYNCCHK(ctx, hipStreamSynchronize(st));
    ctx->fixups++;
  }
  ts.n = m;
  ts.rlen = S.rlen;
  ts.valid = true;
  if (--S.n_pending == 0) ctx->tail_state.reset();
  return MH_OK;
}

int32_t tpl_resolve_all(mh_ctx *ctx) {
  auto Sp = std::static_pointer_cast<SampleState>(ctx->tail_state);
  if (!Sp) return MH_OK;
  for (UnitPlan &q : Sp->plan)
    if (q.out && q.out->pend >= 0) MH_TRY(tpl_resolve(ctx, *q.out));
  return MH_OK;
}

int32_t prefetch_words(mh_ctx *ctx, hipStream_t st, int32_t n_units, const int64_t *p_min, const int64_t *p_max,
                       const uint64_t *seeds, double p) {
  PrefetchedWords &pw = ctx->pf_words;
  pw.valid = false;
  std::vector<UnitPlan> plan(n_units);
  int64_t words_total = 0;
  for (int32_t u = 0; u < n_units; u++) {
    plan_unit_words(plan[u], p_min[u], p_max[u], seeds[u], p, MH_RNG_MITTY, words_total);
    if (plan[u].n > ((int64_t)1 << 30) - 8) return MH_OK;
  }
  MH_TRY(ensure(ctx, pw.buf, 4 * (size_t)words_total + 64));
  std::vector<SegJob> jobs;
  int64_t kmax = 0;
  for (const UnitPlan &q : plan)
    if (q.n > 0) unit_seg_jobs((uint32_t *)pw.buf.p, q, jobs, kmax);
  if (jobs.empty() || ctx->jump_k < kmax + 1 || ctx->jump_seg != seg_words()) return MH_OK;
  MH_TRY(ensure(ctx, pw.jobs, sizeof(SegJob) * jobs.size() + 64));
  HIPCHK(ctx, hipMemcpyAsync(pw.jobs.p, jobs.data(), sizeof(SegJob) * jobs.size(), hipMemcpyHostToDevice, st));
  hipLaunchKernelGGL(k_mt_segments, dim3((unsigned)jobs.size()), dim3(256), 0, st, (const SegJob *)pw.jobs.p,
                     (const uint32_t *)ctx->jump_polys.p);
  HIPCHK(ctx, hipGetLastError());
  SYNCCHK(ctx, hipStreamSynchronize(st));
  pw.p = p;
  pw.seeds.assign(seeds, seeds + n_units);
  pw.p_min.assign(p_min, p_min + n_units);
  pw.p_max.assign(p_max, p_max + n_units);
  pw.words_total = words_total;
  pw.valid = true;
  return MH_OK;
}

int32_t sample_units_async(mh_ctx *ctx, int32_t n_units, const int32_t *tpl_ids, const int64_t *p_min,
                           const int64_t *p_max, const uint64_t *seeds, double p, int32_t rlen, const double *cum_tlen,
                           int32_t n_tlen, int32_t rng_mode, const NodeIdx *nidx) {
  if (!ctx->h_units) {
    if (hipHostMalloc((void **)&ctx->h_units, 32 * (size_t)PK_UNITS, hipHostMallocMapped | hipHostMallocCoherent) !=
        hipSuccess) {
      ctx->h_units = nullptr;
      return arg_fail(ctx, MH_E_OOM, "pinned host memory");
    }
    void *d = nullptr;
    HIPCHK(ctx, hipHostGetDevicePointer(&d, ctx->h_units, 0));
    ctx->d_units = (int64_t *)d;
  }
  auto S = std::make_shared<SampleState>();
  MH_TRY(sample_head(ctx, *S, n_units, tpl_ids, p_min, p_max, seeds, p, rlen, cum_tlen, n_tlen, rng_mode, nidx));
  if (!S->batch || !S->two_lanes) return sample_tail(ctx, *S, nullptr);
  return sample_tail_async(ctx, S);
}

int32_t sample_units(mh_ctx *ctx, int32_t n_units, const int32_t *tpl_ids, const int64_t *p_min, const int64_t *p_max,
                     const uint64_t *seeds, double p, int32_t rlen, const double *cum_tlen, int32_t n_tlen,
                     int32_t rng_mode, int64_t *out_n, const NodeIdx *nidx) {
  SampleState S;
  MH_TRY(sample_head(ctx, S, n_units, tpl_ids, p_min, p_max, seeds, p, rlen, cum_tlen, n_tlen, rng_mode, nidx));
  return sample_tail(ctx, S, out_n);
}

}
```

Before: 1.713 billion.

## Replace host-polled decode convergence loop with fixed passes plus on-device finish kernel

The parallel shuffle decode used to loop global count passes, copying the todo count to the host and synchronising after each pass to test convergence. Now it runs a fixed small number of global passes with no host polling. A new per-unit k_decode_finish kernel then serially scans chunk counts and recounts bad chunks inside a block, and a single k_decode_write kernel fuses the write pass, the tail decode and the j[0] reset. This removes per-pass host round trips and several small launches and memcopies, at the cost of more serialized per-unit work on device, and falls back to the sequential decoder when a unit does not converge. A decode self-test entry point and a tail-safe word loader are also added.

```diff
diff --git a/include/mitty_hip.h b/include/mitty_hip.h
--- a/include/mitty_hip.h
+++ b/include/mitty_hip.h
@@ -35,6 +35,9 @@
                          int64_t *incl, int64_t *excl, int64_t *total, int64_t *info);
 int32_t mh_selftest_sort(mh_ctx *ctx, const uint32_t *keys, int64_t n, int32_t end_bit, uint32_t *keys_out,
                          uint32_t *vals_out);
+int32_t mh_selftest_decode(mh_ctx *ctx, int32_t n_units, const uint32_t *shuffle_seeds, const int64_t *n_draws,
+                           int32_t global_passes, int32_t recount_cap, const int64_t *words_cap, uint32_t *j_out,
+                           int64_t *info);
 
 int32_t mh_read_model_params(int64_t mean_rlen, double coverage, double *p, int64_t *passes);
 int32_t mh_work_units(uint64_t seed, const int32_t *ploidy, int64_t n_regions, int64_t passes,
diff --git a/mitty_amd/_native.py b/mitty_amd/_native.py
--- a/mitty_amd/_native.py
+++ b/mitty_amd/_native.py
@@ -12,7 +12,7 @@
 MH_RNG_MITTY, MH_RNG_PHILOX = 0, 1
 
 EXPORTS = ['mh_version', 'mh_device_count', 'mh_create', 'mh_destroy', 'mh_last_error', 'mh_sync',
-           'mh_selftest_scan_fault', 'mh_selftest_scan', 'mh_selftest_sort', 'mh_selftest_bgzf',
+           'mh_selftest_scan_fault', 'mh_selftest_scan', 'mh_selftest_sort', 'mh_selftest_decode', 'mh_selftest_bgzf',
            'mh_read_model_params', 'mh_work_units', 'mh_upload_contig', 'mh_release_contig', 'mh_build_haplotype', 'mh_upload_variants', 'mh_build_haplotype_vset', 'mh_build_haplotypes_vset', 'mh_prefetch_haplotypes_vset', 'mh_release_variants', 'mh_get_nodes', 'mh_get_haplotype_aux',
            'mh_release_haplotype', 'mh_expand_variant', 'mh_sample_templates', 'mh_sample_templates_span', 'mh_set_templates',
            'mh_get_templates', 'mh_templates_export', 'mh_templates_import', 'mh_emit_reads', 'mh_emit_prepare', 'mh_emit_reads_async', 'mh_emit_collect', 'mh_output_size', 'mh_output_fetch', 'mh_output_reset', 'mh_host_alloc', 'mh_host_free', 'mh_device_cache_trim', 'mh_device_live_bytes',
@@ -75,6 +75,7 @@
   _sig(L, 'mh_selftest_scan_fault', [c_vp])
   _sig(L, 'mh_selftest_scan', [c_vp, c_i32, c_i32, c_vp, c_i64, c_i32, c_vp, c_vp, c_vp, c_vp])
   _sig(L, 'mh_selftest_sort', [c_vp, c_vp, c_i64, c_i32, c_vp, c_vp])
+  _sig(L, 'mh_selftest_decode', [c_vp, c_i32, c_vp, c_vp, c_i32, c_i32, c_vp, c_vp, c_vp])
   _sig(L, 'mh_selftest_bgzf', [c_vp, c_vp, c_i64, c_i32, c_vp, c_i64, P_i64])
   _sig(L, 'mh_read_model_params', [c_i64, c_dbl, ctypes.POINTER(c_dbl), P_i64])
   _sig(L, 'mh_work_units', [c_u64, c_vp, c_i64, c_i64, c_vp, c_vp, c_vp, P_i64])
@@ -1183,6 +1184,22 @@
     self._chk(self._L.mh_selftest_sort(self._h, k.ctypes.data, k.size, int(end_bit), ko.ctypes.data, vo.ctypes.data))
     return ko, vo
 
+  def selftest_decode(self, shuffle_seeds, n_draws, global_passes=-1, recount_cap=-1, words_cap=None):
+    import numpy as np
+    s = np.ascontiguousarray(shuffle_seeds, dtype=np.uint32)
+    n = np.ascontiguousarray(n_draws, dtype=np.int64)
+    assert s.ndim == 1 and s.shape == n.shape
+    cap = np.full(n.size, -1, np.int64) if words_cap is None else np.ascontiguousarray(words_cap, dtype=np.int64)
+    assert cap.shape == n.shape
+    j = np.empty(int(n.sum()), np.uint32)
+    info = np.zeros(34 + 2 * n.size, np.int64)
+    self._chk(self._L.mh_selftest_decode(self._h, n.size, s.ctypes.data, n.ctypes.data, int(global_passes),
+                                         int(recount_cap), cap.ctypes.data, j.ctypes.data, info.ctypes.data))
+    ends = np.cumsum(n)
+    return ([j[e - k:e] for e, k in zip(ends, n)],
+            {'fallback': bool(info[0]), 'global_passes': int(info[1]), 'queue': [int(q) for q in info[2:34] if q >= 0],
+             'recounts': info[34::2].copy(), 'status': info[35::2].copy()})
+
   def selftest_scan(self, kind, x, repeat=1):
     x = np.ascontiguousarray(x, dtype=np.int64)
     if x.ndim not in (1, 2):
diff --git a/mitty_amd/csrc/mh_api.hip b/mitty_amd/csrc/mh_api.hip
--- a/mitty_amd/csrc/mh_api.hip
+++ b/mitty_amd/csrc/mh_api.hip
@@ -583,6 +583,13 @@
   }();
   release(b);
   return rc;
+}
+
+int32_t mh_selftest_decode(mh_ctx *ctx, int32_t n_units, const uint32_t *shuffle_seeds, const int64_t *n_draws,
+                           int32_t global_passes, int32_t recount_cap, const int64_t *words_cap, uint32_t *j_out,
+                           int64_t *info) {
+  CTX_GUARD(ctx);
+  return selftest_decode(ctx, n_units, shuffle_seeds, n_draws, global_passes, recount_cap, words_cap, j_out, info);
 }
 
 int32_t mh_selftest_scan(mh_ctx *ctx, int32_t kind, int32_t fields, const int64_t *in, int64_t n, int32_t repeat,
diff --git a/mitty_amd/csrc/mh_internal.h b/mitty_amd/csrc/mh_internal.h
--- a/mitty_amd/csrc/mh_internal.h
+++ b/mitty_amd/csrc/mh_internal.h
@@ -296,6 +296,8 @@
   mh::DevBuf nrun_tmp;
   mh::DevBuf dec_buf;
   int64_t dec_passes = 0;
+  std::vector<int32_t> dec_queue;
+  std::vector<int32_t> dec_recounts;
 
   mh::DevBuf s[16];
   mh::DevBuf scan_partials;
@@ -447,6 +449,9 @@
 int32_t sample_units(mh_ctx *ctx, int32_t n_units, const int32_t *tpl_ids, const int64_t *p_min, const int64_t *p_max,
                      const uint64_t *seeds, double p, int32_t rlen, const double *cum_tlen, int32_t n_tlen,
                      int32_t rng_mode, int64_t *out_n, const NodeIdx *nidx = nullptr);
+int32_t selftest_decode(mh_ctx *ctx, int32_t n_units, const uint32_t *shuffle_seeds, const int64_t *n_draws,
+                        int32_t global_passes, int32_t recount_cap, const int64_t *words_cap, uint32_t *j_out,
+                        int64_t *info);
 int32_t sample_units_async(mh_ctx *ctx, int32_t n_units, const int32_t *tpl_ids, const int64_t *p_min,
                            const int64_t *p_max, const uint64_t *seeds, double p, int32_t rlen, const double *cum_tlen,
                            int32_t n_tlen, int32_t rng_mode, const NodeIdx *nidx = nullptr);
diff --git a/mitty_amd/csrc/mh_sample.hip b/mitty_amd/csrc/mh_sample.hip
--- a/mitty_amd/csrc/mh_sample.hip
+++ b/mitty_amd/csrc/mh_sample.hip
@@ -190,17 +190,21 @@
   int64_t i0 = job.n - 1;
   int64_t base = 0;
   float ratio = 0.75f;
-  uint4 nxt = make_uint4(0, 0, 0, 0);
-  if (DC_PER * t + 3 < job.n_words) nxt = *(const uint4 *)(job.words + DC_PER * t);
+  auto load4 = [&](int64_t at) {
+    if (at + 3 < job.n_words) return *(const uint4 *)(job.words + at);
+    uint4 q = make_uint4(0, 0, 0, 0);
+    if (at < job.n_words) q.x = job.words[at];
+    if (at + 1 < job.n_words) q.y = job.words[at + 1];
+    if (at + 2 < job.n_words) q.z = job.words[at + 2];
+    return q;
+  };
+  uint4 nxt = load4(DC_PER * t);
   while (i0 >= 1 && base < job.n_words) {
     uint32_t w[DC_PER] = {nxt.x, nxt.y, nxt.z, nxt.w};
     bool valid[DC_PER];
 #pragma unroll
     for (int e = 0; e < DC_PER; e++) valid[e] = base + DC_PER * t + e < job.n_words;
-    {
-      const int64_t nb = base + DC_CHUNK + DC_PER * t;
-      if (nb + 3 < job.n_words) nxt = *(const uint4 *)(job.words + nb);
-    }
+    nxt = load4(base + DC_CHUNK + DC_PER * t);
     int32_t A = (int32_t)(ratio * (float)(DC_PER * t));
     int32_t cnt = 0;
     uint32_t v[DC_PER];
@@ -280,10 +284,9 @@
 constexpr int32_t DC_BIG = 1 << 30;
 
 template <bool WRITE>
-__device__ void decode_chunk(const ChunkJob *jobs, int32_t c, const int64_t *start, int32_t *count, int32_t *margin,
+__device__ void decode_chunk(const ChunkJob *jobs, int32_t c, const int64_t i0, int32_t *count, int32_t *margin,
                              int32_t *wsum, int32_t *wlo, int32_t *whi, int32_t &s_tot) {
   const ChunkJob job = jobs[c];
-  const int64_t i0 = start[c];
   const int t = threadIdx.x, lane = t & 63, wave = t >> 6;
   if (job.tail) {
     if (!WRITE && t == 0) {
@@ -410,17 +413,18 @@
   }
 }
 
-template <bool WRITE>
 __global__ void __launch_bounds__(DC_THREADS) k_decode_chunks(const ChunkJob *jobs, const int32_t *todo,
                                                               const int32_t *n_todo, int32_t n_all,
                                                               const int64_t *start, int32_t *count,
-                                                              int32_t *margin) {
+                                                              int32_t *margin, int32_t *qlen) {
   __shared__ int32_t wsum[DC_WAVES];
   __shared__ int32_t wlo[DC_WAVES], whi[DC_WAVES];
   __shared__ int32_t s_tot;
   const int32_t n = todo ? *n_todo : n_all;
+  if (qlen && blockIdx.x == 0 && threadIdx.x == 0) *qlen = n;
   for (int32_t i = blockIdx.x; i < n; i += gridDim.x) {
-    decode_chunk<WRITE>(jobs, todo ? todo[i] : i, start, count, margin, wsum, wlo, whi, s_tot);
+    const int32_t c = todo ? todo[i] : i;
+    decode_chunk<false>(jobs, c, start[c], count, margin, wsum, wlo, whi, s_tot);
     __syncthreads();
   }
 }
@@ -584,9 +588,7 @@
 
 constexpr int DT_RING = 4;
 
-__global__ void __launch_bounds__(64) k_decode_tail(const TailJob *jobs) {
-  const TailJob job = jobs[blockIdx.x];
-  const int lane = threadIdx.x;
+__device__ void decode_tail(const TailJob &job, int lane) {
   const uint64_t below = lane ? (~0ull >> (64 - lane)) : 0ull;
   int64_t i = *job.start;
   int64_t pos = job.base;
@@ -604,6 +606,233 @@
     }
   }
   if (lane == 0) *job.status = i < 1 ? 0 : i;
+}
+
+struct DecUnit {
+  const uint32_t *words;
+  int64_t n_words;
+  int64_t n;
+  int64_t tail_base;
+  uint32_t *j;
+  int64_t *status;
+  int32_t begin, bulk_end;
+  int32_t tail_c;
+  int32_t pad;
+};
+
+constexpr int DF_THREADS = 1024;
+constexpr int DF_WAVES = DF_THREADS / 64;
+constexpr int DF_PER = DC_CHUNK / 64;
+
+struct ChunkCount {
+  int32_t count, lo, hi;
+};
+
+__device__ ChunkCount decode_chunk_wave(const ChunkJob &job, const int64_t i0, const int lane) {
+  if (i0 < 1) return ChunkCount{0, -DC_BIG, 0};
+  const int per = job.size >> 6;
+  const int64_t at = job.base + (int64_t)per * lane;
+  uint32_t w[DF_PER];
+  if ((per & 3) == 0 && at + per <= job.n_words) {
+#pragma unroll
+    for (int q = 0; q < DF_PER / 4; q++) {
+      uint4 x = make_uint4(0, 0, 0, 0);
+      if (4 * q < per) x = *(const uint4 *)(job.words + at + 4 * q);
+      w[4 * q] = x.x; w[4 * q + 1] = x.y; w[4 * q + 2] = x.z; w[4 * q + 3] = x.w;
+    }
+  } else {
+#pragma unroll
+    for (int e = 0; e < DF_PER; e++) w[e] = (e < per && at + e < job.n_words) ? job.words[at + e] : 0u;
+  }
+  uint32_t validm = 0;
+#pragma unroll
+  for (int e = 0; e < DF_PER; e++) validm |= (uint32_t)(e < per && at + e < job.n_words) << e;
+  const int32_t i32 = (int32_t)i0;
+  const uint32_t m0 = 0xffffffffu >> __clz(i32);
+  int32_t A = (int32_t)((float)(i32 + 1) / ((float)m0 + 1.0f) * (float)(per * lane));
+  uint32_t accm = 0;
+  int32_t tot = 0;
+  bool converged = false;
+  for (int it = 0; it < 66; it++) {
+    int32_t cnt = 0;
+    accm = 0;
+    const int32_t ib = i32 - A;
+#pragma unroll
+    for (int e = 0; e < DF_PER; e++) {
+      const int32_t i = ib - cnt;
+      const uint32_t v = w[e] & (0xffffffffu >> __clz(max(i, 1)));
+      const uint32_t a = ((validm >> e) & 1u) && i >= 1 && v <= (uint32_t)i;
+      accm |= a << e;
+      cnt += (int32_t)a;
+    }
+    int32_t incl = cnt;
+#pragma unroll
+    for (int d = 1; d < 64; d <<= 1) {
+      const int32_t o = __shfl_up(incl, d, 64);
+      if (lane >= d) incl += o;
+    }
+    const int32_t A2 = incl - cnt;
+    const bool same = __ballot(A2 != A) == 0;
+    A = A2;
+    tot = __shfl(incl, 63, 64);
+    if (same) {
+      converged = true;
+      break;
+    }
+  }
+  if (!converged) return ChunkCount{-1, 0, 0};
+  int32_t l32 = -DC_BIG, h32 = DC_BIG;
+  {
+    int32_t a = 0;
+#pragma unroll
+    for (int e = 0; e < DF_PER; e++) {
+      if (!((validm >> e) & 1u)) continue;
+      const int32_t i = i32 - A - a;
+      if (i < 1) { h32 = 0; continue; }
+      const uint32_t m = 0xffffffffu >> __clz(i);
+      const int32_t v = (int32_t)(w[e] & m);
+      l32 = max(l32, (int32_t)(m >> 1) + 1 - i);
+      h32 = min(h32, (int32_t)m - i);
+      const bool acc = (accm >> e) & 1u;
+      if (acc) l32 = max(l32, v - i); else h32 = min(h32, v - i - 1);
+      a += acc;
+    }
+  }
+#pragma unroll
+  for (int d = 32; d >= 1; d >>= 1) {
+    l32 = max(l32, __shfl_xor(l32, d, 64));
+    h32 = min(h32, __shfl_xor(h32, d, 64));
+  }
+  return ChunkCount{tot, l32, h32};
+}
+
+__global__ void __launch_bounds__(DF_THREADS) k_decode_finish(const DecUnit *units, const ChunkJob *jobs,
+                                                              int32_t *count, int32_t *margin, int64_t *s0,
+                                                              int64_t *s1, int64_t *rem, int32_t recount_cap,
+                                                              int32_t *notconv, int32_t *recounts) {
+  __shared__ int32_t wsum[DF_WAVES];
+  __shared__ int32_t wbad[DF_WAVES];
+  __shared__ int32_t lst[DF_WAVES];
+  __shared__ int64_t lst_s[DF_WAVES];
+  __shared__ int32_t res[DF_WAVES][3];
+  const DecUnit un = units[blockIdx.x];
+  const int t = threadIdx.x, lane = t & 63, wave = t >> 6;
+  const uint64_t below = lane ? (~0ull >> (64 - lane)) : 0ull;
+  int64_t run = un.n - 1;
+  int32_t nrec = 0;
+  bool fail = false;
+  if (recount_cap < 0) recount_cap = 4 * (un.bulk_end - un.begin) + 64;
+  for (int32_t c = un.begin; c < un.bulk_end && !fail; c += DF_THREADS) {
+    const int32_t k = c + t;
+    const bool in = k < un.bulk_end;
+    int32_t cnt = in ? count[k] : 0;
+    int64_t o0 = in ? s0[k] : 0;
+    int32_t mlo = in ? margin[2 * k] : 0, mhi = in ? margin[2 * k + 1] : 0;
+    int64_t sv = 0;
+    int32_t tot = 0;
+    for (int round = 0; round <= DF_THREADS; round++) {
+      int32_t incl = cnt;
+#pragma unroll
+      for (int d = 1; d < 64; d <<= 1) {
+        const int32_t o = __shfl_up(incl, d, 64);
+        if (lane >= d) incl += o;
+      }
+      if (lane == 63) wsum[wave] = incl;
+      __syncthreads();
+      int32_t pre = 0;
+      tot = 0;
+#pragma unroll
+      for (int q = 0; q < DF_WAVES; q++) {
+        const int32_t s = wsum[q];
+        pre += q < wave ? s : 0;
+        tot += s;
+      }
+      const int64_t s = run - (int64_t)(pre + incl - cnt);
+      sv = s > 0 ? s : 0;
+      const int64_t d = sv - o0;
+      const bool isbad = in && (d < mlo || d > mhi);
+      const uint64_t bm = __ballot(isbad);
+      if (lane == 0) wbad[wave] = __popcll(bm);
+      __syncthreads();
+      int32_t rank = __popcll(bm & below), nb = 0;
+#pragma unroll
+      for (int q = 0; q < DF_WAVES; q++) {
+        const int32_t b = wbad[q];
+        rank += q < wave ? b : 0;
+        nb += b;
+      }
+      if (nb == 0) break;
+      const int32_t nr = min(nb, DF_WAVES);
+      if (nrec > recount_cap - nr || round == DF_THREADS) {
+        fail = true;
+        break;
+      }
+      nrec += nr;
+      if (isbad && rank < nr) {
+        lst[rank] = t;
+        lst_s[rank] = sv;
+      }
+      __syncthreads();
+      if (wave < nr) {
+        const int32_t kk = c + lst[wave];
+        const int64_t at = lst_s[wave];
+        const ChunkCount r = decode_chunk_wave(jobs[kk], at, lane);
+        if (lane == 0) {
+          if (r.count < 0) *notconv = 1;
+          count[kk] = max(r.count, 0);
+          margin[2 * kk] = r.lo;
+          margin[2 * kk + 1] = r.hi;
+          s0[kk] = at;
+          res[wave][0] = max(r.count, 0);
+          res[wave][1] = r.lo;
+          res[wave][2] = r.hi;
+        }
+      }
+      __syncthreads();
+      if (isbad && rank < nr) {
+        cnt = res[rank][0];
+        mlo = res[rank][1];
+        mhi = res[rank][2];
+        o0 = sv;
+      }
+    }
+    if (fail) break;
+    if (in) s1[k] = sv;
+    run -= tot;
+  }
+  if (t == 0) {
+    recounts[blockIdx.x] = nrec;
+    if (fail) {
+      *notconv = 1;
+    } else {
+      const int64_t left = run < 1 ? 0 : run;
+      rem[blockIdx.x] = left;
+      if (un.tail_c >= 0) s1[un.tail_c] = left; else *un.status = left;
+    }
+  }
+}
+
+__global__ void __launch_bounds__(DC_THREADS) k_decode_write(const DecUnit *units, int32_t n_units,
+                                                             const ChunkJob *jobs, int32_t n_all,
+                                                             const int64_t *start, int32_t *count, int32_t *margin,
+                                                             const int32_t *notconv) {
+  __shared__ int32_t wsum[DC_WAVES];
+  __shared__ int32_t wlo[DC_WAVES], whi[DC_WAVES];
+  __shared__ int32_t s_tot;
+  if (*notconv) return;
+  if ((int32_t)blockIdx.x < n_units) {
+    if (threadIdx.x >= 64) return;
+    const DecUnit un = units[blockIdx.x];
+    if (threadIdx.x == 0) un.j[0] = 0;
+    if (un.tail_c < 0) return;
+    decode_tail(TailJob{un.words, un.n_words, un.tail_base, start + un.tail_c, un.j, un.status}, (int)threadIdx.x);
+    return;
+  }
+  const int32_t stride = (int32_t)gridDim.x - n_units;
+  for (int32_t c = (int32_t)blockIdx.x - n_units; c < n_all; c += stride) {
+    decode_chunk<true>(jobs, c, start[c], count, margin, wsum, wlo, whi, s_tot);
+    __syncthreads();
+  }
 }
 
 constexpr int SD_THREADS = 640;
@@ -955,9 +1184,17 @@
   TplSet *out;
 };
 
-int32_t decode_parallel(mh_ctx *ctx, const std::vector<DecJob> &dec, int64_t *d_status, bool *done) {
+constexpr int DEC_MAX_GLOBAL = 32;
+constexpr int DEC_GLOBAL_PASSES = 1;
+
+int32_t decode_parallel(mh_ctx *ctx, const std::vector<DecJob> &dec, int64_t *d_status, bool *done,
+                        int32_t global_passes = -1, int32_t recount_cap = -1) {
   hipStream_t st = ctx->stream;
   *done = false;
+  const int G = global_passes < 0 ? DEC_GLOBAL_PASSES : std::min<int>(global_passes, DEC_MAX_GLOBAL);
+  const int32_t cap = recount_cap < 0 ? -1 : recount_cap;
+  ctx->dec_queue.clear();
+  ctx->dec_recounts.clear();
   const int64_t div = 128;
   const int64_t minw = 64;
   std::vector<ChunkJob> cj;
@@ -1008,8 +1245,8 @@
       tiles.push_back(DecTile{u, b, std::min(b + tile_sz, first[u + 1]), ft});
   }
   const int32_t T = (int32_t)tiles.size();
-  const size_t bytes = ((sizeof(ChunkJob) * C + 15) / 16) * 16 + 8 * C * 2 + 8 * U * 2 + sizeof(TailJob) * U +
-                       sizeof(DecTile) * (T + 1) + 4 * C * 2 + 8 * C + 512;
+  const size_t bytes = ((sizeof(ChunkJob) * C + 15) / 16) * 16 + 8 * C * 2 + 8 * U * 2 + sizeof(DecUnit) * U +
+                       sizeof(DecTile) * (T + 1) + 4 * C * 2 + 8 * C + 4 * (size_t)(3 + DEC_MAX_GLOBAL + U) + 512;
   MH_TRY(ensure(ctx, ctx->dec_buf, bytes));
   char *p = (char *)ctx->dec_buf.p;
   ChunkJob *d_jobs = (ChunkJob *)p;
@@ -1017,73 +1254,85 @@
   int64_t *d_s1 = d_s0 + C;
   int64_t *d_ndraw = d_s1 + C;
   int64_t *d_rem = d_ndraw + U;
-  TailJob *d_tail = (TailJob *)(d_rem + U);
-  DecTile *d_tiles = (DecTile *)(d_tail + U);
+  DecUnit *d_units = (DecUnit *)(d_rem + U);
+  DecTile *d_tiles = (DecTile *)(d_units + U);
   int32_t *d_count = (int32_t *)(d_tiles + T + 1);
   int32_t *d_todo = d_count + C;
   int32_t *d_margin = d_todo + C;
   int32_t *d_ntodo = d_margin + 2 * C;
+  int32_t *d_notconv = d_ntodo + 2;
+  int32_t *d_qlen = d_notconv + 1;
+  int32_t *d_rec = d_qlen + DEC_MAX_GLOBAL;
   std::vector<int64_t> ndraw(U);
   for (int32_t u = 0; u < U; u++) ndraw[u] = dec[u].n;
-  std::vector<TailJob> tj;
+  std::vector<DecUnit> du(U);
   for (int32_t u = 0; u < U; u++)
-    if (tail_c[u] >= 0 && dec[u].n > 0)
-      tj.push_back(TailJob{dec[u].words, dec[u].n_words, cj[tail_c[u]].base, d_s1 + tail_c[u], dec[u].j, dec[u].status});
+    du[u] = DecUnit{dec[u].words, dec[u].n_words, dec[u].n, tail_c[u] >= 0 ? cj[tail_c[u]].base : 0, dec[u].j,
+                    dec[u].status, first[u], tail_c[u] >= 0 ? tail_c[u] : first[u + 1], tail_c[u], 0};
+  int64_t *hs = pinned_small(ctx);
+  if (!hs) return arg_fail(ctx, MH_E_OOM, "pinned host memory");
   HIPCHK(ctx, hipMemcpyAsync(d_jobs, cj.data(), sizeof(ChunkJob) * C, hipMemcpyHostToDevice, st));
   HIPCHK(ctx, hipMemcpyAsync(d_s0, s0.data(), 8 * C, hipMemcpyHostToDevice, st));
   HIPCHK(ctx, hipMemcpyAsync(d_tiles, tiles.data(), sizeof(DecTile) * T, hipMemcpyHostToDevice, st));
   HIPCHK(ctx, hipMemcpyAsync(d_ndraw, ndraw.data(), 8 * U, hipMemcpyHostToDevice, st));
-  if (!tj.empty()) HIPCHK(ctx, hipMemcpyAsync(d_tail, tj.data(), sizeof(TailJob) * tj.size(), hipMemcpyHostToDevice, st));
-  HIPCHK(ctx, hipMemsetAsync(d_ntodo, 0, 8, st));
+  HIPCHK(ctx, hipMemcpyAsync(d_units, du.data(), sizeof(DecUnit) * U, hipMemcpyHostToDevice, st));
+  HIPCHK(ctx, hipMemsetAsync(d_ntodo, 0, 4 * (size_t)(3 + DEC_MAX_GLOBAL + U), st));
   const unsigned grid = (unsigned)std::min<int64_t>(C, 4096);
-  constexpr int MAX_PASSES = 64;
-  const int PASS_BATCH = 24;
-  hipLaunchKernelGGL(k_decode_chunks<false>, dim3(grid), dim3(DC_THREADS), 0, st, (const ChunkJob *)d_jobs,
+  hipLaunchKernelGGL(k_decode_chunks, dim3(grid), dim3(DC_THREADS), 0, st, (const ChunkJob *)d_jobs,
                      (const int32_t *)nullptr, (const int32_t *)nullptr, (int32_t)C, (const int64_t *)d_s0, d_count,
-                     d_margin);
+                     d_margin, (int32_t *)nullptr);
   HIPCHK(ctx, hipGetLastError());
-  bool conv = false;
   int passes = 1;
-  while (passes < MAX_PASSES) {
-    int32_t *cur = d_ntodo;
-    for (int k = 0; k < PASS_BATCH; k++, passes++) {
-      cur = d_ntodo + (passes & 1);
-      int32_t *nxt = d_ntodo + ((passes + 1) & 1);
-      const unsigned g = passes < 4 ? grid : std::min(grid, 1024u);
-      hipLaunchKernelGGL(k_decode_resolve, dim3(T), dim3(DR_THREADS), 0, st, (const DecTile *)d_tiles,
-                         (const int64_t *)d_ndraw, (const int32_t *)d_count, (const int32_t *)d_margin, d_s0, d_s1,
-                         d_todo, cur, nxt, d_rem);
-      hipLaunchKernelGGL(k_decode_chunks<false>, dim3(g), dim3(DC_THREADS), 0, st, (const ChunkJob *)d_jobs,
-                         (const int32_t *)d_todo, (const int32_t *)cur, (int32_t)C, (const int64_t *)d_s0, d_count,
-                         d_margin);
-    }
+  for (int k = 0; k < G; k++, passes++) {
+    int32_t *cur = d_ntodo + (passes & 1);
+    int32_t *nxt = d_ntodo + ((passes + 1) & 1);
+    const unsigned g = passes < 4 ? grid : std::min(grid, 1024u);
+    hipLaunchKernelGGL(k_decode_resolve, dim3(T), dim3(DR_THREADS), 0, st, (const DecTile *)d_tiles,
+                       (const int64_t *)d_ndraw, (const int32_t *)d_count, (const int32_t *)d_margin, d_s0, d_s1,
+                       d_todo, cur, nxt, d_rem);
+    hipLaunchKernelGGL(k_decode_chunks, dim3(g), dim3(DC_THREADS), 0, st, (const ChunkJob *)d_jobs,
+                       (const int32_t *)d_todo, (const int32_t *)cur, (int32_t)C, (const int64_t *)d_s0, d_count,
+                       d_margin, d_qlen + k);
+  }
+  HIPCHK(ctx, hipGetLastError());
+  ctx->dec_passes = passes;
+  hipLaunchKernelGGL(k_decode_finish, dim3((unsigned)U), dim3(DF_THREADS), 0, st, (const DecUnit *)d_units,
+                     (const ChunkJob *)d_jobs, d_count, d_margin, d_s0, d_s1, d_rem, cap, d_notconv, d_rec);
+  hipLaunchKernelGGL(k_decode_write, dim3(grid + (unsigned)U), dim3(DC_THREADS), 0, st, (const DecUnit *)d_units, U,
+                     (const ChunkJob *)d_jobs, (int32_t)C, (const int64_t *)d_s1, d_count, d_margin,
+                     (const int32_t *)d_notconv);
+  HIPCHK(ctx, hipGetLastError());
+  const int32_t n_rec = 4 * (size_t)(1 + DEC_MAX_GLOBAL + U) <= 8 * (512 - 32) ? U : 0;
+  int32_t *h_info = (int32_t *)(hs + 32);
+  HIPCHK(ctx, hipMemcpyAsync(h_info, d_notconv, 4 * (size_t)(1 + DEC_MAX_GLOBAL + n_rec), hipMemcpyDeviceToHost, st));
+  SYNCCHK(ctx, hipStreamSynchronize(st));
+  ctx->dec_queue.assign(h_info + 1, h_info + 1 + G);
+  ctx->dec_recounts.assign(h_info + 1 + DEC_MAX_GLOBAL, h_info + 1 + DEC_MAX_GLOBAL + n_rec);
+  *done = h_info[0] == 0;
+  if (const char *tp = getenv("MH_DEC_TRACE")) {
+    if (FILE *f = fopen(tp, "a")) {
+      fprintf(f, "units %d chunks %lld notconv %d queue", U, (long long)C, h_info[0]);
+      for (int32_t q : ctx->dec_queue) fprintf(f, " %d", q);
+      fprintf(f, " recounts");
+      for (int32_t r : ctx->dec_recounts) fprintf(f, " %d", r);
+      fprintf(f, "\n");
+      fclose(f);
+    }
+  }
+  return MH_OK;
+}
+
+int32_t decode_batch(mh_ctx *ctx, const std::vector<DecJob> &dec, const DecJob *d_dec, int64_t *d_status,
+                     int32_t global_passes, int32_t recount_cap, bool *fallback) {
+  bool done = false;
+  ctx->dec_queue.clear();
+  ctx->dec_recounts.clear();
+  if (!ctx->decode_sequential) MH_TRY(decode_parallel(ctx, dec, d_status, &done, global_passes, recount_cap));
+  if (!done) {
+    hipLaunchKernelGGL(k_shuffle_decode2, dim3((unsigned)dec.size()), dim3(DC_THREADS), 0, ctx->stream, d_dec);
     HIPCHK(ctx, hipGetLastError());
-    int64_t *hs = pinned_small(ctx);
-    if (!hs) return arg_fail(ctx, MH_E_OOM, "pinned host memory");
-    HIPCHK(ctx, hipMemcpyAsync(hs + 32, cur, 4, hipMemcpyDeviceToHost, st));
-    SYNCCHK(ctx, hipStreamSynchronize(st));
-    const int32_t h_ntodo = (int32_t)(hs[32] & 0xffffffff);
-    if (h_ntodo == 0) {
-      conv = true;
-      break;
-    }
-  }
-  ctx->dec_passes = passes;
-  if (!conv) return MH_OK;
-  hipLaunchKernelGGL(k_decode_chunks<true>, dim3(grid), dim3(DC_THREADS), 0, st, (const ChunkJob *)d_jobs,
-                     (const int32_t *)nullptr, (const int32_t *)nullptr, (int32_t)C, (const int64_t *)d_s1, d_count,
-                     d_margin);
-  HIPCHK(ctx, hipGetLastError());
-  for (int32_t u = 0; u < U; u++)
-    if (dec[u].n > 0 && tail_c[u] < 0) HIPCHK(ctx, hipMemcpyAsync(dec[u].status, d_rem + u, 8, hipMemcpyDeviceToDevice, st));
-  if (!tj.empty()) {
-    hipLaunchKernelGGL(k_decode_tail, dim3((unsigned)tj.size()), dim3(64), 0, st, (const TailJob *)d_tail);
-    HIPCHK(ctx, hipGetLastError());
-  }
-  for (size_t u = 0; u < dec.size(); u++)
-    if (dec[u].n > 0) HIPCHK(ctx, hipMemsetAsync(dec[u].j, 0, 4, st));
-  SYNCCHK(ctx, hipStreamSynchronize(st));
-  *done = true;
+  }
+  if (fallback) *fallback = !done;
   return MH_OK;
 }
 
@@ -1376,13 +1625,7 @@
         stage_end(ctx);
       }
       stage_begin(ctx, "sample_shuffle_decode");
-      bool done = false;
-      if (!ctx->decode_sequential) MH_TRY(decode_parallel(ctx, dec, d_status, &done));
-      if (!done) {
-        hipLaunchKernelGGL(k_shuffle_decode2, dim3((unsigned)dec.size()), dim3(DC_THREADS), 0, st,
-                           (const DecJob *)d_dec);
-        HIPCHK(ctx, hipGetLastError());
-      }
+      MH_TRY(decode_batch(ctx, dec, d_dec, d_status, -1, -1, nullptr));
       stage_end(ctx);
       SYNCCHK(ctx, hipStreamSynchronize(st));
     }
@@ -1691,6 +1934,81 @@
   return MH_OK;
 }
 
+int32_t selftest_decode(mh_ctx *ctx, int32_t n_units, const uint32_t *shuffle_seeds, const int64_t *n_draws,
+                        int32_t global_passes, int32_t recount_cap, const int64_t *words_cap, uint32_t *j_out,
+                        int64_t *info) {
+  if (n_units < 1 || n_units > 4096 || !shuffle_seeds || !n_draws || !j_out || !info)
+    return arg_fail(ctx, MH_E_ARG, "bad decode self-test arguments");
+  std::vector<int64_t> w_off(n_units), j_off(n_units), n_words(n_units);
+  int64_t words_total = 0, j_total = 0;
+  for (int32_t u = 0; u < n_units; u++) {
+    if (n_draws[u] < 1 || n_draws[u] > ((int64_t)1 << 30) - 8)
+      return arg_fail(ctx, MH_E_ARG, "decode self-test: draws out of range");
+    n_words[u] = shuffle_words_alloc(n_draws[u]);
+    if (words_cap && words_cap[u] == 0) return arg_fail(ctx, MH_E_ARG, "decode self-test: words_cap 0");
+    w_off[u] = words_total;
+    words_total = (words_total + n_words[u] + 4 + 3) & ~(int64_t)3;
+    j_off[u] = j_total;
+    j_total += n_draws[u] + 4;
+  }
+  hipStream_t st = ctx->stream;
+  const int64_t SEG_WORDS = seg_words();
+  DevBuf bw, bj, bs, bt;
+  const int32_t rc = [&]() -> int32_t {
+    MH_TRY(ensure(ctx, bw, 4 * (size_t)words_total + 64));
+    MH_TRY(ensure(ctx, bj, 4 * (size_t)j_total + 64));
+    MH_TRY(ensure(ctx, bs, 8 * (size_t)n_units + 64));
+    uint32_t *words = (uint32_t *)bw.p, *jall = (uint32_t *)bj.p;
+    int64_t *d_status = (int64_t *)bs.p;
+    std::vector<SegJob> jobs;
+    std::vector<DecJob> dec;
+    int64_t kmax = 0;
+    for (int32_t u = 0; u < n_units; u++) {
+      for (int64_t k = 0; k * SEG_WORDS < n_words[u]; k++) {
+        const int64_t s0 = k * SEG_WORDS;
+        jobs.push_back(SegJob{words + w_off[u], s0, std::min(SEG_WORDS, n_words[u] - s0), shuffle_seeds[u], (int32_t)k});
+        kmax = std::max(kmax, k);
+      }
+      const int64_t nw = words_cap && words_cap[u] > 0 ? std::min(words_cap[u], n_words[u]) : n_words[u];
+      dec.push_back(DecJob{words + w_off[u], nw, n_draws[u], jall + j_off[u], d_status + u});
+    }
+    MH_TRY(ensure_polys(ctx, st, kmax, SEG_WORDS));
+    MH_TRY(ensure(ctx, bt, sizeof(SegJob) * jobs.size() + sizeof(DecJob) * dec.size() + 64));
+    SegJob *d_jobs = (SegJob *)bt.p;
+    DecJob *d_dec = (DecJob *)((char *)bt.p + ((sizeof(SegJob) * jobs.size() + 15) / 16) * 16);
+    HIPCHK(ctx, hipMemcpyAsync(d_jobs, jobs.data(), sizeof(SegJob) * jobs.size(), hipMemcpyHostToDevice, st));
+    HIPCHK(ctx, hipMemcpyAsync(d_dec, dec.data(), sizeof(DecJob) * dec.size(), hipMemcpyHostToDevice, st));
+    HIPCHK(ctx, hipMemsetAsync(d_status, 0, 8 * (size_t)n_units, st));
+    HIPCHK(ctx, hipMemsetAsync(jall, 0xff, 4 * (size_t)j_total, st));
+    hipLaunchKernelGGL(k_mt_segments, dim3((unsigned)jobs.size()), dim3(256), 0, st, (const SegJob *)d_jobs,
+                       (const uint32_t *)ctx->jump_polys.p);
+    HIPCHK(ctx, hipGetLastError());
+    bool fallback = false;
+    MH_TRY(decode_batch(ctx, dec, d_dec, d_status, global_passes, recount_cap, &fallback));
+    std::vector<int64_t> hstat(n_units);
+    int64_t at = 0;
+    for (int32_t u = 0; u < n_units; u++) {
+      HIPCHK(ctx, hipMemcpyAsync(j_out + at, jall + j_off[u], 4 * (size_t)n_draws[u], hipMemcpyDeviceToHost, st));
+      at += n_draws[u];
+    }
+    HIPCHK(ctx, hipMemcpyAsync(hstat.data(), d_status, 8 * (size_t)n_units, hipMemcpyDeviceToHost, st));
+    SYNCCHK(ctx, hipStreamSynchronize(st));
+    info[0] = fallback ? 1 : 0;
+    info[1] = (int64_t)ctx->dec_queue.size();
+    for (int k = 0; k < DEC_MAX_GLOBAL; k++) info[2 + k] = k < (int)ctx->dec_queue.size() ? ctx->dec_queue[k] : -1;
+    for (int32_t u = 0; u < n_units; u++) {
+      info[2 + DEC_MAX_GLOBAL + 2 * u] = u < (int32_t)ctx->dec_recounts.size() ? ctx->dec_recounts[u] : -1;
+      info[2 + DEC_MAX_GLOBAL + 2 * u + 1] = hstat[u];
+    }
+    return MH_OK;
+  }();
+  release(bw);
+  release(bj);
+  release(bs);
+  release(bt);
+  return rc;
+}
+
 int32_t sample_units_async(mh_ctx *ctx, int32_t n_units, const int32_t *tpl_ids, const int64_t *p_min,
                            const int64_t *p_max, const uint64_t *seeds, double p, int32_t rlen, const double *cum_tlen,
                            int32_t n_tlen, int32_t rng_mode, const NodeIdx *nidx) {
```

Measured after the change: 1.708 billion (median of 3 runs). About the same (-0.3%).
